# jfdev001/algebraic-multigrid

Hardware: AMD Instinct MI355X
Metric: V-cycles/sec, 2D Poisson N=4096^2 (fine-grid smoother HBM GB/s under roofline) (higher is better)
Workload: dtype f64; 1 GPU; 2D 5-point Poisson 4096x4096 (Grid::laplacian/rhs), true Jacobi smoother omega=0.6 2+2 sweeps, 16-level V-cycle, coarsest 511 dofs, fp64, 1xMI355X; smoother has no counterpart in the reference: pinned to the oracle twin; n=4096, dim=2, levels=16, smoother=jacobi, sweeps=2, graph=True, coarse_solve=band-chain (LDS-resident scalar recurrence, half-bandwidth <= 3, bit-exact), layout=dict

## Files before the change

### algebraic-multigrid_amd/amg_ctypes.py

```python
import contextlib
import ctypes as C
import os

import numpy as np

_HERE = os.path.dirname(os.path.abspath(__file__))
LIB_PATH = os.path.join(_HERE, "libamg_hip.so")

OK, EINVAL, EHIP, ENOMEM, EUNSUPPORTED, ECOMM = 0, 1, 2, 3, 4, 5
SM_SPGS, SM_REF_JACOBI, SM_SOR, SM_JACOBI, SM_MULTICOLOR_GS, SM_CHEBYSHEV, SM_LINE_JACOBI = 0, 1, 2, 3, 4, 5, 6
SM_LINE_ALT = 7
LAYOUT_AUTO, LAYOUT_CSR, LAYOUT_SELL, LAYOUT_DICT = 0, 1, 2, 3

_i32p = C.POINTER(C.c_int32)
_f64p = C.POINTER(C.c_double)
_i64p = C.POINTER(C.c_int64)


class AmgHipError(RuntimeError):
    def __init__(self, status, msg):
        super().__init__(f"amg_hip status {status}: {msg}")
        self.status = status
        self.message = msg

# ... 85 lines not shown
                                             C.POINTER(C.c_void_p)]),
    "amg_hip_create_tensor_semi_dev": (C.c_int, [C.c_int64, C.c_void_p, C.c_void_p, C.c_void_p, C.c_void_p,
                                                 C.c_int32, _i64p, C.c_int32, _i32p, C.c_double, C.c_int64,
                                                 C.POINTER(Options), C.POINTER(C.c_void_p)]),
    "amg_hip_get_level_axes": (C.c_int, [C.c_void_p, C.c_int32, _i32p]),
    "amg_hip_create_tensor_opdep": (C.c_int, [C.c_int64, _i32p, _i32p, _f64p, _f64p, C.c_int32, _i64p,
                                              C.c_int32, _i32p, C.c_int64, C.POINTER(Options),
                                              C.POINTER(C.c_void_p)]),
    "amg_hip_set_axis_stencil": (None, [C.c_int32]),
    "amg_hip_get_axis_weights": (C.c_int, [C.c_void_p, C.c_int32, _f64p]),
    "amg_hip_axis_restrict": (C.c_int, [C.c_int32, _i64p, C.c_int32, _f64p, _f64p, _f64p]),
    "amg_hip_axis_prolong_add": (C.c_int, [C.c_int32, _i64p, C.c_int32, _f64p, _f64p, _f64p]),
    "amg_hip_get_natural_sides": (C.c_int, [C.c_void_p, _i32p]),
    "amg_hip_create_tensor_periodic": (C.c_int, [C.c_int64, _i32p, _i32p, _f64p, _f64p, C.c_int32, _i64p,
                                                 C.c_int32, C.c_int32, _i32p, C.POINTER(Options),
                                                 C.POINTER(C.c_void_p)]),
    "amg_hip_create_tensor_periodic_dev": (C.c_int, [C.c_int64, C.c_void_p, C.c_void_p, C.c_void_p, C.c_void_p,
                                                     C.c_int32, _i64p, C.c_int32, C.c_int32, _i32p,
                                                     C.POINTER(Options), C.POINTER(C.c_void_p)]),
    "amg_hip_get_periodic_axes": (C.c_int, [C.c_void_p, _i32p]),
    "amg_hip_tensor_restrict_per": (C.c_int, [C.c_int32, _i64p, C.c_int32, C.c_int32, C.c_int32, _f64p, _f64p]),
    "amg_hip_tensor_prolong_add_per": (C.c_int, [C.c_int32, _i64p, C.c_int32, C.c_int32, C.c_int32, _f64p, _f64p]),
    "amg_hip_tensor_restrict_bc": (C.c_int, [C.c_int32, _i64p, C.c_int32, C.c_int32, _f64p, _f64p]),
    "amg_hip_tensor_prolong_add_bc": (C.c_int, [C.c_int32, _i64p, C.c_int32, C.c_int32, _f64p, _f64p]),
    "amg_hip_tensor_axis_strength": (C.c_int, [C.c_int64, _i32p, _i32p, _f64p, C.c_int32, _i64p, _f64p]),
    "amg_hip_tensor_restrict_axes": (C.c_int, [C.c_int32, _i64p, C.c_int32, _f64p, _f64p]),
    "amg_hip_tensor_prolong_add_axes": (C.c_int, [C.c_int32, _i64p, C.c_int32, _f64p, _f64p]),
    "amg_hip_level_transfer_kind": (C.c_int, [C.c_void_p, C.c_int32, _i32p]),
    "amg_hip_tensor_restrict": (C.c_int, [C.c_int32, _i64p, _f64p, _f64p]),
    "amg_hip_tensor_prolong_add": (C.c_int, [C.c_int32, _i64p, _f64p, _f64p]),
    "amg_hip_destroy": (None, [C.c_void_p]),
    "amg_hip_vcycle": (C.c_int, [C.c_void_p]),
    "amg_hip_vcycles": (C.c_int, [C.c_void_p, C.c_int32]),
    "amg_hip_sync": (C.c_int, [C.c_void_p]),
    "amg_hip_solve": (C.c_int, [C.c_void_p, C.c_double, C.c_int64, C.c_int64, _i64p, _f64p,
                                _i32p]),
    "amg_hip_rss": (C.c_int, [C.c_void_p, _f64p]),
    "amg_hip_apply": (C.c_int, [C.c_void_p, C.c_void_p, C.c_void_p]),
    "amg_hip_pcg": (C.c_int, [C.c_void_p, C.c_double, C.c_int64, _i64p, _f64p]),
    "amg_hip_set_mean_projection": (C.c_int, [C.c_void_p, C.c_int32]),
    "amg_hip_get_mean_projection": (C.c_int, [C.c_void_p, _i32p]),
    "amg_hip_center_vec": (C.c_int, [C.c_void_p, C.c_int32, C.c_int32]),
    "amg_hip_block_vcycles": (C.c_int, [C.c_void_p, C.c_int32, C.c_void_p, C.c_void_p, C.c_int32]),
    "amg_hip_block_rss": (C.c_int, [C.c_void_p, C.c_int32, C.c_void_p, C.c_void_p, _f64p]),
    "amg_hip_block_pcg": (C.c_int, [C.c_void_p, C.c_int32, C.c_void_p, C.c_void_p, C.c_double, C.c_int64,
                                    _i64p, _f64p]),
    "amg_hip_block_must_move": (C.c_int, [C.c_void_p, C.c_int32, _f64p]),
    "amg_hip_apply_f32": (C.c_int, [C.c_void_p, C.c_void_p, C.c_void_p]),
    "amg_hip_pcg_mixed": (C.c_int, [C.c_void_p, C.c_double, C.c_int64, _i64p, _f64p]),
    "amg_hip_f32_must_move": (C.c_int, [C.c_void_p, _f64p]),
    "amg_hip_f32_get_vec": (C.c_int, [C.c_void_p, C.c_int32, C.c_int32, C.POINTER(C.c_float)]),
    "amg_hip_f32_set_vec": (C.c_int, [C.c_void_p, C.c_int32, C.c_int32, C.POINTER(C.c_float)]),
    "amg_hip_f32_level_op": (C.c_int, [C.c_void_p, C.c_int32, C.c_int32]),
    "amg_hip_f32_line_subsweep": (C.c_int, [C.c_void_p, C.c_int32, C.c_int32, C.c_int32]),
    "amg_hip_f32_line_factors": (C.c_int, [C.c_void_p, C.c_int32] + [C.POINTER(C.c_float)] * 3),
    "amg_hip_set_f32_lines": (None, [C.c_int32]),
    "amg_hip_set_f32_dict": (None, [C.c_int32]),
    "amg_hip_set_block_lines": (None, [C.c_int32]),
    "amg_hip_n_levels": (C.c_int32, [C.c_void_p]),
    "amg_hip_get_n_dofs": (C.c_int64, [C.c_void_p, C.c_int32]),
    "amg_hip_get_level_nnz": (C.c_int64, [C.c_void_p, C.c_int32]),
    "amg_hip_get_level_matrix": (C.c_int, [C.c_void_p, C.c_int32, _i32p, _i32p, _f64p]),
    "amg_hip_get_transfer_nnz": (C.c_int64, [C.c_void_p, C.c_int32, C.c_int32]),
    "amg_hip_get_transfer": (C.c_int, [C.c_void_p, C.c_int32, C.c_int32, _i32p, _i32p, _f64p]),
    "amg_hip_get_vec": (C.c_int, [C.c_void_p, C.c_int32, C.c_int32, _f64p]),
    "amg_hip_set_vec": (C.c_int, [C.c_void_p, C.c_int32, C.c_int32, _f64p]),
    "amg_hip_copy_vec_dev": (C.c_int, [C.c_void_p, C.c_int32, C.c_int32, C.c_void_p, C.c_int32]),
    "amg_hip_zero_vec": (C.c_int, [C.c_void_p, C.c_int32, C.c_int32]),
    "amg_hip_coarse_halfbw": (C.c_int64, [C.c_void_p]),
    "amg_hip_coarse_solve_kind": (C.c_int32, [C.c_void_p]),
    "amg_hip_fine_sweep_info": (C.c_int, [C.c_void_p, C.c_char_p, C.c_int32, _i32p, _f64p]),
    "amg_hip_set_patch_min_rows": (None, [C.c_int64]),
    "amg_hip_set_band_chain": (None, [C.c_int32]),
    "amg_hip_set_tail_fusion": (None, [C.c_int32]),
    "amg_hip_set_pair_duo": (None, [C.c_int32]),
    "amg_hip_pair_duo_partner": (C.c_int32, [C.c_void_p, C.c_int32]),
    "amg_hip_duo_windows": (C.c_int32, [C.c_int32, C.c_int32, C.c_int32, _i32p]),
    "amg_hip_duo_owned": (C.c_int32, [C.c_int32, C.c_int32, _i32p]),
    "amg_hip_duo_tile_rows": (C.c_int32, [C.c_int32]),
    "amg_hip_set_periodic_device_setup": (None, [C.c_int32]),
    "amg_hip_set_patch_tile_flags": (None, [C.c_int32]),
    "amg_hip_set_patch_xf": (None, [C.c_int32]),
    "amg_hip_set_patch_tall": (None, [C.c_int32]),
    "amg_hip_set_patch_seam": (None, [C.c_int32]),
    "amg_hip_patch_leg_lines": (C.c_int32, [C.c_void_p, C.c_int32, C.c_int32]),
    "amg_hip_create_rs": (C.c_int, [C.c_int64, _i32p, _i32p, _f64p, _f64p, C.c_int32, C.c_double, C.c_int64,
                                    C.POINTER(Options), C.POINTER(C.c_void_p)]),
    "amg_hip_slab_plan": (C.c_int, [C.c_int64, C.c_int32, C.c_int32, C.c_int32, C.POINTER(SlabInfo)]),
    "amg_hip_slab_setup": (C.c_int, [C.c_void_p, C.c_int32, C.c_int32, C.c_int32, C.POINTER(SlabInfo)]),
    "amg_hip_slab_run": (C.c_int, [C.c_void_p, C.c_int32]),
    "amg_hip_create_poisson_window": (C.c_int, [C.c_int32, C.c_int64, C.c_int64, C.c_int64, C.c_int32,
                                                C.POINTER(Options), C.POINTER(C.c_void_p)]),
    "amg_hip_window_setup": (C.c_int, [C.c_void_p, _i64p, _i64p, _i64p, _i64p]),
    "amg_hip_window_run": (C.c_int, [C.c_void_p, C.c_int32]),
    "amg_hip_vec_dev_ptr": (C.c_int, [C.c_void_p, C.c_int32, C.c_int32, C.POINTER(C.c_void_p), _i64p]),
    "amg_hip_get_stream": (C.c_int, [C.c_void_p, C.POINTER(C.c_void_p)]),
    "amg_hip_comm_unique_id": (C.c_int, [C.c_char_p]),
    "amg_hip_comm_create": (C.c_int, [C.c_char_p, C.c_int32, C.c_int32, C.c_int32, C.POINTER(C.c_void_p)]),
    "amg_hip_comm_destroy": (None, [C.c_void_p]),
    "amg_hip_comm_rank": (C.c_int32, [C.c_void_p]),
    "amg_hip_comm_world": (C.c_int32, [C.c_void_p]),
    "amg_hip_comm_neighbor_exchange": (C.c_int, [C.c_void_p, C.c_void_p, C.c_int64, C.c_void_p, C.c_int64,
                                                 C.c_void_p, C.c_int64, C.c_void_p, C.c_int64, C.c_void_p]),
    "amg_hip_comm_all_gather": (C.c_int, [C.c_void_p, C.c_void_p, C.c_void_p, C.c_int64, C.c_void_p]),
    "amg_hip_slab_cycle": (C.c_int, [C.c_void_p, C.c_void_p, C.POINTER(SlabInfo)]),
    "amg_hip_window_cycle": (C.c_int, [C.c_void_p, C.c_void_p, C.c_void_p, C.POINTER(WindowPlanC)]),
    "amg_hip_level_layout": (C.c_int32, [C.c_void_p, C.c_int32, C.POINTER(C.c_int32), C.POINTER(C.c_int64)]),
    "amg_hip_get_colors": (C.c_int, [C.c_void_p, C.c_int32, _i32p, _i32p]),
    "amg_hip_level_op": (C.c_int, [C.c_void_p, C.c_int32, C.c_int32]),
    "amg_hip_cheb_bounds": (C.c_int, [C.c_void_p, C.c_int32, _f64p, _f64p]),
    "amg_hip_line_stride": (C.c_int, [C.c_void_p, C.c_int32, C.POINTER(C.c_int64)]),
    "amg_hip_smooth_line": (C.c_int, [C.c_int64, _i32p, _i32p, _f64p, C.c_int64, C.c_double, C.c_int64,
                                      _f64p, _f64p]),
    "amg_hip_line_directions": (C.c_int, [C.c_void_p, C.c_int32, C.POINTER(C.c_int32), C.POINTER(C.c_int64)]),
    "amg_hip_smooth_line_alt": (C.c_int, [C.c_int64, _i32p, _i32p, _f64p, C.c_int32, C.POINTER(C.c_int64),
                                          C.c_double, C.c_int64, C.c_int32, _f64p, _f64p]),
    "amg_hip_line_cyclic": (C.c_int, [C.c_void_p, C.c_int32, _i32p]),
    "amg_hip_smooth_line_alt_per": (C.c_int, [C.c_int64, _i32p, _i32p, _f64p, C.c_int32, C.POINTER(C.c_int64),
                                              C.c_int32, C.c_double, C.c_int64, C.c_int32, _f64p, _f64p]),
    "amg_hip_smooth_chebyshev": (C.c_int, [C.c_int64, _i32p, _i32p, _f64p, _f64p, _f64p, C.c_int32,
                                           C.c_double, C.c_double, C.c_int64]),
    "amg_hip_cycle_bytes": (C.c_int, [C.c_void_p, _f64p, _f64p]),
    "amg_hip_cycle_must_move": (C.c_int, [C.c_void_p, C.c_int32, _f64p]),
    "amg_hip_profile_fine_sweep": (C.c_int, [C.c_void_p, C.c_int32, _f64p, _f64p]),
    "amg_hip_smooth": (C.c_int, [C.c_int32, C.c_int64, _i32p, _i32p, _f64p, _f64p, _f64p,
                                 C.c_double, C.c_double, C.c_int64, C.c_int64, _i64p, _i32p]),
    "amg_hip_spgs_sweep": (C.c_int, [C.c_int32, C.c_int64, _i32p, _i32p, _f64p, _f64p, _f64p]),
    "amg_hip_residual": (C.c_int, [C.c_int64, _i32p, _i32p, _f64p, _f64p, _f64p, _f64p]),
    "amg_hip_spmv": (C.c_int, [C.c_int64, C.c_int64, _i32p, _i32p, _f64p, _f64p, _f64p]),
    "amg_hip_linear_restrict": (C.c_int, [C.c_int64, C.c_int64, _f64p, _f64p]),
    "amg_hip_linear_prolong_add": (C.c_int, [C.c_int64, C.c_int64, _f64p, _f64p]),
    "amg_hip_rss_host": (C.c_int, [C.c_int64, _i32p, _i32p, _f64p, _f64p, _f64p, _f64p]),
    "amg_hip_coarse_solve": (C.c_int, [C.c_int64, _i32p, _i32p, _f64p, _f64p, _f64p, _i64p]),
    "amg_hip_coarse_solve_fast": (C.c_int, [C.c_int64, _i32p, _i32p, _f64p, _f64p, _f64p, _i64p,
                                            _i32p]),
    "amg_hip_laplacian": (C.c_int64, [C.c_int32, C.c_int64, _i32p, _i32p, _f64p]),
    "amg_hip_rhs": (C.c_int, [C.c_int32, C.c_int64, _f64p]),
    "amg_hip_csr_shape": (C.c_int, [C.c_int64, _i32p, _i32p, _i32p]),
    "amg_hip_dev_residual": (C.c_int, [C.c_int64, C.c_int64, C.c_int32, C.c_int32, C.c_void_p,
                                       C.c_void_p, C.c_void_p, C.c_void_p, C.c_void_p,
                                       C.c_void_p, C.c_void_p]),
    "amg_hip_dev_jacobi": (C.c_int, [C.c_int64, C.c_int64, C.c_int32, C.c_int32, C.c_void_p,
                                     C.c_void_p, C.c_void_p, C.c_void_p, C.c_void_p, C.c_void_p,
                                     C.c_double, C.c_int64, C.c_void_p]),
    "amg_hip_dev_spmv": (C.c_int, [C.c_int64, C.c_int64, C.c_int32, C.c_int32, C.c_void_p,
                                   C.c_void_p, C.c_void_p, C.c_void_p, C.c_void_p, C.c_void_p]),
    "amg_hip_devmat_create": (C.c_int, [C.c_int64, C.c_int64, _i32p, _i32p, _f64p, C.c_int32,
                                        C.c_int64, C.c_int32, C.POINTER(C.c_void_p)]),
    "amg_hip_set_index16": (None, [C.c_int32]),
    "amg_hip_set_nontemporal": (None, [C.c_int32]),
    "amg_hip_set_dict_rows": (None, [C.c_int32]),
    "amg_hip_set_dict_stencil": (None, [C.c_int32]),
    "amg_hip_set_xcd_mapping": (None, [C.c_int32]),
    "amg_hip_set_row_types": (None, [C.c_int32]),
    "amg_hip_dict_probe": (C.c_int, [C.c_int64, C.c_int64, _i32p, _i32p, _f64p, C.c_int64,
                                     C.POINTER(C.c_int32), C.POINTER(C.c_int32), C.POINTER(C.c_int32)]),
    "amg_hip_devmat_destroy": (None, [C.c_void_p]),
    "amg_hip_devmat_layout": (C.c_int, [C.c_void_p, C.POINTER(C.c_int32), C.POINTER(C.c_int64)]),
    "amg_hip_devmat_apply": (C.c_int, [C.c_void_p, C.c_int32, C.c_void_p, C.c_void_p, C.c_void_p,
                                       C.c_double, C.c_int64, C.c_void_p]),
    "amg_hip_dev_jacobi_from_zero": (C.c_int, [C.c_int64, C.c_void_p, C.c_void_p, C.c_void_p,
                                               C.c_double, C.c_void_p]),
    "amg_hip_dev_axpy1": (C.c_int, [C.c_int64, C.c_void_p, C.c_void_p, C.c_void_p]),
    "amg_hip_arena_create": (C.c_int, [C.c_int64, C.c_int32, C.POINTER(C.c_void_p)]),
    "amg_hip_arena_destroy": (None, [C.c_void_p]),
    "amg_hip_arena_base": (C.c_void_p, [C.c_void_p]),
# ... 60 lines not shown


def set_default_layout(layout):
    lib().amg_hip_set_default_layout(layout)


def set_index16(on):
    lib().amg_hip_set_index16(int(on))


def set_nontemporal(on):
    lib().amg_hip_set_nontemporal(int(on))


def set_dict_rows(rows_per_lane):
    lib().amg_hip_set_dict_rows(int(rows_per_lane))


def set_dict_stencil(on):
    lib().amg_hip_set_dict_stencil(int(on))


def dict_probe(rowptr, col, val, ncols, diag_shift=0):
    rowptr, col, val = _a32(rowptr), _a32(col), _a64(val)
    a, b, c = C.c_int32(0), C.c_int32(0), C.c_int32(0)
    st = lib().amg_hip_dict_probe(rowptr.size - 1, ncols, _p32(rowptr), _p32(col), _p64(val),
                                  diag_shift, C.byref(a), C.byref(b), C.byref(c))
    if st == EUNSUPPORTED:
        return None
    _chk(st)
    return a.value, b.value, c.value


class Comm:

    def __init__(self, id_bytes, rank, world, device=-1):
        h = C.c_void_p()
        _chk(lib().amg_hip_comm_create(bytes(id_bytes), int(rank), int(world), int(device), C.byref(h)))
        self._h, self.rank, self.world = h, rank, world

    @staticmethod
    def unique_id():
        buf = C.create_string_buffer(128)
        _chk(lib().amg_hip_comm_unique_id(buf))
        return buf.raw

    def slab_cycle(self, mg, info):
        _chk(lib().amg_hip_slab_cycle(mg._h, self._h, C.byref(info)))

    def window_cycle(self, window_mg, tail_mg, plan_c):
        _chk(lib().amg_hip_window_cycle(window_mg._h, tail_mg._h, self._h, C.byref(plan_c)))

    def close(self):
        if getattr(self, "_h", None):
            lib().amg_hip_comm_destroy(self._h)
            self._h = None

    def __del__(self):
        self.close()


def slab_plan(lines, rank, world, levels):
    info = SlabInfo()
    _chk(lib().amg_hip_slab_plan(int(lines), int(rank), int(world), int(levels), C.byref(info)))
    return info


def set_patch_tile_flags(on):
    lib().amg_hip_set_patch_tile_flags(int(bool(on)))


def set_axis_stencil(on):
    lib().amg_hip_set_axis_stencil(int(bool(on)))


def set_patch_xf(on):
    lib().amg_hip_set_patch_xf(int(bool(on)))


def set_patch_tall(on):
    lib().amg_hip_set_patch_tall(int(bool(on)))


def set_patch_seam(on):
    lib().amg_hip_set_patch_seam(int(bool(on)))


def set_tail_fusion(on):
    lib().amg_hip_set_tail_fusion(int(bool(on)))


def set_pair_duo(on):
    lib().amg_hip_set_pair_duo(int(bool(on)))


DUO_WINDOWS_LEN = 31


def duo_windows(hb_l, hb_l1, tile_rows=510):
    out = np.zeros(DUO_WINDOWS_LEN, np.int32)
    rc = lib().amg_hip_duo_windows(int(hb_l), int(hb_l1), int(tile_rows), out.ctypes.data_as(_i32p))
    return rc == 0, out


def duo_owned(tile, tile_rows=510):
    out = np.zeros(6, np.int32)
    if lib().amg_hip_duo_owned(int(tile), int(tile_rows), out.ctypes.data_as(_i32p)) != 0:
        raise ValueError("amg_hip_duo_owned: bad argument")
    return [(int(out[0]), int(out[1])), (int(out[2]), int(out[3])), (int(out[4]), int(out[5]))]


def duo_tile_rows(hb_l):
    return int(lib().amg_hip_duo_tile_rows(int(hb_l)))


def set_periodic_device_setup(on):
    lib().amg_hip_set_periodic_device_setup(int(bool(on)))


def set_f32_lines(on):
    lib().amg_hip_set_f32_lines(int(bool(on)))


@contextlib.contextmanager
def f32_lines():
    set_f32_lines(1)
    try:
        yield
    finally:
        set_f32_lines(0)


def set_f32_dict(on):
    lib().amg_hip_set_f32_dict(int(bool(on)))


@contextlib.contextmanager
def f32_dict():
    set_f32_dict(1)
    try:
        yield
    finally:
        set_f32_dict(0)


def set_block_lines(on):
    lib().amg_hip_set_block_lines(int(bool(on)))


@contextlib.contextmanager
def block_lines():
    set_block_lines(1)
    try:
        yield
    finally:
        set_block_lines(0)


def set_band_chain(on):
    lib().amg_hip_set_band_chain(int(bool(on)))


PATCH_MIN_ROWS_DEFAULT = 1000000


def set_patch_min_rows(rows):
# ... 525 lines not shown
        return int(lib().amg_hip_get_n_dofs(self._h, level))

    def get_coefficient_matrix(self, level):
        n = self.get_n_dofs(level)
        nnz = lib().amg_hip_get_level_nnz(self._h, level)
        colptr = np.empty(n + 1, np.int32)
        rowind = np.empty(nnz, np.int32)
        val = np.empty(nnz, np.float64)
        _chk(lib().amg_hip_get_level_matrix(self._h, level, _p32(colptr), _p32(rowind), _p64(val)))
        return colptr, rowind, val

    def get_transfer(self, level, which):
        w = 1 if which == "R" else 0
        nnz = lib().amg_hip_get_transfer_nnz(self._h, level, w)
        if nnz < 0:
            raise ValueError("level out of range")
        n_h, n_H = self.get_n_dofs(level), self.get_n_dofs(level + 1)
        cols = n_h if w else n_H
        colptr = np.empty(cols + 1, np.int32)
        rowind = np.empty(nnz, np.int32)
        val = np.empty(nnz, np.float64)
        _chk(lib().amg_hip_get_transfer(self._h, level, w, _p32(colptr), _p32(rowind), _p64(val)))
        return colptr, rowind, val

    def _get(self, level, which):
        out = np.empty(self.get_n_dofs(level), np.float64)
        _chk(lib().amg_hip_get_vec(self._h, level, which, _p64(out)))
        return out

    def get_soln(self, level=0):
        return self._get(level, 0)

    def get_rhs(self, level=0):
        return self._get(level, 1)

    def get_residual(self, level=0):
        return self._get(level, 2)

    def set_vec(self, level, which, v):
        v = _a64(v)
        assert v.size == self.get_n_dofs(level)
        _chk(lib().amg_hip_set_vec(self._h, level, {"u": 0, "f": 1, "r": 2}[which], _p64(v)))

    def copy_vec_dev(self, level, which, dev_ptr, to_solver):
        _chk(lib().amg_hip_copy_vec_dev(self._h, level, {"u": 0, "f": 1, "r": 2}[which],
                                        C.c_void_p(dev_ptr), int(to_solver)))

    def zero_vec(self, level, which):
        _chk(lib().amg_hip_zero_vec(self._h, level, {"u": 0, "f": 1, "r": 2}[which]))

    def get_tolerance(self):
        return self.tolerance

    def level_layout(self, level):
        lay, nb = C.c_int32(0), C.c_int64(0)
        _chk(lib().amg_hip_level_layout(self._h, level, C.byref(lay), C.byref(nb)))
        return int(lay.value), int(nb.value)

    def coarse_halfbw(self):
        return int(lib().amg_hip_coarse_halfbw(self._h))

    def get_colors(self, level):
        color = np.empty(self.get_n_dofs(level), np.int32)
        nc = C.c_int32(0)
        _chk(lib().amg_hip_get_colors(self._h, level, _p32(color), C.byref(nc)))
        return color, nc.value

    def cycle_bytes(self):
        a, b = C.c_double(0), C.c_double(0)
        _chk(lib().amg_hip_cycle_bytes(self._h, C.byref(a), C.byref(b)))
        return a.value, b.value

    def cycle_must_move(self, part=0):
        b = C.c_double(0)
        _chk(lib().amg_hip_cycle_must_move(self._h, int(part), C.byref(b)))
        return b.value

    def pair_duo_partner(self, level):
        return int(lib().amg_hip_pair_duo_partner(self._h, int(level)))

    def patch_leg_lines(self, level, leg):
        return int(lib().amg_hip_patch_leg_lines(self._h, int(level), int(leg)))

    def profile_fine_sweep(self, n_launches):
        a, b = C.c_double(0), C.c_double(0)
        _chk(lib().amg_hip_profile_fine_sweep(self._h, n_launches, C.byref(a), C.byref(b)))
        name = C.create_string_buffer(256)
        k, nb = C.c_int32(0), C.c_double(0)
        _chk(lib().amg_hip_fine_sweep_info(self._h, name, 256, C.byref(k), C.byref(nb)))
        return a.value, b.value, k.value, name.value.decode(), nb.value

    def fine_sweep_info(self):
        name = C.create_string_buffer(256)
        k, nb = C.c_int32(0), C.c_double(0)
        _chk(lib().amg_hip_fine_sweep_info(self._h, name, 256, C.byref(k), C.byref(nb)))
        return name.value.decode(), k.value, nb.value

    def cheb_bounds(self, level):
        lo, hi = C.c_double(0), C.c_double(0)
        st = lib().amg_hip_cheb_bounds(self._h, int(level), C.byref(lo), C.byref(hi))
        if st == EINVAL:
            raise ValueError(lib().amg_hip_last_error().decode())
        _chk(st)
        return lo.value, hi.value

    def line_stride(self, level):
        s = C.c_int64(0)
        st = lib().amg_hip_line_stride(self._h, int(level), C.byref(s))
        if st == EINVAL:
            raise ValueError(lib().amg_hip_last_error().decode())
        _chk(st)
        return s.value

    def line_directions(self, level):
        nd = C.c_int32(0)
        st3 = (C.c_int64 * 3)()
        st = lib().amg_hip_line_directions(self._h, int(level), C.byref(nd), st3)
        if st == EINVAL:
            raise ValueError(lib().amg_hip_last_error().decode())
        _chk(st)
        return [int(st3[d]) for d in range(nd.value)]

    def line_cyclic(self, level):
        m = C.c_int32(0)
        st = lib().amg_hip_line_cyclic(self._h, int(level), C.byref(m))
        if st == EINVAL:
            raise ValueError(lib().amg_hip_last_error().decode())
        _chk(st)
        return m.value

    def coarse_solve_kind(self):
        return {0: "band (one wave, sequential, bit-exact)", 1: "spike (partitioned, parallel)",
                2: "band-wide (blocked sequential, any half-bandwidth, bit-exact)",
                3: "band-chain (LDS-resident scalar recurrence, half-bandwidth <= 3, bit-exact)"}[
                    int(lib().amg_hip_coarse_solve_kind(self._h))]

    def level_op(self, level, op):
        _chk(lib().amg_hip_level_op(self._h, level, op))

    def vcycle(self, n=1):
        _chk(lib().amg_hip_vcycles(self._h, n))

    def sync(self):
        _chk(lib().amg_hip_sync(self._h))

    def rss(self):
        out = C.c_double(0)
        _chk(lib().amg_hip_rss(self._h, C.byref(out)))
        return out.value

    def slab_setup(self, rank, world, max_levels=-1):
        info = SlabInfo()
        _chk(lib().amg_hip_slab_setup(self._h, int(rank), int(world), int(max_levels), C.byref(info)))
        return info

    def slab_run(self, part):
        _chk(lib().amg_hip_slab_run(self._h, int(part)))

    def apply_dev(self, v_dev, z_dev):
        _chk(lib().amg_hip_apply(self._h, C.c_void_p(v_dev), C.c_void_p(z_dev)))

    def pcg(self, rtol=1e-10, max_iters=100):
        it, rel = C.c_int64(0), C.c_double(0)
        _chk(lib().amg_hip_pcg(self._h, rtol, max_iters, C.byref(it), C.byref(rel)))
        return self.get_soln(0), it.value, rel.value

# ... 360 lines not shown
```

### algebraic-multigrid_amd/csrc/kernels.hip

```cpp
#include <hip/hip_runtime.h>
#include <cstdlib>
#include <stdint.h>

#include <cstdio>
#include <type_traits>
#include <utility>
#include <vector>
#include <algorithm>
#include <cmath>

#include "kernels.hpp"

namespace amg_hip {

__device__ __forceinline__ void lds_barrier() {
  asm volatile("s_waitcnt lgkmcnt(0)\n\ts_barrier" ::: "memory");
}

constexpr bool mode_cheb(int m) { return (m & ~3) == 16; }
constexpr bool mode_jac(int m) { return m == CSR_JACOBI || mode_cheb(m); }
constexpr bool cheb_first(int m) { return (m & 1) != 0; }
constexpr bool cheb_last(int m) { return (m & 2) != 0; }
template <int MODE>
__device__ __forceinline__ double cheb_update(double t, double xi, double di, double alpha, double beta,
// ... 1506 lines not shown
  constexpr int WC0 = DUO_U_M0 * W0, WC1 = DUO_U_M1 * W1;
  __shared__ DictEntry tab[256];
  __shared__ __attribute__((aligned(16))) uint64_t wc0[WC0];
  __shared__ __attribute__((aligned(16))) uint64_t wc1[WC1];
  __shared__ uint16_t tw0[DUO_U_M0 / 2];
  __shared__ uint16_t tw1[DUO_U_M1 / 2];
  __shared__ __attribute__((aligned(16))) double aw1[DUO_U_A1];
  __shared__ __attribute__((aligned(16))) double fw1[DUO_U_M1];
  __shared__ __attribute__((aligned(16))) double uw1[DUO_U_M1];
  __shared__ __attribute__((aligned(16))) double aw0[DUO_U_A0];
  __shared__ __attribute__((aligned(16))) double fw0[DUO_U_M0];
  __shared__ __attribute__((aligned(16))) double uw0[DUO_U_M0];
  double* vw1 = aw1;
  double* rs = aw0;
  int w[DW_COUNT];
  duo_windows(hbw0, hbw1, T, w);
  const int tile = xcd_tile(blockIdx.x, gridDim.x, xcd_map);
  const int t0 = tile * T, ce = (t0 / 2) & ~1;
  const int m0 = t0 - hbw0, M0 = w[DW_U_M0], A0 = w[DW_U_A0];
  const int m1 = ce - w[DW_U_M1_LO], M1 = w[DW_U_M1], A1 = w[DW_U_A1];
  const bool types0 = rtype0 != nullptr, types1 = rtype1 != nullptr;
  const int t = threadIdx.x;
  DuoLoads<W1, (DUO_U_A1 / 2 + 255) / 256, 1> g1;
  DuoLoads<W0, (DUO_U_A0 / 2 + 255) / 256, (DUO_U_M0 + 511) / 512> g0;
  if (types1) duo_issue<W1, true>(g1, n1, m1 - hbw1, A1, m1, M1, codes1, rtype1, rwords1, doff1, dval1, ntab1, a1, f1);
  else duo_issue<W1, false>(g1, n1, m1 - hbw1, A1, m1, M1, codes1, rtype1, rwords1, doff1, dval1, ntab1, a1, f1);
  if (types0) duo_issue<W0, true>(g0, n0, m0 - hbw0, A0, m0, M0, codes0, rtype0, rwords0, doff0, dval0, ntab0, u0_in, f0);
  else duo_issue<W0, false>(g0, n0, m0 - hbw0, A0, m0, M0, codes0, rtype0, rwords0, doff0, dval0, ntab0, u0_in, f0);
  pair_f64x2 pre[2];
  double pre1;
  if (T == DUO_T) dict_prolong_pre<DUO_T>(tile, n0, n_h, uh_in, pre, pre1);
  else dict_prolong_pre<DUO_T_SMALL>(tile, n0, n_h, uh_in, pre, pre1);
  dict_put_table<CSR_JACOBI>(tab, g1.tv, g1.to, ntab1);
  if (types1) duo_commit<W1, true>(g1, n1, A1, m1, M1, wc1, tw1, aw1, fw1);
  else duo_commit<W1, false>(g1, n1, A1, m1, M1, wc1, tw1, aw1, fw1);
  if (types0) duo_commit<W0, true>(g0, n0, A0, m0, M0, wc0, tw0, aw0, fw0);
  else duo_commit<W0, false>(g0, n0, A0, m0, M0, wc0, tw0, aw0, fw0);
  __syncthreads();
  duo_stage<CSR_JACOBI, W1, U1>(n1, m1, M1, 0, M1, types1, tab, wc1, tw1, fw1, aw1, hbw1, omega, uw1, nullptr, 0, 0);
  __syncthreads();
  int own[6];
  duo_owned(t0, T, own);
  const int c_own = own[2], c_end = own[3];
  duo_stage<CSR_JACOBI, W1, U1>(n1, m1, M1, hbw1, w[DW_U_S1], types1, tab, wc1, tw1, fw1, uw1, 0, omega, vw1,
                                u1_out, c_own, c_end);
  __syncthreads();
  dict_put_table<CSR_JACOBI>(tab, g0.tv, g0.to, ntab0);
  {
    const int s1 = ce - w[DW_U_S1_LO], a_lo = m0 - hbw0;
    for (int k = 2 * t; k < A0; k += 512) {
      const int i = a_lo + k;
      if (i < 0 || i >= n0) continue;
      const int j = i >> 1;
      double p0 = 0.0, p1 = 0.0;
      const double b = (j < n1) ? vw1[j - s1] : 0.0;
      if (j >= 1 && j - 1 < n1) p0 += 0.5 * vw1[j - 1 - s1];
      if (j < n1) {
        p0 += 0.5 * b;
        p1 += 1.0 * b;
      }
      aw0[k] = aw0[k] + p0;
      if (i + 1 < n0) aw0[k + 1] = aw0[k + 1] + p1;
    }
  }
  __syncthreads();
  duo_stage<CSR_JACOBI, W0, U0>(n0, m0, M0, 0, M0, types0, tab, wc0, tw0, fw0, aw0, hbw0, omega, uw0, nullptr, 0, 0);
  __syncthreads();
  duo_stage<CSR_JACOBI, W0, U0>(n0, m0, M0, hbw0, w[DW_U_S0], types0, tab, wc0, tw0, fw0, uw0, 0, omega, rs, u0_out,
                                own[0], own[1]);
  __syncthreads();
  if (T == DUO_T) dict_prolong_tail<DUO_T>(tile, n0, rs, n_h, pre, pre1, uh_out);
  else dict_prolong_tail<DUO_T_SMALL>(tile, n0, rs, n_h, pre, pre1, uh_out);
}

constexpr int PATCH_TW = 64;
constexpr int PATCH_EH = 48;
constexpr int patch_th(int rings) { return PATCH_EH - 2 * rings; }
static bool patch_rings_ok(int rings) { return rings == 2 || rings == 3; }
constexpr int PATCH_EC = PATCH_TW + 8;
constexpr int PATCH_NT = 432;
constexpr int PATCH_K = PATCH_EH * PATCH_EC / PATCH_NT;
constexpr int PATCH_BUF = (PATCH_EH + 2) * PATCH_EC;
constexpr int PATCH_MAXTAB = 192;
static_assert(PATCH_EH * PATCH_EC == PATCH_K * PATCH_NT && PATCH_NT % PATCH_EC == 0, "patch geometry");
template <int EH_, int EC_>
struct PatchFrameT {
  static constexpr int EH = EH_, EC = EC_, CL = (EC_ - PATCH_TW) / 2;
  static constexpr int NT = EH_ / PATCH_K * EC_, BUF = (EH_ + 2) * EC_;
  static constexpr int th(int rings) { return EH_ - 2 * rings; }
  static_assert(EH_ % PATCH_K == 0 && (EC_ - PATCH_TW) % 2 == 0 && NT >= PATCH_MAXTAB && NT <= 1024, "patch frame");
};
using PatchFrame = PatchFrameT<PATCH_EH, PATCH_EC>;
static_assert(PatchFrame::NT == PATCH_NT && PatchFrame::BUF == PATCH_BUF && PatchFrame::CL == 4, "patch geometry");

struct PatchJ { double a, d; };
struct PatchR { double a; int32_t loff, ok; };

struct PatchCells {
  int cell0, row0, lj0, li;
  double f[PATCH_K];
  uint32_t ty[PATCH_K / 4];
  bool live[PATCH_K];
  bool uniform;
  uint32_t tu;
  bool flagged;
  __device__ __forceinline__ uint32_t type(int k) const {
    return flagged ? tu : (ty[k >> 2] >> (8 * (k & 3))) & 255u;
  }
};

struct PatchU {
  double wj[9], wr[9], diag;
#ifdef AMG_PATCH_FASTDIV
  double rdiag;
#endif
  uint32_t rmask, corners;
};
__device__ __forceinline__ void patch_load_u(PatchU& U, uint32_t tu, const double* __restrict__ utabd,
                                             const int32_t* __restrict__ utabi) {
  const double* d = utabd + (size_t)tu * 19;
  const int32_t* i = utabi + (size_t)tu * 2;
#pragma unroll
  for (int e = 0; e < 9; ++e) {
    U.wj[e] = d[e];
    U.wr[e] = d[9 + e];
  }
  U.diag = d[18];
#ifdef AMG_PATCH_FASTDIV
  U.rdiag = 1.0 / (U.diag == 0.0 ? 1.0 : U.diag);
#endif
  U.rmask = (uint32_t)i[0];
  U.corners = (uint32_t)i[1];
}
template <bool RESID, bool CORNERS, bool GS = false, int MASK = -1, class FR = PatchFrame>
__device__ __forceinline__ void patch_eval_u(const double* buf, int cell0, const PatchU& U,
                                             const double (&f)[PATCH_K], double omega,
                                             double (&res)[PATCH_K]) {
  const double* p = buf + cell0 - FR::EC;
  if (!CORNERS && !RESID && U.diag == 0.0) {
#pragma unroll
    for (int k = 0; k < PATCH_K; ++k) res[k] = p[(k + 1) * FR::EC];
    return;
  }
  double w[3][3];
#pragma unroll
  for (int r = 0; r < 2; ++r)
#pragma unroll
    for (int c = 0; c < 3; ++c) w[r][c] = (CORNERS || c == 1 || r == 1) ? p[r * FR::EC + c - 1] : 0.0;
#pragma unroll
  for (int k = 0; k < PATCH_K; ++k) {
#pragma unroll
    for (int c = 0; c < 3; ++c)
      w[2][c] = (CORNERS || c == 1) ? p[(k + 2) * FR::EC + c - 1] : 0.0;
    if (!CORNERS) {
      w[2][0] = p[(k + 2) * FR::EC - 1];
      w[2][2] = p[(k + 2) * FR::EC + 1];
    }
    const double xi = w[1][1];
    if (RESID) {
      double acc = f[k];
#pragma unroll
      for (int s9 = 0; s9 < 9; ++s9) {
        const int r = s9 / 3, c = s9 % 3;
        if (!CORNERS && r != 1 && c != 1) continue;
        if (MASK >= 0) {
          if ((MASK >> s9) & 1) acc -= U.wr[s9] * w[r][c];
        } else {
          double t = U.wr[s9] * w[r][c];
          t = ((U.rmask >> s9) & 1u) ? t : 0.0;
          acc -= t;
        }
      }
      res[k] = acc;
    } else {
      double acc = 0.0;
#pragma unroll
      for (int s9 = 0; s9 < 9; ++s9) {
        const int r = s9 / 3, c = s9 % 3;
        if (s9 == 4 || (!CORNERS && r != 1 && c != 1)) continue;
        if (MASK >= 0 && !((MASK >> s9) & 1)) continue;
        acc += U.wj[s9] * w[r][c];
      }
      if (CORNERS && U.diag == 0.0) {
        res[k] = xi;
      } else {
#ifdef AMG_PATCH_FASTDIV
        const double nm = f[k] - acc;
        const double q0 = nm * U.rdiag;
        const double r0 = __builtin_fma(-U.diag, q0, nm);
        const double q1 = __builtin_fma(r0, U.rdiag, q0);
        const double r1 = __builtin_fma(-U.diag, q1, nm);
        const double q = __builtin_fma(r1, U.rdiag, q1);
#else
        const double q = (f[k] - acc) / U.diag;
#endif
        res[k] = GS ? q : xi + omega * (q - xi);
      }
    }
#pragma unroll
    for (int c = 0; c < 3; ++c) {
      w[0][c] = w[1][c];
      w[1][c] = w[2][c];
    }
  }
}
template <int UN, bool RESID, bool GS = false>
__device__ __forceinline__ double patch_eval(const double* buf, int cell, uint32_t type,
                                             const PatchJ* tabJ, const PatchR* tabR, double fi,
                                             double omega) {
  const int t0 = (int)type * UN;
  double xx[UN];
  if (RESID) {
    double av[UN];
    bool ok[UN];
#pragma unroll
    for (int e = 0; e < UN; ++e) {
      const PatchR r = tabR[t0 + e];
      av[e] = r.a;
      ok[e] = r.ok != 0;
      xx[e] = buf[cell + r.loff];
    }
    double acc = fi;
#pragma unroll
    for (int e = 0; e < UN; ++e) {
      double t = av[e] * xx[e];
      t = ok[e] ? t : 0.0;
      acc -= t;
    }
    return acc;
  }
  double aj[UN], dj[UN];
#pragma unroll
  for (int e = 0; e < UN; ++e) {
    const PatchJ j = tabJ[t0 + e];
    aj[e] = j.a; dj[e] = j.d;
    xx[e] = buf[cell + tabR[t0 + e].loff];
  }
  double acc = 0.0, diag = 0.0;
  const double xi = buf[cell];
#pragma unroll
  for (int e = 0; e < UN; ++e) {
    acc += aj[e] * xx[e];
    diag += dj[e];
  }
  const bool nod = diag == 0.0;
  const double q = (fi - acc) / (nod ? 1.0 : diag);
  return nod ? xi : (GS ? q : xi + omega * (q - xi));
}

template <int UN, int UM, bool RESID, bool NT, bool ZERO, int TH, class FR = PatchFrame>
__device__ __forceinline__ void patch_stage(const PatchCells& pc, int m, int ntypes, double* buf,
                                            const PatchU& U, const PatchJ* tabJ, const PatchR* tabR,
                                            double omega, int l0, int l1, int c0, int c1, double* out) {
  const bool inc = pc.li >= c0 && pc.li < c1;
  double res[PATCH_K];
  bool did[PATCH_K], inr[PATCH_K];
#pragma unroll
  for (int k = 0; k < PATCH_K; ++k) {
    const int lj = pc.lj0 + k;
    inr[k] = inc && lj >= l0 && lj < l1;
    did[k] = inr[k] && pc.live[k];
  }
  if (pc.uniform && U.rmask == (uint32_t)UM) {
    patch_eval_u<RESID, (UM & 0x145) != 0, false, (UM & 0x145) ? -1 : UM, FR>(buf, pc.cell0, U, pc.f, omega, res);
  } else {
#pragma unroll
    for (int k = 0; k < PATCH_K; ++k)
      res[k] = patch_eval<UN, RESID>(buf, pc.cell0 + k * FR::EC,
                                     did[k] ? pc.type(k) : (uint32_t)ntypes, tabJ, tabR, pc.f[k], omega);
  }
  lds_barrier();
  const bool outc = out != nullptr && pc.li >= 0 && pc.li < PATCH_TW;
#pragma unroll
  for (int k = 0; k < PATCH_K; ++k) {
    if (did[k]) buf[pc.cell0 + k * FR::EC] = res[k];
    else if (ZERO && inr[k]) buf[pc.cell0 + k * FR::EC] = 0.0;
    const int lj = pc.lj0 + k;
    if (outc && did[k] && lj >= 0 && lj < TH) {
      double* op = out + (pc.row0 + k * m);
      if (NT) __builtin_nontemporal_store(res[k], op);
      else *op = res[k];
    }
  }
}

template <bool NT, int RINGS, class FR = PatchFrame>
__device__ __forceinline__ void patch_copy_out(const double* buf, double* __restrict__ out, int n, int m,
                                               int j0, int i0) {
  for (int q = threadIdx.x; q < FR::th(RINGS) * PATCH_TW; q += FR::NT) {
    const int lj = q / PATCH_TW, li = q - lj * PATCH_TW;
    const int64_t row = (int64_t)(j0 + lj) * m + i0 + li;
    if (row < (int64_t)n) {
      const double v = buf[(lj + RINGS + 1) * FR::EC + li + FR::CL];
      if (NT) __builtin_nontemporal_store(v, out + row);
      else out[row] = v;
    }
  }
}

struct __attribute__((aligned(8))) PatchPair { double x, y; };

__device__ __forceinline__ uint32_t patch_flag(const uint8_t* __restrict__ flag, int idx) {
  const uint32_t* __restrict__ w = reinterpret_cast<const uint32_t*>(flag);
  return (w[idx >> 2] >> (8 * (idx & 3))) & 255u;
}

static_assert(PATCH_MAXTAB <= PATCH_NT, "one table row per thread");
struct PatchTabRow { double v[4]; };
__device__ __forceinline__ void patch_issue_tables(PatchTabRow& tb, const double* __restrict__ ptab, int nent) {
  const int t = (int)threadIdx.x < nent ? (int)threadIdx.x : 0;
#pragma unroll
  for (int q = 0; q < 4; ++q) tb.v[q] = ptab[4 * t + q];
}
template <class FR = PatchFrame>
__device__ __forceinline__ void patch_stage_tables(PatchJ* tabJ, PatchR* tabR, const PatchTabRow& tb, int nent) {
  const int t = threadIdx.x;
  if (t >= PATCH_MAXTAB) return;
  PatchJ j = {0.0, 0.0};
  PatchR r = {0.0, 0, 0};
  if (t < nent) {
    j.a = tb.v[0];
    j.d = tb.v[1];
    r.a = tb.v[2];
    const double lo = tb.v[3];
    r.ok = lo > -1.0e8 ? 1 : 0;
    r.loff = r.ok ? (int)lo : 0;
    if (FR::EC != PATCH_EC) r.loff += (r.loff > PATCH_EC / 2 ? 1 : (r.loff < -PATCH_EC / 2 ? -1 : 0)) * (FR::EC - PATCH_EC);
  }
  tabJ[t] = j;
  tabR[t] = r;
}
template <class FR = PatchFrame>
__device__ __forceinline__ void patch_clear_guards(double* buf) {
  for (int t = threadIdx.x; t < 2 * FR::EC; t += FR::NT)
    buf[t < FR::EC ? t : FR::BUF - 2 * FR::EC + t] = 0.0;
}
template <int UM, class FR = PatchFrame>
__device__ __forceinline__ void patch_prologue(const PatchCells& pc, const PatchU& U, double* buf, PatchJ* tabJ,
                                               PatchR* tabR, const double* __restrict__ ptab, int nent) {
  if (pc.flagged && U.rmask != (uint32_t)UM) {
    PatchTabRow tb;
    patch_issue_tables(tb, ptab, nent);
    patch_stage_tables<FR>(tabJ, tabR, tb, nent);
  }
  patch_clear_guards<FR>(buf);
}

template <class FR = PatchFrame>
__device__ __forceinline__ void patch_form_x(const PatchCells& pc, const PatchU& U,
                                             const double* __restrict__ utabd, double omega, double* buf) {
  double dv[PATCH_K];
  if (pc.uniform) {
#pragma unroll
    for (int k = 0; k < PATCH_K; ++k) dv[k] = U.diag;
  } else {
#pragma unroll
    for (int k = 0; k < PATCH_K; ++k) dv[k] = utabd[(size_t)pc.type(k) * 19 + 18];
  }
#pragma unroll
  for (int k = 0; k < PATCH_K; ++k) {
    const double sum = pc.f[k], d = dv[k];
    const double xi = 0.0, acc = 0.0;
    const double x0 = (d == 0.0) ? xi : xi + omega * ((sum - acc) / d - xi);
    buf[pc.cell0 + k * FR::EC] = pc.live[k] ? x0 : 0.0;
  }
}

template <int RINGS, bool PROLONG, bool XF = false, class FR = PatchFrame>
__device__ __forceinline__ void patch_load(PatchCells& pc, PatchU& U, const uint8_t* __restrict__ tflag,
                                           int tile, int n, int m,
                                           int j0, int i0, const double* __restrict__ x,
                                           const double* __restrict__ f,
                                           const uint8_t* __restrict__ rtype, int ntypes,
                                           const double* __restrict__ uH, int nH,
                                           const double* __restrict__ ptab, int nent,
                                           const double* __restrict__ utabd,
                                           const int32_t* __restrict__ utabi, double omega, double* buf,
                                           PatchJ* tabJ, PatchR* tabR) {
  const int g = (int)threadIdx.x / FR::EC, col = (int)threadIdx.x - g * FR::EC;
  const int le = g * PATCH_K;
  pc.lj0 = le - RINGS;
  pc.li = col - FR::CL;
  pc.cell0 = (le + 1) * FR::EC + col;
  const int64_t r0 = (int64_t)(j0 + pc.lj0) * m + i0 + pc.li;
  pc.row0 = (int)(r0 < -((int64_t)1 << 30) ? -((int64_t)1 << 30) : r0);
  double xv[PATCH_K];
  PatchPair pr[PATCH_K];
#pragma unroll
  for (int k = 0; k < PATCH_K; ++k) {
    const int64_t r64 = r0 + (int64_t)k * m;
    pc.live[k] = r64 >= 0 && r64 < (int64_t)n;
    if (!XF) xv[k] = x[pc.live[k] ? (int)r64 : 0];
  }
  if (PROLONG) {
#pragma unroll
    for (int k = 0; k < PATCH_K; ++k) {
      const int row = pc.row0 + k * m;
      const int j = pc.live[k] ? (row >> 1) : 0;
      const int jc = j < 1 ? 1 : (j > nH - 1 ? nH - 1 : j);
      pr[k] = *reinterpret_cast<const PatchPair*>(uH + (jc - 1));
    }
  }
  if (!PROLONG) {
#pragma unroll
    for (int k = 0; k < PATCH_K; ++k) {
      const int64_t r64 = r0 + (int64_t)k * m;
      pc.f[k] = f[pc.live[k] ? (int)r64 : 0];
    }
  }
  __builtin_amdgcn_sched_barrier(0);
  const uint32_t tf = tflag ? patch_flag(tflag, tile) : 255u;
  const uint32_t nty = (uint32_t)ntypes;
  pc.flagged = tf != 255u;
  if (pc.flagged) {
    pc.tu = tf;
    pc.uniform = true;
  } else {
    PatchTabRow tb;
    patch_issue_tables(tb, ptab, nent);
    uint32_t mism = 0, ty[PATCH_K];
#pragma unroll
    for (int k = 0; k < PATCH_K; ++k) {
      const int64_t r64 = r0 + (int64_t)k * m;
      ty[k] = (uint32_t)rtype[pc.live[k] ? (int)r64 : 0];
    }
#pragma unroll
    for (int q = 0; q < PATCH_K / 4; ++q) pc.ty[q] = 0;
#pragma unroll
    for (int k = 0; k < PATCH_K; ++k) {
      ty[k] = (pc.live[k] && ty[k] < nty) ? ty[k] : nty;
      pc.ty[k >> 2] |= ty[k] << (8 * (k & 3));
    }
    pc.tu = (uint32_t)__builtin_amdgcn_readfirstlane((int)ty[0]);
#pragma unroll
    for (int q = 0; q < PATCH_K / 4; ++q) mism |= pc.ty[q] ^ (pc.tu * 0x01010101u);
    pc.uniform = __builtin_amdgcn_ballot_w64(mism != 0) == 0 && pc.tu < nty;
    patch_stage_tables<FR>(tabJ, tabR, tb, nent);
  }
  {
    int fl = pc.flagged;
    asm("" : "+v"(fl));
    pc.flagged = __builtin_amdgcn_readfirstlane(fl) != 0;
  }
  patch_load_u(U, pc.uniform ? pc.tu : 0u, utabd, utabi);
  __builtin_amdgcn_sched_barrier(0);
  if (XF) patch_form_x<FR>(pc, U, utabd, omega, buf);
  if (PROLONG) {
    int row0 = pc.row0;
    asm volatile("" : "+v"(row0));
    pc.row0 = row0;
  }
#pragma unroll
  for (int k = 0; k < PATCH_K && !XF; ++k) {
    const int row = pc.row0 + k * m;
    double x0 = pc.live[k] ? xv[k] : 0.0;
    if (PROLONG) {
      const int j = pc.live[k] ? (row >> 1) : 0;
      const int jc = j < 1 ? 1 : (j > nH - 1 ? nH - 1 : j);
      const bool odd = (row & 1) != 0;
      const bool a_ok = pc.live[k] && !odd && j >= 1 && j - 1 < nH;
      const bool b_ok = pc.live[k] && j < nH;
      const double a = (j == jc) ? pr[k].x : pr[k].y;
      const double b = (j == jc) ? pr[k].y : pr[k].x;
      double t = 0.0;
      t = a_ok ? t + 0.5 * a : t;
      t = b_ok ? t + (odd ? 1.0 : 0.5) * b : t;
      x0 = pc.live[k] ? x0 + t : x0;
    }
    buf[pc.cell0 + k * FR::EC] = x0;
  }
  if (PROLONG) {
    __builtin_amdgcn_sched_barrier(0);
#pragma unroll
    for (int k = 0; k < PATCH_K; ++k) pc.f[k] = f[pc.live[k] ? pc.row0 + k * m : 0];
  }
}

__global__ __launch_bounds__(256) void patch_tile_flags_kernel(int n, int m, int px_count, int rings, int eh, int ec,
                                                               const uint8_t* __restrict__ rtype,
                                                               int ntypes, uint8_t* __restrict__ flag) {
  const int tile = blockIdx.x;
  const int py = tile / px_count, px = tile - py * px_count;
  const int64_t base = (int64_t)(py * (eh - 2 * rings) - rings) * m + px * PATCH_TW - (ec - PATCH_TW) / 2;
  const int64_t first = base < 0 ? 0 : (base < n ? base : n - 1);
  const uint32_t t0 = rtype[first];
  int ok = base >= 0 && t0 < (uint32_t)ntypes;
  for (int q = threadIdx.x; q < eh * ec; q += 256) {
    const int le = q / ec, c = q - le * ec;
    const int64_t r = base + (int64_t)le * m + c;
    ok = ok && r >= 0 && r < (int64_t)n && rtype[r < 0 ? 0 : (r < n ? r : n - 1)] == t0;
  }
  ok = __syncthreads_and(ok);
  if (threadIdx.x == 0) flag[tile] = ok ? (uint8_t)t0 : (uint8_t)255;
}
hipError_t launch_patch_tile_flags(int64_t n, int64_t m, int rings, const uint8_t* rtype, int ntypes,
                                   uint8_t* flag, int64_t* n_tiles, hipStream_t st) {
  if (!patch_geometry_ok(n, m) || !patch_rings_ok(rings)) return hipErrorInvalidValue;
  const int64_t lines = (n + m - 1) / m;
  const int pxc = (int)(m / PATCH_TW);
  const int64_t th = patch_th(rings);
  const int64_t tiles = (lines + th - 1) / th * pxc;
  if (n_tiles) *n_tiles = tiles;
  if (!flag) return hipSuccess;
  hipLaunchKernelGGL(patch_tile_flags_kernel, dim3((unsigned)tiles), dim3(256), 0, st, (int)n, (int)m, pxc,
                     rings, PATCH_EH, PATCH_EC, rtype, ntypes, flag);
  return hipGetLastError();
}

__global__ __launch_bounds__(256) void patch_coarse_flags_kernel(int n, int m, int px_count, int th, int nH,
                                                                 const double* __restrict__ diagH, double dref,
                                                                 uint8_t* __restrict__ cflag) {
  const int tile = blockIdx.x;
  const int py = tile / px_count, px = tile - py * px_count;
  const int j0 = py * th, i0 = px * PATCH_TW;
  int ok = 1;
  for (int q = threadIdx.x; q < th * (PATCH_TW / 2); q += 256) {
    const int lj = q / (PATCH_TW / 2), cx = q - lj * (PATCH_TW / 2);
    const int64_t i = (int64_t)(j0 + lj) * m + i0 + 2 * cx;
    const int64_t c = i >> 1;
    if (i >= (int64_t)n || c >= nH) continue;
    ok = ok && __double_as_longlong(diagH[c]) == __double_as_longlong(dref);
  }
  ok = __syncthreads_and(ok);
  if (threadIdx.x == 0) cflag[tile] = ok ? 1 : 0;
}
hipError_t launch_patch_coarse_flags(int64_t n, int64_t m, int rings, int64_t nH, const double* diagH,
                                     double dref, uint8_t* cflag, hipStream_t st) {
  if (!patch_geometry_ok(n, m) || !patch_rings_ok(rings) || !diagH || !cflag) return hipErrorInvalidValue;
  const int64_t lines = (n + m - 1) / m;
  const int pxc = (int)(m / PATCH_TW);
  const int64_t th = patch_th(rings);
  const int64_t tiles = (lines + th - 1) / th * pxc;
  hipLaunchKernelGGL(patch_coarse_flags_kernel, dim3((unsigned)tiles), dim3(256), 0, st, (int)n, (int)m, pxc,
                     (int)th, (int)nH, diagH, dref, cflag);
  return hipGetLastError();
}

#ifdef AMG_PATCH_STAMPS
__device__ unsigned long long* g_patch_stamps = nullptr;
__device__ __forceinline__ void patch_stamp(int k) {
  if (threadIdx.x == 0 && g_patch_stamps) {
    unsigned long long t = __builtin_amdgcn_s_memrealtime();
    asm volatile("s_waitcnt lgkmcnt(0)" ::: "memory");
    g_patch_stamps[(size_t)blockIdx.x * 8 + k] = t;
    if (k == 0) {
      const unsigned hw = __builtin_amdgcn_s_getreg((31 << 11) | 4);
      const unsigned xcc = __builtin_amdgcn_s_getreg((3 << 11) | 20);
      g_patch_stamps[(size_t)blockIdx.x * 8 + 7] = ((unsigned long long)xcc << 32) | hw;
    }
  }
}
hipError_t debug_set_patch_stamps(unsigned long long* p) {
  return hipMemcpyToSymbol(HIP_SYMBOL(g_patch_stamps), &p, sizeof(p));
}
#define PATCH_STAMP(k) patch_stamp(k)
#else
#define PATCH_STAMP(k)
#endif
template <int UN, int UM, bool FIRST, bool NT, bool XF = false, int RINGS = 3>
#ifndef AMG_PATCH_WAVES
#define AMG_PATCH_WAVES 7
#endif
__global__ __launch_bounds__(PATCH_NT, (UN == 5 ? AMG_PATCH_WAVES : AMG_PATCH_WAVES - 1)) void patch_down_kernel(
    int n, int m, int px_count, const uint8_t* __restrict__ rtype, const double* __restrict__ ptab,
    const double* __restrict__ utabd, const int32_t* __restrict__ utabi,
    int nent, int ntypes, const double* x, const double* __restrict__ f, double* u_out, double* r_out, int nH,
    double* __restrict__ fH, const double* __restrict__ diagH, double* __restrict__ uH1,
    double omega, int xcd_map, int py0, const uint8_t* __restrict__ tflag,
    const uint8_t* __restrict__ cflag, double dHu) {
  __shared__ double buf[PATCH_BUF];
  __shared__ PatchJ tabJ[PATCH_MAXTAB];
  __shared__ PatchR tabR[PATCH_MAXTAB];
  PATCH_STAMP(0);
  const int tile = xcd_tile(blockIdx.x, gridDim.x, xcd_map);
  const int py = tile / px_count, px = tile - py * px_count;
  constexpr int TH = patch_th(RINGS);
  const int j0 = (py + py0) * TH, i0 = px * PATCH_TW;
  PatchCells pc;
  PatchU U;
  const int ftile = (py + py0) * px_count + px;
  static_assert(!(FIRST && XF), "level 0 starts from its own u");
  static_assert(RINGS == 3 || (RINGS == 2 && !FIRST), "three dependent stages (FIRST) need three rings");
  patch_load<RINGS, false, XF>(pc, U, tflag, ftile, n, m, j0, i0, x, f, rtype, ntypes, nullptr, 0, ptab, nent,
                               utabd, utabi, omega, buf, tabJ, tabR);
  patch_prologue<UM>(pc, U, buf, tabJ, tabR, ptab, nent);
  const bool cuni = uH1 && cflag && patch_flag(cflag, ftile) != 0;
  lds_barrier();
  PATCH_STAMP(1);
  if (FIRST) {
    patch_stage<UN, UM, false, NT, false, TH>(pc, m, ntypes, buf, U, tabJ, tabR, omega, -2, TH + 2, -2,
                                              PATCH_TW + 3, nullptr);
    lds_barrier();
  }
  PATCH_STAMP(2);
  patch_stage<UN, UM, false, NT, false, TH>(pc, m, ntypes, buf, U, tabJ, tabR, omega, -1, TH + 1, -1,
                                            PATCH_TW + 2, nullptr);
  lds_barrier();
  PATCH_STAMP(3);
  patch_copy_out<NT, RINGS>(buf, u_out, n, m, j0, i0);
  patch_stage<UN, UM, true, NT, true, TH>(pc, m, ntypes, buf, U, tabJ, tabR, omega, 0, TH, 0, PATCH_TW + 1,
                                          r_out);
  lds_barrier();
  PATCH_STAMP(4);
  const double* rsb = buf;
  for (int q = threadIdx.x; q < TH * (PATCH_TW / 2); q += PATCH_NT) {
    const int lj = q / (PATCH_TW / 2), cx = q - lj * (PATCH_TW / 2);
    const int64_t i = (int64_t)(j0 + lj) * m + i0 + 2 * cx;
    const int64_t c = i >> 1;
    if (i >= (int64_t)n || c >= nH) continue;
    const double* rs = rsb + (lj + RINGS + 1) * PATCH_EC + 2 * cx + 4;
    double sum = 0.0;
    if (i < n) sum += 0.5 * rs[0];
    if (i + 1 < n) sum += 1.0 * rs[1];
    if (i + 2 < n) sum += 0.5 * rs[2];
    fH[c] = sum;
    if (uH1 == nullptr) continue;
    const double xi = 0.0, acc = 0.0;
    const double d = cuni ? dHu : diagH[c];
    uH1[c] = (d == 0.0) ? xi : xi + omega * ((sum - acc) / d - xi);
  }
  PATCH_STAMP(5);
}

template <int UN, int UM, bool NT, int RINGS = 3>
__global__ __launch_bounds__(PATCH_NT, AMG_PATCH_WAVES) void patch_up_kernel(
    int n, int m, int px_count, const uint8_t* __restrict__ rtype, const double* __restrict__ ptab,
    const double* __restrict__ utabd, const int32_t* __restrict__ utabi,
    int nent, int ntypes, const double* x, const double* __restrict__ f, const double* __restrict__ uH, int nH,
    double* u_out, double omega, int xcd_map, int py0, const uint8_t* __restrict__ tflag) {
  __shared__ double buf[PATCH_BUF];
  __shared__ PatchJ tabJ[PATCH_MAXTAB];
  __shared__ PatchR tabR[PATCH_MAXTAB];
  const int tile = xcd_tile(blockIdx.x, gridDim.x, xcd_map);
  const int py = tile / px_count, px = tile - py * px_count;
  static_assert(RINGS == 2 || RINGS == 3, "two dependent stages");
  constexpr int TH = patch_th(RINGS);
  const int j0 = (py + py0) * TH, i0 = px * PATCH_TW;
  PatchCells pc;
  PatchU U;
  patch_load<RINGS, true>(pc, U, tflag, (py + py0) * px_count + px, n, m, j0, i0, x, f, rtype, ntypes, uH, nH,
                          ptab, nent, utabd, utabi, omega, buf, tabJ, tabR);
  patch_prologue<UM>(pc, U, buf, tabJ, tabR, ptab, nent);
  lds_barrier();
  patch_stage<UN, UM, false, NT, false, TH>(pc, m, ntypes, buf, U, tabJ, tabR, omega, -1, TH + 1, -1,
                                            PATCH_TW + 1, nullptr);
  lds_barrier();
  patch_stage<UN, UM, false, NT, false, TH>(pc, m, ntypes, buf, U, tabJ, tabR, omega, 0, TH, 0, PATCH_TW,
                                            nullptr);
  lds_barrier();
  patch_copy_out<NT, RINGS>(buf, u_out, n, m, j0, i0);
}

constexpr int PATCH_SEAM_RINGS = 5;
template <int UN, int UM, bool NT, class FR, int WAVES>
__global__ __launch_bounds__(FR::NT, WAVES) void patch_seam_kernel(
    int n, int m, int px_count, const uint8_t* __restrict__ rtype, const double* __restrict__ ptab,
    const double* __restrict__ utabd, const int32_t* __restrict__ utabi,
    int nent, int ntypes, const double* x, const double* __restrict__ f, const double* __restrict__ uH, int nH,
    double* u_out, double* __restrict__ fH, double omega, int xcd_map, const uint8_t* __restrict__ tflag) {
  __shared__ double buf[FR::BUF];
  __shared__ PatchJ tabJ[PATCH_MAXTAB];
  __shared__ PatchR tabR[PATCH_MAXTAB];
  const int tile = xcd_tile(blockIdx.x, gridDim.x, xcd_map);
  const int py = tile / px_count, px = tile - py * px_count;
  constexpr int RINGS = PATCH_SEAM_RINGS, TH = FR::th(RINGS);
  static_assert(TH >= 1 && FR::CL >= RINGS + 1, "five stages and the restriction's column");
  const int j0 = py * TH, i0 = px * PATCH_TW;
  PatchCells pc;
  PatchU U;
  patch_load<RINGS, true, false, FR>(pc, U, tflag, tile, n, m, j0, i0, x, f, rtype, ntypes, uH, nH, ptab, nent,
                                     utabd, utabi, omega, buf, tabJ, tabR);
  patch_prologue<UM, FR>(pc, U, buf, tabJ, tabR, ptab, nent);
  lds_barrier();
#pragma unroll
  for (int q = 4; q >= 1; --q) {
    patch_stage<UN, UM, false, NT, false, TH, FR>(pc, m, ntypes, buf, U, tabJ, tabR, omega, -q, TH + q, -q,
                                                  PATCH_TW + q + 1, nullptr);
    lds_barrier();
  }
  patch_copy_out<NT, RINGS, FR>(buf, u_out, n, m, j0, i0);
  patch_stage<UN, UM, true, NT, true, TH, FR>(pc, m, ntypes, buf, U, tabJ, tabR, omega, 0, TH, 0, PATCH_TW + 1,
                                              nullptr);
  lds_barrier();
  for (int q = threadIdx.x; q < TH * (PATCH_TW / 2); q += FR::NT) {
    const int lj = q / (PATCH_TW / 2), cx = q - lj * (PATCH_TW / 2);
    const int64_t i = (int64_t)(j0 + lj) * m + i0 + 2 * cx;
    const int64_t c = i >> 1;
    if (i >= (int64_t)n || c >= nH) continue;
    const double* rs = buf + (lj + RINGS + 1) * FR::EC + 2 * cx + FR::CL;
    double sum = 0.0;
    if (i < n) sum += 0.5 * rs[0];
    if (i + 1 < n) sum += 1.0 * rs[1];
    if (i + 2 < n) sum += 0.5 * rs[2];
    fH[c] = sum;
  }
}

template <int UN, int UM>
__device__ __forceinline__ void patch_stage_color(const PatchCells& pc, int ntypes, double* buf,
                                                  const PatchU& U, const PatchJ* tabJ, const PatchR* tabR,
                                                  int l0, int l1, int c0, int c1, uint32_t cbits,
                                                  uint32_t c) {
  const bool inc = pc.li >= c0 && pc.li < c1;
  double res[PATCH_K];
  bool did[PATCH_K];
#pragma unroll
  for (int k = 0; k < PATCH_K; ++k) {
    const int lj = pc.lj0 + k;
    did[k] = inc && lj >= l0 && lj < l1 && pc.live[k] && ((cbits >> (2 * k)) & 3u) == c;
  }
  bool any = false;
#pragma unroll
  for (int k = 0; k < PATCH_K; ++k) any |= did[k];
  if (__builtin_amdgcn_ballot_w64(any) == 0) return;
  if (pc.uniform && U.rmask == (uint32_t)UM) {
    constexpr bool CN = (UM & 0x145) != 0;
    constexpr int MK = (UM & 0x145) ? -1 : UM;
    patch_eval_u<false, CN, true, MK>(buf, pc.cell0, U, pc.f, 1.0, res);
  } else {
#pragma unroll
    for (int k = 0; k < PATCH_K; ++k)
      res[k] = patch_eval<UN, false, true>(buf, pc.cell0 + k * PATCH_EC,
                                           did[k] ? pc.type(k) : (uint32_t)ntypes, tabJ, tabR, pc.f[k], 1.0);
  }
#pragma unroll
  for (int k = 0; k < PATCH_K; ++k)
    if (did[k]) buf[pc.cell0 + k * PATCH_EC] = res[k];
}

template <int UN, int UM, bool NT, bool PROLONG, bool TAIL>
#ifndef AMG_RB_WAVES
#define AMG_RB_WAVES 5
#endif
__global__ __launch_bounds__(PATCH_NT, AMG_RB_WAVES) void patch_rb_kernel(
    int n, int m, int px_count, const uint8_t* __restrict__ rtype, const double* __restrict__ ptab,
    const double* __restrict__ utabd, const int32_t* __restrict__ utabi, int nent, int ntypes,
    const double* x, const double* __restrict__ f, const double* __restrict__ uH, int nH, double* u_out,
    double* r_out, double* __restrict__ fH, double* __restrict__ uH_zero, uint32_t stages, uint32_t ctab,
    int xcd_map, int py0, const uint8_t* __restrict__ tflag) {
  __shared__ double buf[PATCH_BUF];
  __shared__ PatchJ tabJ[PATCH_MAXTAB];
  __shared__ PatchR tabR[PATCH_MAXTAB];
  const int tile = xcd_tile(blockIdx.x, gridDim.x, xcd_map);
  const int py = tile / px_count, px = tile - py * px_count;
  constexpr int RINGS = 3, TH = patch_th(RINGS);
  const int j0 = (py + py0) * TH, i0 = px * PATCH_TW;
  PatchCells pc;
  PatchU U;
  patch_load<RINGS, PROLONG>(pc, U, tflag, (py + py0) * px_count + px, n, m, j0, i0, x, f, rtype, ntypes, uH, nH,
                             ptab, nent, utabd, utabi, 1.0, buf, tabJ, tabR);
  patch_prologue<UM>(pc, U, buf, tabJ, tabR, ptab, nent);
  uint32_t cbits = 0;
  {
    const int col = i0 + pc.li;
    const uint32_t line = (uint32_t)(j0 + pc.lj0 + (col < 0 ? -1 : (col >= m ? 1 : 0)) + 64);
    const int tc = col < 0 ? col + m : (col >= m ? col - m : col);
    const uint32_t cls = tc == 0 ? 0u : (tc == 1 ? 1u : (tc == m - 2 ? 2u : (tc == m - 1 ? 3u : 4u + ((uint32_t)tc & 1u))));
#pragma unroll
    for (int k = 0; k < PATCH_K; ++k)
      cbits |= ((ctab >> (2u * (((line + (uint32_t)k) & 1u) * 6u + cls))) & 3u) << (2 * k);
  }
  lds_barrier();
  if (pc.flagged) pc.ty[0] = pc.ty[1] = 0;
  constexpr int E = TAIL ? 1 : 0;
  const int nst = (int)(stages & 7u);
  for (int sg = 0; sg < nst; ++sg) {
    const int ext = nst - 1 - sg + E;
    asm volatile("" : "+v"(pc.ty[0]), "+v"(pc.ty[1]));
    patch_stage_color<UN, UM>(pc, ntypes, buf, U, tabJ, tabR, -ext, TH + ext, -ext, PATCH_TW + ext + E,
                              cbits, (stages >> (4 + 2 * sg)) & 3u);
    lds_barrier();
  }
  patch_copy_out<NT, RINGS>(buf, u_out, n, m, j0, i0);
  if (TAIL) {
    patch_stage<UN, UM, true, NT, true, TH>(pc, m, ntypes, buf, U, tabJ, tabR, 1.0, 0, TH, 0, PATCH_TW + 1,
                                            r_out);
    lds_barrier();
    for (int q = threadIdx.x; q < TH * (PATCH_TW / 2); q += PATCH_NT) {
      const int lj = q / (PATCH_TW / 2), cx = q - lj * (PATCH_TW / 2);
      const int64_t i = (int64_t)(j0 + lj) * m + i0 + 2 * cx;
      const int64_t c = i >> 1;
      if (i >= (int64_t)n || c >= nH) continue;
      const double* rs = buf + (lj + RINGS + 1) * PATCH_EC + 2 * cx + 4;
      double sum = 0.0;
      if (i < n) sum += 0.5 * rs[0];
      if (i + 1 < n) sum += 1.0 * rs[1];
      if (i + 2 < n) sum += 0.5 * rs[2];
      fH[c] = sum;
      if (uH_zero) uH_zero[c] = 0.0;
    }
  }
}
int patch_un(int un) { return un <= 5 ? 5 : un <= 7 ? 7 : 9; }
bool patch_geometry_ok(int64_t n, int64_t m) {
  return m >= 2 * PATCH_TW && (m % PATCH_TW) == 0 && n >= m && n < ((int64_t)1 << 31) - 4 * m - 64;
}
static unsigned patch_grid(int64_t n, int64_t m, int th, int64_t line_lo, int64_t line_hi, int* px_count,
                           int* py0) {
  const int64_t lines = (n + m - 1) / m;
  if (line_hi < 0 || line_hi > lines) line_hi = lines;
  if (line_lo < 0) line_lo = 0;
  if (line_lo > line_hi) line_lo = line_hi;
  *px_count = (int)(m / PATCH_TW);
  *py0 = (int)(line_lo / th);
  return (unsigned)(((line_hi + th - 1) / th - *py0) * *px_count);
}
int patch_tile_lines(int rings) { return patch_rings_ok(rings) ? patch_th(rings) : 0; }
int patch_leg_rings(bool first) { return first ? 3 : 2; }
int patch_default_umask(int un) { return un <= 5 ? 0x0BA : (un <= 7 ? 0x1D7 : 0x1FF); }
int patch_kind_umask(int un, int umask) { return (un > 7 && un <= 9 && umask == 0x1D7) ? 0x1D7 : patch_default_umask(un); }
template <class F>
static hipError_t patch_dispatch(int un, int umask, bool nt, F&& go) {
  using std::integral_constant;
  auto with_nt = [&](auto U, auto M) {
    if (nt) go(U, M, integral_constant<bool, true>{});
    else go(U, M, integral_constant<bool, false>{});
  };
  if (un <= 5) with_nt(integral_constant<int, 5>{}, integral_constant<int, 0x0BA>{});
  else if (un <= 7) with_nt(integral_constant<int, 7>{}, integral_constant<int, 0x1D7>{});
  else if (un <= 9 && umask == 0x1D7) with_nt(integral_constant<int, 9>{}, integral_constant<int, 0x1D7>{});
  else if (un <= 9) with_nt(integral_constant<int, 9>{}, integral_constant<int, 0x1FF>{});
  else return hipErrorInvalidValue;
  return hipGetLastError();
}
hipError_t launch_patch_down(bool first, int64_t n, int64_t m, const PatchRef& P, const double* x,
                             const double* f, double* u_out, double* r_out, int64_t nH, double* fH,
                             const double* diagH, double* uH1, double omega, hipStream_t st,
                             int64_t line_lo, int64_t line_hi, bool xf) {
  if (!patch_geometry_ok(n, m) || !P.rtype || !P.ptab || !P.utabd || !P.utabi || (P.ntypes + 1) * patch_un(P.un) > PATCH_MAXTAB ||
      P.nent != P.ntypes * patch_un(P.un) || !fH || (uH1 && !diagH) || !u_out || u_out == x || (xf ? first : !x) ||
      !patch_rings_ok(P.rings) || P.rings < patch_leg_rings(first))
    return hipErrorInvalidValue;
  int pxc = 0, py0 = 0;
  const unsigned grid = patch_grid(n, m, patch_th(P.rings), line_lo, line_hi, &pxc, &py0);
  if (grid == 0) return hipSuccess;
  const int xm = g_xcd_map ? 1 : 0;
  return patch_dispatch(P.un, P.umask, P.nt != 0, [&](auto U, auto M, auto NTF) {
#define AMG_DOWN(FST, XFF, RG)                                                                                 \
  hipLaunchKernelGGL((patch_down_kernel<decltype(U)::value, decltype(M)::value, FST, decltype(NTF)::value, XFF, RG>), \
                     dim3(grid), dim3(PATCH_NT), 0, st, (int)n, (int)m, pxc, P.rtype, P.ptab, P.utabd, P.utabi, \
                     P.nent, P.ntypes, x, f, u_out, r_out, (int)nH, fH, diagH, uH1, omega, xm, py0, P.tflag,    \
                     P.cflag, P.dHu)
    if (first) AMG_DOWN(true, false, 3);
    else if (xf && P.rings == 2) AMG_DOWN(false, true, 2);
    else if (xf) AMG_DOWN(false, true, 3);
    else if (P.rings == 2) AMG_DOWN(false, false, 2);
    else AMG_DOWN(false, false, 3);
#undef AMG_DOWN
  });
}
hipError_t launch_patch_up(int64_t n, int64_t m, const PatchRef& P, const double* x, const double* f,
                           const double* uH, int64_t nH, double* u_out, double omega,
                           hipStream_t st, int64_t line_lo, int64_t line_hi) {
  if (!patch_geometry_ok(n, m) || !P.rtype || !P.ptab || !P.utabd || !P.utabi || (P.ntypes + 1) * patch_un(P.un) > PATCH_MAXTAB ||
      P.nent != P.ntypes * patch_un(P.un) || !uH || !u_out || u_out == x || !patch_rings_ok(P.rings))
    return hipErrorInvalidValue;
  int pxc = 0, py0 = 0;
  const unsigned grid = patch_grid(n, m, patch_th(P.rings), line_lo, line_hi, &pxc, &py0);
  if (grid == 0) return hipSuccess;
  const int xm = g_xcd_map ? 1 : 0;
  return patch_dispatch(P.un, P.umask, P.nt != 0, [&](auto U, auto M, auto NTF) {
#define AMG_UP(RG)                                                                                            \
  hipLaunchKernelGGL((patch_up_kernel<decltype(U)::value, decltype(M)::value, decltype(NTF)::value, RG>),     \
                     dim3(grid), dim3(PATCH_NT), 0, st, (int)n, (int)m, pxc, P.rtype, P.ptab, P.utabd, P.utabi, \
                     P.nent, P.ntypes, x, f, uH, (int)nH, u_out, omega, xm, py0, P.tflag)
    if (P.rings == 2) AMG_UP(2);
    else AMG_UP(3);
#undef AMG_UP
  });
}
using SeamFrame = PatchFrameT<48, 76>;
constexpr int PATCH_SEAM_WAVES = 6;
int patch_seam_lines() { return SeamFrame::th(PATCH_SEAM_RINGS); }
static bool patch_seam_geometry_ok(int64_t n, int64_t m) {
  return patch_geometry_ok(n, m) && n < ((int64_t)1 << 31) - 64 * m - 128;
}
hipError_t launch_patch_seam_flags(int64_t n, int64_t m, const uint8_t* rtype, int ntypes, uint8_t* flag,
                                   int64_t* n_tiles, hipStream_t st) {
  if (!patch_seam_geometry_ok(n, m)) return hipErrorInvalidValue;
  const int64_t lines = (n + m - 1) / m;
  const int pxc = (int)(m / PATCH_TW);
  const int64_t th = patch_seam_lines();
  const int64_t tiles = (lines + th - 1) / th * pxc;
  if (n_tiles) *n_tiles = tiles;
  if (!flag) return hipSuccess;
  hipLaunchKernelGGL(patch_tile_flags_kernel, dim3((unsigned)tiles), dim3(256), 0, st, (int)n, (int)m, pxc,
                     PATCH_SEAM_RINGS, SeamFrame::EH, SeamFrame::EC, rtype, ntypes, flag);
  return hipGetLastError();
}
hipError_t launch_patch_seam(int64_t n, int64_t m, const PatchRef& P, const double* x, const double* f,
                             const double* uH, int64_t nH, double* u_out, double* fH, double omega,
                             hipStream_t st) {
  if (!patch_seam_geometry_ok(n, m) || !P.rtype || !P.ptab || !P.utabd || !P.utabi ||
      (P.ntypes + 1) * patch_un(P.un) > PATCH_MAXTAB || P.nent != P.ntypes * patch_un(P.un) || !x || !f || !uH ||
      nH < 2 || !u_out || u_out == x || !fH || P.rings != PATCH_SEAM_RINGS || patch_un(P.un) != 5)
    return hipErrorInvalidValue;
  int pxc = 0, py0 = 0;
  const unsigned grid = patch_grid(n, m, patch_seam_lines(), 0, -1, &pxc, &py0);
  if (grid == 0) return hipSuccess;
  const int xm = g_xcd_map ? 1 : 0;
#define AMG_SEAM(NTF)                                                                                          \
  hipLaunchKernelGGL((patch_seam_kernel<5, 0x0BA, NTF, SeamFrame, PATCH_SEAM_WAVES>), dim3(grid), dim3(SeamFrame::NT), \
                     0, st, (int)n, (int)m, pxc, P.rtype, P.ptab, P.utabd, P.utabi, P.nent, P.ntypes, x, f, uH,  \
                     (int)nH, u_out, fH, omega, xm, P.tflag)
  if (P.nt) AMG_SEAM(true);
  else AMG_SEAM(false);
#undef AMG_SEAM
  return hipGetLastError();
}
int patch_rb_max_stages(bool tail) { return tail ? 2 : 3; }
uint32_t patch_rb_stages(const int* colors, int count) {
  uint32_t v = (uint32_t)count & 7u;
  for (int q = 0; q < count && q < 4; ++q) v |= ((uint32_t)colors[q] & 3u) << (4 + 2 * q);
  return v;
}
hipError_t launch_patch_rb(bool prolong, bool tail, int64_t n, int64_t m, const PatchRef& P, const double* x,
                           const double* f, const double* uH, int64_t nH, double* u_out, double* r_out,
                           double* fH, double* uH_zero, uint32_t stages, uint32_t ctab, hipStream_t st,
                           int64_t line_lo, int64_t line_hi) {
  const int nst = (int)(stages & 7u);
  if (!patch_geometry_ok(n, m) || !P.rtype || !P.ptab || !P.utabd || !P.utabi || (P.ntypes + 1) * patch_un(P.un) > PATCH_MAXTAB ||
      P.nent != P.ntypes * patch_un(P.un) || !u_out || u_out == x || (prolong && (!uH || tail)) || (tail && !fH) || nH < 2 ||
      nst < 1 || nst > patch_rb_max_stages(tail) || (m & 1) || P.rings != 3)
    return hipErrorInvalidValue;
  int pxc = 0, py0 = 0;
  const unsigned grid = patch_grid(n, m, patch_th(3), line_lo, line_hi, &pxc, &py0);
  if (grid == 0) return hipSuccess;
  const int xm = g_xcd_map ? 1 : 0;
  return patch_dispatch(P.un, P.umask, P.nt != 0, [&](auto U, auto M, auto NTF) {
#define AMG_RB(PRO, TL)                                                                              \
  hipLaunchKernelGGL((patch_rb_kernel<decltype(U)::value, decltype(M)::value, decltype(NTF)::value, PRO, TL>), dim3(grid), \
                     dim3(PATCH_NT), 0, st, (int)n, (int)m, pxc, P.rtype, P.ptab, P.utabd, P.utabi,    \
                     P.nent, P.ntypes, x, f, uH, (int)nH, u_out, r_out, fH, uH_zero, stages, ctab, xm, py0,  \
                     P.tflag)
    if (tail) AMG_RB(false, true);
    else if (prolong) AMG_RB(true, false);
    else AMG_RB(false, false);
#undef AMG_RB
  });
}
int patch_lds_pitch() { return PATCH_EC; }
int patch_max_entries() { return PATCH_MAXTAB; }

template <int WORDS, int UN>
__global__ __launch_bounds__(256) void dict_gs_color_kernel(
    int p0, int count, const uint64_t* __restrict__ codes, const int32_t* __restrict__ rowid,
    const int32_t* __restrict__ doff, const double* __restrict__ dval, int ntab,
    const double* __restrict__ f, double* u, int xcd_map) {
  typedef uint64_t u64x2 __attribute__((ext_vector_type(2)));
  __shared__ DictEntry tab[256];
  const int k = xcd_tile(blockIdx.x, gridDim.x, xcd_map) * 256 + (int)threadIdx.x;
  const int p = p0 + k;
  const int row = k < count ? rowid[p] : -1;
  DictStream<WORDS, 1> s;
  s.live[0] = row >= 0;
  s.cw[0][0] = s.cw[0][1] = ~(uint64_t)0;
  s.ty = 0xFFFFu;
  s.fi[0] = s.xi[0] = 0.0;
  if (s.live[0]) {
    const uint64_t* cp = codes + (int64_t)p * WORDS;
    if (WORDS == 2) {
      const u64x2 t = *reinterpret_cast<const u64x2*>(cp);
      s.cw[0][0] = t.x; s.cw[0][1] = t.y;
    } else {
      s.cw[0][0] = cp[0];
    }
    s.fi[0] = f[row];
    s.xi[0] = u[row];
  }
  dict_stage_table<CSR_GS>(tab, doff, dval, ntab);
  __syncthreads();
  double res[1];
  dict_rows<CSR_GS, WORDS, UN, 1>(s, s.live[0] ? row : 0, tab, u, 1.0, 0, res);
  if (s.live[0]) u[row] = res[0];
}
template <int WORDS, int UN>
__global__ __launch_bounds__(1024) void dict_gs_sweep_kernel(
    int nc, const int32_t* __restrict__ starts, const uint64_t* __restrict__ codes,
    const int32_t* __restrict__ rowid, const int32_t* __restrict__ doff,
    const double* __restrict__ dval, int ntab, const double* __restrict__ f, double* u) {
  typedef uint64_t u64x2 __attribute__((ext_vector_type(2)));
  __shared__ DictEntry tab[256];
  if (threadIdx.x < 256) dict_stage_table<CSR_GS>(tab, doff, dval, ntab);
  __syncthreads();
  for (int phase = 0; phase < 2 * nc; ++phase) {
    const int c = phase < nc ? phase : 2 * nc - 1 - phase;
    const int p0 = starts[c], count = starts[c + 1] - p0;
// ... 5563 lines not shown
```

### algebraic-multigrid_amd/csrc/kernels.hpp

```cpp
#pragma once
#include <hip/hip_runtime_api.h>
#include <stddef.h>
#include <stdint.h>

namespace amg_hip {

enum CsrMode {
  CSR_RESID = 0,
  CSR_JACOBI = 1,
  CSR_SPMV = 2,
  CSR_RSSQ = 3,
  CSR_GS = 4,
  CSR_JACOBI_P = 5,
  CSR_SPMV_ADD = 6,
  CSR_CHEB = 7
};
constexpr int cheb_kernel_mode(bool first, bool last) { return 16 + (first ? 1 : 0) + (last ? 2 : 0); }
struct ChebStep {
  double* d = nullptr;
  double alpha = 0.0, beta = 0.0;
  bool first = true, last = true;
};

hipError_t launch_dict_gs_sweep(int nc, const int32_t* starts_dev, int64_t n_storage, int words, int wmax,
// ... 77 lines not shown
  int hb = 0;
  const double* utd = nullptr;
  const int32_t* uti = nullptr;
};
void set_xcd_mapping(int on);
void set_dict_rows_per_lane(int r);
void set_dict_stencil(int on);
hipError_t launch_dict(int mode, int64_t n, const DictRef& D, const double* x, const double* f,
                       double* out, double omega, int64_t diag_shift, hipStream_t st);
hipError_t launch_dict_cheb(int64_t n, const DictRef& D, const double* x, const double* f, double* out,
                            const ChebStep& c, hipStream_t st);
void dict_kernel_name(int mode, int64_t n, const DictRef& D, const void* f, const void* out,
                      char* buf, size_t cap);
hipError_t launch_dict_gs_color(int64_t p0, int64_t count, int words, int wmax,
                                const uint64_t* codes, const int32_t* rowid, const int32_t* doff,
                                const double* dval, int ntab, const double* f, double* u,
                                hipStream_t st);
hipError_t launch_dict_resid_restrict(int64_t n, const DictRef& D, const double* x,
                                      const double* f, double* r_out, int64_t nH, double* fH,
                                      const double* diagH, double* uH1, double* uH0,
                                      double omega, hipStream_t st);
hipError_t launch_dict_jacobi_prolong(int64_t n, const DictRef& D, const double* x,
                                      const double* f, double* out, double omega, int64_t n_h,
                                      const double* uh_in, double* uh_out, hipStream_t st);
bool dict_pair_ok(int64_t n, const DictRef& D, int hb, const void* a, const void* b, const void* c);
hipError_t launch_dict_pair_down(int64_t n, const DictRef& D, int hb, const double* a,
                                 const double* f, double* u_out, double* r_out, int64_t nH,
                                 double* fH, const double* diagH, double* uH1, double omega,
                                 hipStream_t st);
hipError_t launch_dict_pair_up(int64_t n, const DictRef& D, int hb, const double* a,
                               const double* f, double* u_out, double omega, int64_t n_h,
                               const double* uh_in, double* uh_out, hipStream_t st);
constexpr int AMG_DUO_WINDOWS_LEN = 31;
int duo_windows_host(int hb0, int hb1, int tile_rows, int32_t* out);
int duo_owned_host(int tile, int tile_rows, int32_t* out);
int duo_tile_rows(int hb0);
bool dict_duo_ok(int64_t n0, const DictRef& D0, int hb0, int64_t n1, const DictRef& D1, int hb1, int64_t n2);
hipError_t launch_dict_duo_down(int64_t n0, const DictRef& D0, int hb0, int64_t n1, const DictRef& D1, int hb1,
                                const double* a0, const double* f0, double* u0_out, double* r0_out,
                                double* f1_out, const double* diag1, double* u1_out, double* r1_out, int64_t n2,
                                double* f2_out, const double* diag2, double* v2_out, double omega,
                                hipStream_t st);
hipError_t launch_dict_duo_up(int64_t n0, const DictRef& D0, int hb0, int64_t n1, const DictRef& D1, int hb1,
                              const double* a1, const double* f1, double* u1_out, const double* u0_in,
                              const double* f0, double* u0_out, double omega, int64_t n_h, const double* uh_in,
                              double* uh_out, hipStream_t st);
constexpr int TAIL_LEVELS_MAX = 6;
struct TailLevelRef {
  int n, hbw, words, ntab;
  const uint8_t* rtype;
  const uint64_t* rwords;
  const int32_t* doff;
  const double* dval;
  const double* f;
  double* u;
  double* tmp;
  const double* diag;
};
struct TailRef {
  int nlev;
  TailLevelRef L[TAIL_LEVELS_MAX];
  int nc, wc;
  const double *cf, *cb, *dg;
  double *fc, *uc, *tmpc;
  const double* diagc;
  int n_fine;
  const double* uf_in;
  double* uf_out;
  double omega;
};
bool tail_level_ok(int64_t n, const DictRef& D, int hb);
int tail_max_coarse();
size_t tail_lds_bytes(const TailRef& A);
size_t tail_lds_capacity();
hipError_t launch_tail(const TailRef& A, hipStream_t st);

struct PatchRef {
  const uint8_t* rtype = nullptr;
  const double* ptab = nullptr;
  const double* utabd = nullptr;
  const int32_t* utabi = nullptr;
  int rings = 3;
  const uint8_t* tflag = nullptr;
  int nent = 0, ntypes = 0, un = 0, nt = 0;
  int umask = 0;
  const uint8_t* cflag = nullptr;
  double dHu = 0.0;
};
hipError_t launch_patch_coarse_flags(int64_t n, int64_t m, int rings, int64_t nH, const double* diagH,
                                     double dref, uint8_t* cflag, hipStream_t st);
hipError_t launch_patch_tile_flags(int64_t n, int64_t m, int rings, const uint8_t* rtype, int ntypes,
                                   uint8_t* flag, int64_t* n_tiles, hipStream_t st);
bool patch_geometry_ok(int64_t n, int64_t m);
int patch_un(int longest_row);
int patch_default_umask(int un);
int patch_kind_umask(int un, int umask);
int patch_lds_pitch();
int patch_max_entries();
hipError_t launch_patch_down(bool first, int64_t n, int64_t m, const PatchRef& P, const double* x,
                             const double* f, double* u_out, double* r_out, int64_t nH, double* fH,
                             const double* diagH, double* uH1, double omega, hipStream_t st,
                             int64_t line_lo = 0, int64_t line_hi = -1, bool xf = false);
int patch_tile_lines(int rings);
int patch_leg_rings(bool first);
hipError_t launch_patch_up(int64_t n, int64_t m, const PatchRef& P, const double* x, const double* f,
                           const double* uH, int64_t nH, double* u_out, double omega,
                           hipStream_t st, int64_t line_lo = 0, int64_t line_hi = -1);
int patch_seam_lines();
hipError_t launch_patch_seam_flags(int64_t n, int64_t m, const uint8_t* rtype, int ntypes, uint8_t* flag,
                                   int64_t* n_tiles, hipStream_t st);
hipError_t launch_patch_seam(int64_t n, int64_t m, const PatchRef& P, const double* x, const double* f,
                             const double* uH, int64_t nH, double* u_out, double* fH, double omega,
                             hipStream_t st);
int patch_rb_max_stages(bool tail);
uint32_t patch_rb_stages(const int* colors, int count);
hipError_t launch_patch_rb(bool prolong, bool tail, int64_t n, int64_t m, const PatchRef& P, const double* x,
                           const double* f, const double* uH, int64_t nH, double* u_out, double* r_out,
                           double* fH, double* uH_zero, uint32_t stages, uint32_t ctab, hipStream_t st,
                           int64_t line_lo = 0, int64_t line_hi = -1);
struct MarchRef {
  int m = 0, lines = 0, planes = 0, ntypes = 0, tint = -1, chunk_planes = 0;
  double omega = 1.0, dint = 0.0;
  double wint[6] = {0, 0, 0, 0, 0, 0};
  const double* wtab = nullptr;
  const uint8_t* rtype = nullptr;
  const double* x = nullptr;
  const double* f = nullptr;
  double* out = nullptr;
};
bool march_ok(const MarchRef& A);
hipError_t launch_march(MarchRef A, hipStream_t st);
struct MarchForbid {
  int ntypes = 0;
  uint8_t bits[64] = {};
};
hipError_t launch_march_box_check(int64_t n, int m, int lines, const MarchForbid& F, const uint8_t* rtype,
                                  int32_t* bad, hipStream_t st);
struct StripRef {
  int n = 0, nH = 0, T = 0, H = 0, hbw = 0, nst = 0, ntab = 0;
  uint64_t stages = 0;
  const uint8_t* rtype = nullptr;
  const uint64_t* rwords = nullptr;
  const int32_t* doff = nullptr;
  const double* dval = nullptr;
  const uint8_t* color = nullptr;
  const double* x = nullptr;
  const double* f = nullptr;
  double* u_out = nullptr;
  double* r_out = nullptr;
  const double* uH = nullptr;
  double* fH = nullptr;
  double* uH_zero = nullptr;
};
int strip_window_max();
hipError_t launch_mc_strip(bool prolong, bool tail, StripRef A, const DictRef& D, hipStream_t st);
hipError_t launch_linear_prolong_to(int64_t n_h, int64_t n_H, const double* uH,
                                    const double* uh_in, double* uh_out, hipStream_t st);
hipError_t launch_sell_jacobi_prolong(int64_t n, int idx16, const int64_t* soff,
                                      const void* scol, const double* sval, const double* u,
                                      const double* uH, int64_t nH, const double* f, double* out,
                                      double omega, hipStream_t st);
hipError_t launch_jacobi_from_zero(int64_t n, const double* diag, const double* f, double* out,
                                   double omega, hipStream_t st);
hipError_t launch_sell_gs_color(int64_t n_storage, int max_width, const int64_t* soff,
                                const int32_t* scol, const double* sval, const int32_t* rowid,
                                int64_t row0, int64_t count, const double* f, double* u,
                                hipStream_t st);

hipError_t launch_linear_restrict(int64_t n_h, int64_t n_H, const double* r, double* fH,
                                  double* uH_zero, hipStream_t st);
hipError_t launch_linear_prolong_add(int64_t n_h, int64_t n_H, const double* uH,
                                     double* uh, hipStream_t st);
hipError_t launch_tensor_restrict(int dim, const int64_t dims[3], uint32_t mask, uint32_t sides, uint32_t periodic,
                                  const double* r, double* fH, double* uH_zero, hipStream_t st);
hipError_t launch_tensor_prolong_add(int dim, const int64_t dims[3], uint32_t mask, uint32_t sides, uint32_t periodic,
                                     const double* uH, double* uh, hipStream_t st);
hipError_t launch_axis_restrict(int dim, const int64_t dims[3], int axis, const double* W, const double* r,
                                double* fH, double* uH_zero, hipStream_t st);
hipError_t launch_axis_prolong_add(int dim, const int64_t dims[3], int axis, const double* W, const double* uH,
                                   double* uh, hipStream_t st);
hipError_t launch_zero_strided(double* x, int64_t stride, int count, hipStream_t st);
hipError_t launch_add_inplace(int64_t n, const double* x, double* y, hipStream_t st);
hipError_t launch_sum(int64_t n, const double* x, double* out, double* scratch, int square,
                      hipStream_t st);

hipError_t launch_dot(int64_t n, const double* x, const double* y, double* out, double* scratch,
                      hipStream_t st);
hipError_t launch_pcg_update_xr(int64_t n, const double* num, const double* den, double* x, double* r,
                                const double* p, const double* q, hipStream_t st);
hipError_t launch_pcg_update_p(int64_t n, const double* num, const double* den, double* p,
                               const double* z, hipStream_t st);
hipError_t launch_center(int64_t n, const double* sum, const double* src, double* dst, hipStream_t st);
hipError_t launch_center_dot(int64_t n, const double* sum, double* z, const double* r, double* out,
// ... 166 lines not shown
```

### algebraic-multigrid_amd/csrc/solver.cpp

```cpp
#include <cstddef>
#include <hip/hip_runtime.h>

#include <algorithm>
#include <cmath>
#include <chrono>
#include <cstdio>
#include <cstdlib>
#include <cstring>
#include <functional>
#include <map>
#include <memory>
#include <string>
#include <thread>
#include <vector>

#include <dlfcn.h>

#include "../../include/amg_hip.h"
#include "capture_once.hpp"
#include "host_setup.hpp"
#include "kernels.hpp"

using namespace amg_hip;
#ifdef AMG_PATCH_STAMPS
namespace amg_hip { hipError_t debug_set_patch_stamps(unsigned long long* p); }
#endif

namespace {

thread_local std::string g_err;

amg_hip_status fail(amg_hip_status st, const std::string& msg) {
  g_err = msg;
  return st;
}

#define HIP_TRY(expr)                                                          \
  do {                                                                         \
    hipError_t _e = (expr);                                                    \
    if (_e != hipSuccess)                                                      \
      return fail(_e == hipErrorOutOfMemory ? AMG_HIP_ENOMEM : AMG_HIP_EHIP,   \
                  std::string(#expr) + ": " + hipGetErrorString(_e));          \
  } while (0)
#define AMG_TRY(expr)                                                          \
  do {                                                                         \
    const amg_hip_status _s = (expr);                                          \
    if (_s != AMG_HIP_OK) return _s;                                           \
  } while (0)

int host_threads() {
  unsigned h = std::thread::hardware_concurrency();
  if (h == 0) h = 1;
  return (int)std::min(h, 16u);
}

struct DevMem {
  void* p = nullptr;
  size_t bytes = 0;
  DevMem() = default;
  DevMem(const DevMem&) = delete;
  DevMem& operator=(const DevMem&) = delete;
  DevMem(DevMem&& o) noexcept : p(o.p), bytes(o.bytes) { o.p = nullptr; o.bytes = 0; }
  DevMem& operator=(DevMem&& o) noexcept {
    if (this != &o) { release(); p = o.p; bytes = o.bytes; o.p = nullptr; o.bytes = 0; }
    return *this;
  }
  ~DevMem() { release(); }
  void release() {
    if (p) (void)hipFree(p);
    p = nullptr;
    bytes = 0;
  }
  hipError_t alloc(size_t n) {
    release();
    bytes = n;
    return hipMalloc(&p, n + 64);
  }
  template <class T> T* as() const { return reinterpret_cast<T*>(p); }
};

template <class T>
hipError_t upload(DevMem& m, const T* src, size_t count) {
  hipError_t e = m.alloc(count * sizeof(T));
  if (e != hipSuccess) return e;
  if (count == 0) return hipSuccess;
  return hipMemcpy(m.p, src, count * sizeof(T), hipMemcpyHostToDevice);
}

struct DevCsr {
  int64_t n_rows = 0, n_cols = 0, nnz = 0;
  int max_block_nnz = 0, max_row_nnz = 0;
  DevMem ptr, idx, val;
  const int32_t* rowptr() const { return ptr.as<int32_t>(); }
  const int32_t* col() const { return idx.as<int32_t>(); }
  const double* v() const { return val.as<double>(); }
};

hipError_t download_csr(int64_t n, const int32_t* ptr, const int32_t* idx, const double* val, hipStream_t st,
                        Sparse* H) {
  H->n_outer = H->n_inner = n;
  H->ptr.resize((size_t)n + 1);
  hipError_t e = hipMemcpyAsync(H->ptr.data(), ptr, sizeof(int32_t) * H->ptr.size(), hipMemcpyDeviceToHost, st);
  if (e == hipSuccess) e = hipStreamSynchronize(st);
  if (e != hipSuccess) return e;
  const size_t nnz = (size_t)H->ptr.back();
  H->idx.resize(nnz);
  H->val.resize(nnz);
  if (nnz == 0) return hipSuccess;
// ... 99 lines not shown
                                  nullptr, nullptr, ovf.as<int32_t>(), nullptr)) != hipSuccess)
    return e;
  int32_t over = 0;
  if ((e = hipMemcpy(&over, ovf.p, sizeof(int32_t), hipMemcpyDeviceToHost)) != hipSuccess) return e;
  if (over) return hipSuccess;
  if ((e = AH->ptr.alloc(sizeof(int32_t) * (n_H + 1))) != hipSuccess) return e;
  if ((e = launch_exclusive_scan(n_H, cnt.as<int32_t>(), AH->ptr.as<int32_t>(), bsum.as<int64_t>(),
                                 total.as<int64_t>(), nullptr)) != hipSuccess)
    return e;
  int64_t nnz = 0;
  if ((e = hipMemcpy(&nnz, total.p, sizeof(int64_t), hipMemcpyDeviceToHost)) != hipSuccess) return e;
  if (nnz >= ((int64_t)1 << 31) - 1) return hipErrorInvalidValue;
  if ((e = AH->idx.alloc(sizeof(int32_t) * std::max<int64_t>(nnz, 1))) != hipSuccess) return e;
  if ((e = AH->val.alloc(sizeof(double) * std::max<int64_t>(nnz, 1))) != hipSuccess) return e;
  if ((e = launch_tensor_galerkin(true, dim, dims, mask, sides, periodic, A.rowptr(), A.col(), A.v(), nullptr, AH->ptr.as<int32_t>(),
                                  AH->idx.as<int32_t>(), AH->val.as<double>(), ovf.as<int32_t>(), nullptr)) != hipSuccess)
    return e;
  AH->n_rows = AH->n_cols = n_H;
  AH->nnz = nnz;
  *ok = true;
  return hipSuccess;
}

hipError_t device_spgemm(const DevCsr& A, const DevCsr& B, DevCsr* C, bool* ok) {
  *ok = false;
  const int64_t n = A.n_rows;
  hipError_t e;
  DevMem cnt, bsum, total, ovf;
  if ((e = cnt.alloc(sizeof(int32_t) * (n + 1))) != hipSuccess) return e;
  if ((e = bsum.alloc(sizeof(int64_t) * ((n + 1023) / 1024 + 1))) != hipSuccess) return e;
  if ((e = total.alloc(sizeof(int64_t))) != hipSuccess) return e;
  if ((e = ovf.alloc(sizeof(int32_t))) != hipSuccess) return e;
  if ((e = hipMemset(ovf.p, 0, sizeof(int32_t))) != hipSuccess) return e;
  if ((e = launch_spgemm(false, n, A.rowptr(), A.col(), A.v(), B.rowptr(), B.col(), B.v(),
                         cnt.as<int32_t>(), nullptr, nullptr, nullptr, ovf.as<int32_t>(), nullptr)) != hipSuccess)
    return e;
  int32_t over = 0;
  if ((e = hipMemcpy(&over, ovf.p, sizeof(int32_t), hipMemcpyDeviceToHost)) != hipSuccess) return e;
  if (over) return hipSuccess;
  if ((e = C->ptr.alloc(sizeof(int32_t) * (n + 1))) != hipSuccess) return e;
  if ((e = launch_exclusive_scan(n, cnt.as<int32_t>(), C->ptr.as<int32_t>(), bsum.as<int64_t>(),
                                 total.as<int64_t>(), nullptr)) != hipSuccess)
    return e;
  int64_t nnz = 0;
  if ((e = hipMemcpy(&nnz, total.p, sizeof(int64_t), hipMemcpyDeviceToHost)) != hipSuccess) return e;
  if (nnz >= ((int64_t)1 << 31) - 1) return hipSuccess;
  if ((e = C->idx.alloc(sizeof(int32_t) * std::max<int64_t>(nnz, 1))) != hipSuccess) return e;
  if ((e = C->val.alloc(sizeof(double) * std::max<int64_t>(nnz, 1))) != hipSuccess) return e;
  if ((e = launch_spgemm(true, n, A.rowptr(), A.col(), A.v(), B.rowptr(), B.col(), B.v(), nullptr,
                         C->ptr.as<int32_t>(), C->idx.as<int32_t>(), C->val.as<double>(),
                         ovf.as<int32_t>(), nullptr)) != hipSuccess)
    return e;
  C->n_rows = n;
  C->n_cols = B.n_cols;
  C->nnz = nnz;
  *ok = true;
  return hipSuccess;
}
hipError_t device_galerkin_generic(const DevCsr& A, const DevCsr& P, const DevCsr& R, DevCsr* AH,
                                   Sparse* host, bool* ok) {
  DevCsr AP;
  hipError_t e = device_spgemm(A, P, &AP, ok);
  if (e != hipSuccess || !*ok) return e;
  e = device_spgemm(R, AP, AH, ok);
  if (e != hipSuccess || !*ok) return e;
  const int64_t n_H = AH->n_rows, nnz = AH->nnz;
  host->n_outer = host->n_inner = n_H;
  host->ptr.resize(n_H + 1);
  host->idx.resize(nnz);
  host->val.resize(nnz);
  if ((e = hipMemcpy(host->ptr.data(), AH->ptr.p, sizeof(int32_t) * (n_H + 1), hipMemcpyDeviceToHost)) != hipSuccess) return e;
  if (nnz > 0) {
    if ((e = hipMemcpy(host->idx.data(), AH->idx.p, sizeof(int32_t) * nnz, hipMemcpyDeviceToHost)) != hipSuccess) return e;
    if ((e = hipMemcpy(host->val.data(), AH->val.p, sizeof(double) * nnz, hipMemcpyDeviceToHost)) != hipSuccess) return e;
  }
  return hipSuccess;
}

int g_patch_tile_flags = 1;
int g_axis_stencil = 1;
int g_patch_xf = 1;
int g_patch_tall = 1;
int g_patch_seam = 1;

struct DevMat {
  bool sell = false;
  int64_t n_rows = 0, nnz = 0;
  DevCsr csr;
  int max_width = 0;
  int64_t slots = 0;
  int idx16 = 0;
  DevMem soff, scol, sval;
  bool dict = false;
  int dict_words = 0, dict_wmax = 0, dict_ntab = 0, dict_nt = 0;
  int64_t dict_shift = 0;
  int dict_hb = 0;
  bool dict_typed = false;
  DevMem dcodes, doff, dval, drtype, drwords;
  DevMem dutd, duti;
  DevMem dmarch;
  int march_m = 0, march_M = 0, march_ntypes = 0, march_tint = -1;
  double march_wint[6] = {0, 0, 0, 0, 0, 0}, march_dint = 0.0;
  int64_t scan_gap = 0, scan_far = 0;
  int scan_new = 99;
  bool patch = false;
  int64_t patch_m = 0;
  int patch_un = 0, patch_ntypes = 0, patch_umask = 0;
  DevMem patch_tab, patch_utabd, patch_utabi, patch_flags, patch_flags2, patch_flags5;
  DevMem patch_cflags;
  int patch_crings = 3;
  double patch_dH = 0.0;
  double patch_cfrac = 0.0;
  PatchRef patch_ref(int rings = 3) const {
    PatchRef P;
    P.rings = rings;
    P.rtype = drtype.as<uint8_t>();
    P.tflag = g_patch_tile_flags ? (rings == 2 ? patch_flags2 : (rings == 5 ? patch_flags5 : patch_flags)).as<uint8_t>()
                                 : nullptr;
    P.cflag = g_patch_tile_flags && rings == patch_crings ? patch_cflags.as<uint8_t>() : nullptr;
    P.dHu = patch_dH;
    P.ptab = patch_tab.as<double>();
    P.utabd = patch_utabd.as<double>();
    P.utabi = patch_utabi.as<int32_t>();
    P.ntypes = patch_ntypes;
    P.un = patch_un;
    P.umask = patch_umask;
    P.nent = patch_ntypes * patch_un;
    P.nt = dict_nt;
    return P;
  }
  DictRef dict_ref() const {
    DictRef D;
    D.words = dict_words; D.wmax = dict_wmax; D.nt = dict_nt; D.ntab = dict_ntab;
    D.codes = dcodes.as<uint64_t>();
    D.rtype = dict_typed ? drtype.as<uint8_t>() : nullptr;
    D.rwords = dict_typed ? drwords.as<uint64_t>() : nullptr;
    D.doff = doff.as<int32_t>();
    D.dval = dval.as<double>();
    D.scan_new = scan_new;
    D.hb = dict_hb;
    D.utd = (dict_typed && dutd.p) ? dutd.as<double>() : nullptr;
    D.uti = (dict_typed && duti.p) ? duti.as<int32_t>() : nullptr;
    return D;
  }
};

int g_row_types = 1;

int g_index16 = 1;
int g_nontemporal = 1;

int g_default_layout = AMG_HIP_LAYOUT_AUTO;

Sparse without_exact_zeros(const Sparse& M) {
  Sparse R;
  R.n_outer = M.n_outer;
  R.n_inner = M.n_inner;
  R.ptr.assign(M.n_outer + 1, 0);
  R.idx.reserve(M.idx.size());
  R.val.reserve(M.val.size());
  for (int64_t o = 0; o < M.n_outer; ++o) {
    for (int32_t p = M.ptr[o]; p < M.ptr[o + 1]; ++p)
      if (M.val[p] != 0.0) {
        R.idx.push_back(M.idx[p]);
        R.val.push_back(M.val[p]);
      }
    R.ptr[o + 1] = (int32_t)R.idx.size();
  }
  return R;
}

hipError_t upload_mat(const Sparse& M, int layout, DevMat* D, int64_t diag_shift, bool allow16);

bool build_patch_table(const DictMat& T, int64_t n, int64_t* m_out, int* un_out, int* ntypes_out,
                       std::vector<double>* tab) {
  if (T.rwords.empty() || T.max_width > 9 || T.doff.empty()) return false;
  int64_t omax = 0;
  for (int32_t o : T.doff) omax = std::max<int64_t>(omax, o < 0 ? -(int64_t)o : o);
  int ntypes = 0;
  for (int t = 0; t < 255; ++t) {
    bool used = false;
    for (int k = 0; k < T.words; ++k) used = used || T.rwords[(size_t)t * T.words + k] != ~(uint64_t)0;
    if (used) ntypes = t + 1;
  }
  const int un = patch_un(T.max_width);
  if (ntypes < 1 || (ntypes + 1) * un > patch_max_entries()) return false;
  const int pitch = patch_lds_pitch();
  for (int64_t m : {omax, omax - 1}) {
    if (!patch_geometry_ok(n, m)) continue;
    bool ok = true;
    std::vector<double> out((size_t)ntypes * un * 4, 0.0);
    for (int t = 0; t < ntypes && ok; ++t)
      for (int e = 0; e < un; ++e) {
        double* q = &out[((size_t)t * un + e) * 4];
        const int code = e < 8 * T.words ? (int)((T.rwords[(size_t)t * T.words + e / 8] >> (8 * (e % 8))) & 0xFF) : 0xFF;
        if (code == 0xFF) { q[3] = -1.0e9; continue; }
        if (code >= (int)T.doff.size()) { ok = false; break; }
        const int64_t o = T.doff[code];
        const double v = T.dval[code];
        int64_t dj = 0;
        if (o > m / 2) dj = 1;
// ... 124 lines not shown
        tint = t;
        pm = r[5].first;
        pM = r[6].first;
      }
    }
    if (tint >= 0 && last < 64 && pM < ((int64_t)1 << 30) && n % pM == 0) {
      const int64_t P[6] = {-pM, -pm, -1, 1, pm, pM};
      std::vector<double> wt((size_t)(last + 1) * 8, 0.0);
      bool ok = true;
      for (int t = 0; t <= last && ok; ++t) {
        double diag = 0.0;
        for (const auto& e : rows[(size_t)t]) {
          if (e.first == 0) {
            diag = diag + e.second;
            continue;
          }
          int at = -1;
          for (int u = 0; u < 6; ++u)
            if (P[u] == e.first) at = u;
          if (at < 0) { ok = false; break; }
          wt[(size_t)t * 8 + at] = e.second;
        }
        wt[(size_t)t * 8 + 6] = diag;
      }
      if (ok) {
        MarchForbid F;
        F.ntypes = last + 1;
        for (int t = 0; t <= last; ++t)
          for (const auto& e : rows[(size_t)t])
            F.bits[t] |= (uint8_t)((e.first == -1 ? 1 : 0) | (e.first == 1 ? 2 : 0) | (e.first == -pm ? 4 : 0) |
                                   (e.first == pm ? 8 : 0));
        DevMem dbad;
        int32_t bad = 0;
        if ((e = dbad.alloc(sizeof(int32_t))) != hipSuccess) return e;
        if ((e = hipMemset(dbad.p, 0, sizeof(int32_t))) != hipSuccess) return e;
        if ((e = launch_march_box_check(n, (int)pm, (int)(pM / pm), F, D->drtype.as<uint8_t>(),
                                        dbad.as<int32_t>(), nullptr)) != hipSuccess)
          return e;
        if ((e = hipMemcpy(&bad, dbad.p, sizeof(int32_t), hipMemcpyDeviceToHost)) != hipSuccess) return e;
        ok = bad == 0;
      }
      if (ok) {
        if ((e = upload(D->dmarch, wt.data(), wt.size())) != hipSuccess) return e;
        D->march_m = (int)pm;
        D->march_M = (int)pM;
        D->march_ntypes = last + 1;
        D->march_tint = tint;
        for (int u = 0; u < 6; ++u) D->march_wint[u] = wt[(size_t)tint * 8 + u];
        D->march_dint = wt[(size_t)tint * 8 + 6];
      }
    }
  }
  D->patch = false;
  if (D->dict_typed && diag_shift == 0) {
    std::vector<double> tab;
    if (build_patch_table(T, n, &D->patch_m, &D->patch_un, &D->patch_ntypes, &tab)) {
      if ((e = upload(D->patch_tab, tab.data(), tab.size())) != hipSuccess) return e;
      const int un = D->patch_un, nty = D->patch_ntypes, pitch = patch_lds_pitch();
      std::vector<double> ud((size_t)(nty + 1) * 19, 0.0);
      std::vector<int32_t> ui((size_t)(nty + 1) * 2, 0);
      for (int t = 0; t < nty; ++t) {
        double diag = 0.0;
        uint32_t rm = 0;
        for (int k = 0; k < un; ++k) {
          const double* q = &tab[((size_t)t * un + k) * 4];
          if (!(q[3] > -1.0e8)) continue;
          const int lo = (int)q[3];
          const int dj = lo > pitch / 2 ? 1 : (lo < -pitch / 2 ? -1 : 0), di = lo - dj * pitch;
          const int slot = (dj + 1) * 3 + (di + 1);
          ud[(size_t)t * 19 + slot] = q[0];
          ud[(size_t)t * 19 + 9 + slot] = q[2];
          diag += q[1];
          rm |= 1u << slot;
        }
        ud[(size_t)t * 19 + 18] = diag;
        ui[(size_t)t * 2] = (int32_t)rm;
        ui[(size_t)t * 2 + 1] = (rm & 0x145u) ? 1 : 0;
      }
      if ((e = upload(D->patch_utabd, ud.data(), ud.size())) != hipSuccess) return e;
      if ((e = upload(D->patch_utabi, ui.data(), ui.size())) != hipSuccess) return e;
      int64_t tiles = 0;
      for (int rings = 2; rings <= 3; ++rings) {
        DevMem& F = rings == 2 ? D->patch_flags2 : D->patch_flags;
        if ((e = launch_patch_tile_flags(n, D->patch_m, rings, nullptr, nty, nullptr, &tiles, nullptr)) != hipSuccess) return e;
        if ((e = F.alloc(((size_t)tiles + 3) & ~(size_t)3)) != hipSuccess) return e;
        if ((e = hipMemset(F.p, 0, F.bytes)) != hipSuccess) return e;
        if ((e = launch_patch_tile_flags(n, D->patch_m, rings, D->drtype.as<uint8_t>(), nty, F.as<uint8_t>(),
                                         nullptr, nullptr)) != hipSuccess) return e;
      }
      if (patch_un(un) == 5) {
        int64_t t5 = 0;
        if ((e = launch_patch_seam_flags(n, D->patch_m, nullptr, nty, nullptr, &t5, nullptr)) == hipSuccess) {
          if ((e = D->patch_flags5.alloc(((size_t)t5 + 3) & ~(size_t)3)) != hipSuccess) return e;
          if ((e = hipMemset(D->patch_flags5.p, 0, D->patch_flags5.bytes)) != hipSuccess) return e;
          if ((e = launch_patch_seam_flags(n, D->patch_m, D->drtype.as<uint8_t>(), nty, D->patch_flags5.as<uint8_t>(),
                                           nullptr, nullptr)) != hipSuccess) return e;
        }
      }
      if ((e = hipDeviceSynchronize()) != hipSuccess) return e;
      {
        std::vector<uint8_t> fl((size_t)tiles);
        if ((e = hipMemcpy(fl.data(), D->patch_flags.p, fl.size(), hipMemcpyDeviceToHost)) != hipSuccess) return e;
        std::vector<int64_t> cnt(256, 0);
        for (uint8_t f : fl) ++cnt[f];
        int best = -1;
        for (int t = 0; t < nty; ++t)
          if (cnt[t] > 0 && (best < 0 || cnt[t] > cnt[best])) best = t;
        D->patch_umask = best >= 0 ? ui[(size_t)best * 2] : patch_default_umask(patch_un(un));
      }
      D->patch = true;
    }
  }
  return hipSuccess;
}

hipError_t upload_mat_pruned(const Sparse& M, int layout, bool prune, DevMat* D,
                             int64_t diag_shift = 0) {
  bool any = false;
  if (prune)
    for (double v : M.val)
      if (v == 0.0) { any = true; break; }
  if (!any) return upload_mat(M, layout, D, diag_shift, true);
  return upload_mat(without_exact_zeros(M), layout, D, diag_shift, true);
}

hipError_t upload_mat(const Sparse& M, int layout, DevMat* D, int64_t diag_shift, bool allow16);
hipError_t upload_mat(const Sparse& M, int layout, DevMat* D) {
  return upload_mat(M, layout, D, 0, true);
}
hipError_t upload_mat(const Sparse& M, int layout, DevMat* D, int64_t diag_shift, bool allow16) {
  D->n_rows = M.n_outer;
  D->nnz = M.nnz();
  D->dict = false;
  if ((layout == AMG_HIP_LAYOUT_AUTO || layout == AMG_HIP_LAYOUT_DICT) && allow16 &&
      M.n_outer < ((int64_t)1 << 31) - 512) {
    DictMat T;
    if (to_dict(M, diag_shift, &T)) {
      hipError_t e;
      D->dict_typed = g_row_types != 0 && !T.rtype.empty();
      if (D->dict_typed) {
        if ((e = upload(D->drtype, T.rtype.data(), T.rtype.size())) != hipSuccess) return e;
      } else {
        if ((e = upload(D->dcodes, T.codes.data(), T.codes.size())) != hipSuccess) return e;
      }
      return finish_dict(T, M.n_outer, diag_shift, D);
    }
    if (layout == AMG_HIP_LAYOUT_DICT) layout = AMG_HIP_LAYOUT_SELL;
  }
  if (layout == AMG_HIP_LAYOUT_DICT) layout = AMG_HIP_LAYOUT_SELL;
  bool sell = layout == AMG_HIP_LAYOUT_SELL;
  Sell64 S;
  if (layout != AMG_HIP_LAYOUT_CSR && M.n_outer < ((int64_t)1 << 31) - 512) {
    to_sell64(M, &S);
    if (layout == AMG_HIP_LAYOUT_AUTO) sell = (double)S.slots() <= 1.25 * (double)M.nnz() + 4096.0;
  } else {
    sell = false;
  }
  D->sell = sell;
  if (!sell) return upload_csr(M, &D->csr);
  D->max_width = S.max_width;
  D->slots = S.slots();
  hipError_t e;
  if ((e = upload(D->soff, S.soff.data(), S.soff.size())) != hipSuccess) return e;
  bool fits = allow16 && g_index16 != 0;
  std::vector<int16_t> c16;
  if (fits) {
    c16.assign(S.col.size(), (int16_t)-32768);
    const int64_t np = (int64_t)S.soff.size() - 1;
    for (int64_t p = 0; p < np && fits; ++p) {
      const int64_t w = (S.soff[p + 1] - S.soff[p]) / 64;
      for (int64_t j = 0; j < w && fits; ++j)
        for (int64_t l = 0; l < 64; ++l) {
          const int64_t at = S.soff[p] + j * 64 + l;
          const int32_t c = S.col[at];
          if (c < 0) continue;
          const int64_t d = (int64_t)c - (p * 64 + l + diag_shift);
          if (d < -32767 || d > 32767) { fits = false; break; }
          c16[at] = (int16_t)d;
        }
// ... 3582 lines not shown
  }
  return AMG_HIP_OK;
}

amg_hip_status enqueue_f32_vcycle(amg_hip_solver* s, bool dry) {
  const int nl = (int)s->lv.size();
  amg_hip_status r;
  F32_DO(launch_zero_f32(s->lv[0].n, s->f32.lv[0].u.as<float>(), s->stream));
  s->facct(4.0 * (double)s->lv[0].n);
  for (int l = 0; l + 1 < nl; ++l) {
    if ((r = enqueue_f32_smooth(s, l, dry)) != AMG_HIP_OK) return r;
    if ((r = enqueue_f32_residual(s, l, dry)) != AMG_HIP_OK) return r;
    if ((r = enqueue_f32_restrict(s, l, dry)) != AMG_HIP_OK) return r;
  }
  if ((r = enqueue_f32_coarse(s, dry)) != AMG_HIP_OK) return r;
  for (int l = nl - 2; l >= 0; --l) {
    if ((r = enqueue_f32_prolong(s, l, dry)) != AMG_HIP_OK) return r;
    if ((r = enqueue_f32_smooth(s, l, dry, true)) != AMG_HIP_OK) return r;
  }
  return AMG_HIP_OK;
}
#undef F32_DO

amg_hip_status f32_apply(amg_hip_solver* s, const double* v, double* z) {
  F32& F = s->f32;
  const int64_t n = s->lv[0].n;
  HIP_TRY(launch_to_f32(n, v, F.lv[0].f.as<float>(), s->stream));
  if (!s->opt.use_graph) {
    amg_hip_status r = enqueue_f32_vcycle(s, false);
    if (r != AMG_HIP_OK) return r;
  } else {
    if (!F.exec) AMG_TRY(capture_once(s->stream, [s] { return enqueue_f32_vcycle(s, false); }, &F.graph, &F.exec));
    HIP_TRY(hipGraphLaunch(F.exec, s->stream));
  }
  HIP_TRY(launch_to_f64(n, F.lv[0].u.as<float>(), z, s->stream));
  return AMG_HIP_OK;
}

}

namespace amg_hip {
amg_hip_status fail_status(amg_hip_status st, const std::string& msg) { return fail(st, msg); }
}

extern "C" {

const char* amg_hip_last_error(void) { return g_err.c_str(); }

static_assert(offsetof(amg_hip_options, cyclic_lines) == 68 && offsetof(amg_hip_options, stream) == 72 &&
                  offsetof(amg_hip_options, singular) == 108 && sizeof(amg_hip_options) == 112,
              "amg_hip_options: the layout of the earlier releases must not move");
void amg_hip_default_options(amg_hip_options* o) {
  if (!o) return;
  std::memset(o, 0, sizeof(*o));
  o->smoother = AMG_HIP_SM_SPGS;
  o->smoother_iters = 1;
  o->omega = 1.0;
  o->device = -1;
  o->use_graph = 1;
  o->stencil_transfers = 1;
  o->layout = g_default_layout;
  o->keep_structural_zeros = 0;
  o->no_fusion = 0;
  o->fuse_prolong = 0;
  o->fast_coarse_solve = 0;
  o->stream = nullptr;
  o->window = 0;
  o->cheb_degree = 2;
  o->cheb_lower = 0.3;
  o->cheb_upper = 1.0;
}

void amg_hip_set_index16(int32_t on) { g_index16 = on ? 1 : 0; }
void amg_hip_set_nontemporal(int32_t on) { g_nontemporal = on ? 1 : 0; }
void amg_hip_set_xcd_mapping(int32_t on) { set_xcd_mapping(on); }
void amg_hip_set_row_types(int32_t on) { g_row_types = on ? 1 : 0; }
void amg_hip_set_dict_rows(int32_t rows_per_lane) { set_dict_rows_per_lane(rows_per_lane); }
void amg_hip_set_dict_stencil(int32_t on) { set_dict_stencil(on); }
void amg_hip_set_patch_tile_flags(int32_t on) { g_patch_tile_flags = on ? 1 : 0; }
void amg_hip_set_axis_stencil(int32_t on) { g_axis_stencil = on ? 1 : 0; }
void amg_hip_set_patch_xf(int32_t on) { g_patch_xf = on ? 1 : 0; }
void amg_hip_set_patch_tall(int32_t on) { g_patch_tall = on ? 1 : 0; }
void amg_hip_set_patch_seam(int32_t on) { g_patch_seam = on ? 1 : 0; }
void amg_hip_set_band_chain(int32_t on) { g_no_band_chain = on ? 0 : 1; }
void amg_hip_set_tail_fusion(int32_t on) { g_tail_fusion = on ? 1 : 0; }
void amg_hip_set_pair_duo(int32_t on) { g_pair_duo = on ? 1 : 0; }
int32_t amg_hip_pair_duo_partner(const amg_hip_solver* s, int32_t level) {
  if (!s || level < 0 || level >= (int32_t)s->lv.size()) return -1;
  const LegForm up = current_plan(s).lv[(size_t)level].up;
  return up == LEG_DUO_FINE ? level + 1 : (up == LEG_DUO_COARSE ? level - 1 : -1);
}
int32_t amg_hip_duo_windows(int32_t hb_l, int32_t hb_l1, int32_t tile_rows, int32_t* out) {
  return duo_windows_host(hb_l, hb_l1, tile_rows, out);
}
int32_t amg_hip_duo_owned(int32_t tile, int32_t tile_rows, int32_t* out) { return duo_owned_host(tile, tile_rows, out); }
int32_t amg_hip_duo_tile_rows(int32_t hb_l) { return hb_l < 0 ? -1 : duo_tile_rows(hb_l); }
void amg_hip_set_periodic_device_setup(int32_t on) { g_periodic_device_setup = on ? 1 : 0; }
void amg_hip_set_f32_lines(int32_t on) { g_f32_lines = on ? 1 : 0; }
void amg_hip_set_f32_dict(int32_t on) { g_f32_dict = on ? 1 : 0; }
void amg_hip_set_block_lines(int32_t on) { g_block_lines = on ? 1 : 0; }
void amg_hip_set_patch_min_rows(int64_t rows) { g_patch_min_rows = rows < 0 ? INT64_MAX : rows; }

void amg_hip_set_default_layout(int32_t layout) {
  if (layout >= AMG_HIP_LAYOUT_AUTO && layout <= AMG_HIP_LAYOUT_DICT) g_default_layout = layout;
}

int amg_hip_device_count(void) {
  int n = 0;
  if (hipGetDeviceCount(&n) != hipSuccess) return 0;
  return n;
}

amg_hip_status amg_hip_create(int64_t n, const int32_t* colptr, const int32_t* rowind,
                              const double* val, const double* b, int32_t n_levels,
                              const amg_hip_options* opts, amg_hip_solver** out) {
  return build_solver(n, colptr, rowind, val, b, n_levels, opts, out);
}

amg_hip_status amg_hip_create_custom(int64_t n, const int32_t* colptr, const int32_t* rowind,
                                     const double* val, const double* b, int32_t n_levels,
                                     const int32_t* const* P_colptr,
                                     const int32_t* const* P_rowind, const double* const* P_val,
                                     const int32_t* const* R_colptr,
                                     const int32_t* const* R_rowind, const double* const* R_val,
                                     const amg_hip_options* opts, amg_hip_solver** out) {
  if (n_levels > 1 && (!P_colptr || !P_rowind || !P_val || !R_colptr || !R_rowind || !R_val))
    return fail(AMG_HIP_EINVAL, "custom transfer operator arrays are null");
  HierarchySpec h;
  h.Pc = P_colptr, h.Pr = P_rowind, h.Pv = P_val;
  h.Rc = R_colptr, h.Rr = R_rowind, h.Rv = R_val;
  return build_solver(n, colptr, rowind, val, b, n_levels, opts, out, h);
}

amg_hip_status amg_hip_create_rs(int64_t n, const int32_t* colptr, const int32_t* rowind,
                                 const double* val, const double* b, int32_t max_levels,
                                 double theta, int64_t min_coarse, const amg_hip_options* opts,
                                 amg_hip_solver** out) {
  if (!(theta >= 0.0 && theta <= 1.0)) return fail(AMG_HIP_EINVAL, "`theta` must be in [0, 1]");
  if (min_coarse < 1) return fail(AMG_HIP_EINVAL, "`min_coarse` must be at least 1");
  HierarchySpec h;
  h.rs_theta = theta;
  h.rs_min_coarse = min_coarse;
  return build_solver(n, colptr, rowind, val, b, max_levels, opts, out, h);
}

static std::string tensor_dims_error(int32_t dim, const int64_t* dims) {
  if (dim != 2 && dim != 3) return "`dim` must be 2 or 3";
  if (!dims) return "`dims` is null";
  if (dims[0] < 1 || dims[1] < 1 || dims[2] < 1) return "every entry of `dims` must be at least 1";
  if (dim == 2 && dims[2] != 1) return "`dims[2]` must be 1 when `dim` is 2";
  if (dims[0] >= ((int64_t)1 << 31) / dims[1] / dims[2]) return "the grid has 2^31 points or more";
  return "";
}

static std::string window_error(const std::string& who, const char* kind) {
  return who + "window solvers (opt.window) coarsen the flat index; a " + kind + "-coarsening hierarchy is not sharded";
}
static std::string grid_size_error(int64_t n, const int64_t* dims, bool figures) {
  if (n == dims[0] * dims[1] * dims[2]) return "";
  const std::string grid = std::to_string(dims[0]) + " x " + std::to_string(dims[1]) + " x " +
                           std::to_string(dims[2]) + " grid";
  return "`n`" + (figures ? " = " + std::to_string(n) : "") + " is not the " + (figures ? grid : "number of points") +
         " of `dims`";
}
static amg_hip_status tensor_grid_args(const std::string& who, int64_t n, int32_t dim, const int64_t* dims,
                                       int32_t window, const char* kind) {
// ... 512 lines not shown
    sb.levels = 0;
    return r;
  }
  s->reset_seam_graphs();
  if (s->graph_ready) {
    (void)hipGraphExecDestroy(s->graph_exec);
    (void)hipGraphDestroy(s->graph);
    s->graph_exec = nullptr;
    s->graph = nullptr;
    s->graph_ready = false;
  }
  *info = pl;
  info->pitch0 = m0;
  info->gather_pitch = mk;
  info->gather_rows = G.n;
  info->u0 = s->lv[0].u.as<double>();
  info->f_gather = G.f.as<double>();
  return AMG_HIP_OK;
}

amg_hip_status amg_hip_slab_run(amg_hip_solver* s, int32_t part) {
  if (!s || part < CYCLE_SLAB_DOWN || part > CYCLE_SLAB_UP)
    return fail(AMG_HIP_EINVAL, "amg_hip_slab_run: part is 1 (down-legs), 2 (replicated rest) or 3 (up-legs)");
  Slab& sb = s->slab;
  if (sb.levels < 1) return fail(AMG_HIP_EINVAL, "amg_hip_slab_run: amg_hip_slab_setup has not succeeded");
  amg_hip_status r = set_device(s);
  if (r != AMG_HIP_OK) return r;
  if (!s->opt.use_graph) return enqueue_vcycle(s, part);
  const int gi = part - 1;
  if (!sb.exec[gi])
    AMG_TRY(capture_once(s->stream, [s, part] { return enqueue_vcycle(s, part); }, &sb.graph[gi], &sb.exec[gi]));
  HIP_TRY(hipGraphLaunch(sb.exec[gi], s->stream));
  return AMG_HIP_OK;
}

amg_hip_status amg_hip_window_setup(amg_hip_solver* s, const int64_t* down_lo, const int64_t* down_hi,
                                    const int64_t* up_lo, const int64_t* up_hi) {
  if (!s) return fail(AMG_HIP_EINVAL, "null solver");
  if (!s->opt.window) return fail(AMG_HIP_EINVAL, "amg_hip_window_setup: not a window solver (opt.window)");
  if ((down_lo || down_hi || up_lo || up_hi) && !(down_lo && down_hi && up_lo && up_hi))
    return fail(AMG_HIP_EINVAL, "amg_hip_window_setup: give all four range arrays or none");
  amg_hip_status r = set_device(s);
  if (r != AMG_HIP_OK) return r;
  HIP_TRY(hipStreamSynchronize(s->stream));
  const int k = (int)s->lv.size() - 1;
  Slab& sb = s->slab;
  sb.reset_graphs();
  s->plan_kept = false;
  sb.levels = k;
  sb.rank = 0;
  sb.world = 1;
  sb.down_lo.assign(k, 0);
  sb.down_hi.assign(k, -1);
  sb.up_lo.assign(k, 0);
  sb.up_hi.assign(k, -1);
  if (down_lo)
    for (int l = 0; l < k; ++l) {
      if (down_lo[l] < 0 || up_lo[l] < 0 || down_hi[l] < down_lo[l] || up_hi[l] < up_lo[l])
        return fail(AMG_HIP_EINVAL, "amg_hip_window_setup: bad line range");
      sb.down_lo[l] = down_lo[l];
      sb.down_hi[l] = down_hi[l];
      sb.up_lo[l] = up_lo[l];
      sb.up_hi[l] = up_hi[l];
    }
  return AMG_HIP_OK;
}

amg_hip_status amg_hip_window_run(amg_hip_solver* s, int32_t part) {
  if (!s || (part != CYCLE_SLAB_DOWN && part != CYCLE_SLAB_UP))
    return fail(AMG_HIP_EINVAL, "amg_hip_window_run: part is 1 (down-legs) or 3 (up-legs)");
  if (!s->opt.window) return fail(AMG_HIP_EINVAL, "amg_hip_window_run: not a window solver (opt.window)");
  if (s->slab.levels < 1) {
    amg_hip_status r = amg_hip_window_setup(s, nullptr, nullptr, nullptr, nullptr);
    if (r != AMG_HIP_OK) return r;
  }
  return amg_hip_slab_run(s, part);
}

#ifdef AMG_PATCH_STAMPS
amg_hip_status amg_hip_debug_patch_stamps(void* dev_ptr) {
  HIP_TRY(debug_set_patch_stamps((unsigned long long*)dev_ptr));
  return AMG_HIP_OK;
}
#endif

amg_hip_status amg_hip_get_stream(amg_hip_solver* s, void** stream) {
  if (!s || !stream) return fail(AMG_HIP_EINVAL, "bad argument");
  if (s->opt.host_only) return fail(AMG_HIP_EINVAL, "solver was created with host_only = 1: no device state");
  *stream = (void*)s->stream;
  return AMG_HIP_OK;
}

static DevMem* level_vec(amg_hip_solver* s, int32_t level, int32_t which) {
  if (!s || level < 0 || level >= (int32_t)s->lv.size()) return nullptr;
  Level& L = s->lv[level];
  if (which == 0) return &resting(s, current_plan(s), level);
  return which == 1 ? &L.f : (which == 2 ? &L.r : nullptr);
}
struct DuoView {
  Level* lv[2] = {nullptr, nullptr};
  DuoView(amg_hip_solver* s, int level) {
    const int nl = (int)s->lv.size();
    const CyclePlan P = current_plan(s);
    for (int q = 0; q < 2; ++q)
      if (level + q < nl && P.lv[(size_t)level + q].rests_tmp) {
        lv[q] = &s->lv[level + q];
        std::swap(lv[q]->u, lv[q]->tmp);
      }
  }
  ~DuoView() {
    for (Level* L : lv)
      if (L) std::swap(L->u, L->tmp);
  }
  DuoView(const DuoView&) = delete;
  DuoView& operator=(const DuoView&) = delete;
};

amg_hip_status amg_hip_vec_dev_ptr(amg_hip_solver* s, int32_t level, int32_t which, void** ptr, int64_t* n) {
  if (!s || !ptr || level < 0 || level >= (int32_t)s->lv.size() || which < 0 || which > 2)
    return fail(AMG_HIP_EINVAL, "bad argument");
  if (s->opt.host_only) return fail(AMG_HIP_EINVAL, "solver was created with host_only = 1: no device state");
  Level& L = s->lv[level];
  *ptr = level_vec(s, level, which)->p;
  if (n) *n = L.n;
  return AMG_HIP_OK;
}

amg_hip_status amg_hip_sync(amg_hip_solver* s) {
  if (!s) return fail(AMG_HIP_EINVAL, "null solver");
  amg_hip_status r = set_device(s);
  if (r != AMG_HIP_OK) return r;
  HIP_TRY(hipStreamSynchronize(s->stream));
  return AMG_HIP_OK;
}

amg_hip_status amg_hip_copy_vec_dev(amg_hip_solver* s, int32_t level, int32_t which,
                                    void* dev_ptr, int32_t to_solver) {
  if (!s || !dev_ptr || level < 0 || level >= (int32_t)s->lv.size() || which < 0 || which > 2)
    return fail(AMG_HIP_EINVAL, "bad argument");
  amg_hip_status r = set_device(s);
  if (r != AMG_HIP_OK) return r;
  Level& L = s->lv[level];
  void* v = level_vec(s, level, which)->p;
  if (to_solver)
    HIP_TRY(hipMemcpyAsync(v, dev_ptr, sizeof(double) * L.n, hipMemcpyDeviceToDevice, s->stream));
  else
    HIP_TRY(hipMemcpyAsync(dev_ptr, v, sizeof(double) * L.n, hipMemcpyDeviceToDevice, s->stream));
  return AMG_HIP_OK;
}

amg_hip_status amg_hip_zero_vec(amg_hip_solver* s, int32_t level, int32_t which) {
  if (!s || level < 0 || level >= (int32_t)s->lv.size() || which < 0 || which > 2)
    return fail(AMG_HIP_EINVAL, "bad argument");
  amg_hip_status r = set_device(s);
  if (r != AMG_HIP_OK) return r;
  Level& L = s->lv[level];
  void* v = level_vec(s, level, which)->p;
  HIP_TRY(hipMemsetAsync(v, 0, sizeof(double) * L.n, s->stream));
  return AMG_HIP_OK;
}

amg_hip_status amg_hip_level_op(amg_hip_solver* s, int32_t level, int32_t op) {
  if (!s) return fail(AMG_HIP_EINVAL, "null solver");
  const int nl = (int)s->lv.size();
  if (level < 0 || level >= nl) return fail(AMG_HIP_EINVAL, "level out of range");
  amg_hip_status r = set_device(s);
// ... 570 lines not shown
  auto restore = [&]() -> amg_hip_status {
    if (mc && !mc_patch)
      HIP_TRY(hipMemcpyAsync(L.u.p, L.r.p, sizeof(double) * L.n, hipMemcpyDeviceToDevice, s->stream));
    return AMG_HIP_OK;
  };
  return time_launches(s->stream, n_launches, avg_ms, min_ms, restore, [&]() -> amg_hip_status {
    if (mc_patch) {
      int nd = 0;
      const std::vector<McLaunch> plan = mc_plan(s, 0, &nd);
      HIP_TRY(launch_patch_rb(false, false, L.n, L.A_rows.patch_m, L.A_rows.patch_ref(), L.u.as<double>(),
                              L.f.as<double>(), nullptr, s->lv[1].n, L.tmp.as<double>(), nullptr, nullptr,
                              nullptr, plan[0].stages, (uint32_t)L.mc_ctab, s->stream));
    } else if (mc) {
      if (L.mc_dict)
        HIP_TRY(launch_dict_gs_color(L.mc_start[0], L.mc_start[1] - L.mc_start[0], L.mc_words, L.mc_wmax,
                                     L.mc_codes.as<uint64_t>(), L.mc_rowid.as<int32_t>(),
                                     L.mc_doff.as<int32_t>(), L.mc_dval.as<double>(), L.mc_ntab,
                                     L.f.as<double>(), L.u.as<double>(), s->stream));
      else
        HIP_TRY(launch_sell_gs_color(L.mc_mat.n_rows, L.mc_mat.max_width, L.mc_mat.soff.as<int64_t>(),
                                     L.mc_mat.scol.as<int32_t>(), L.mc_mat.sval.as<double>(),
                                     L.mc_rowid.as<int32_t>(), L.mc_start[0], L.mc_start[1] - L.mc_start[0],
                                     L.f.as<double>(), L.u.as<double>(), s->stream));
    } else if (march) {
      HIP_TRY(launch_march(MR, s->stream));
    } else if (patch) {
      Level& C = s->lv[1];
      HIP_TRY(launch_patch_down(true, L.n, A.patch_m, A.patch_ref(), L.u.as<double>(),
                                L.f.as<double>(), L.tmp.as<double>(), nullptr, C.n, C.f.as<double>(),
                                C.diag.as<double>(), P.lv[0].xf_out ? nullptr : C.tmp.as<double>(),
                                s->opt.omega, s->stream,
                                slab ? s->slab.down_lo[0] : 0, slab ? s->slab.down_hi[0] : -1));
    } else {
      HIP_TRY(launch_mat(CSR_JACOBI, A, L.u.as<double>(), L.f.as<double>(), L.tmp.as<double>(),
                         s->opt.omega, s->stream));
    }
    return AMG_HIP_OK;
  });
}

amg_hip_status amg_hip_cycle_must_move(amg_hip_solver* s, int32_t part, double* bytes) {
  if (!s || !bytes || part < 0 || part > 4) return fail(AMG_HIP_EINVAL, "bad argument");
  if (s->opt.host_only) return fail(AMG_HIP_EINVAL, "host_only solver has no device cycle");
  if (part == 4) {
    if (!current_plan(s).seam) return amg_hip_cycle_must_move(s, CYCLE_ALL, bytes);
    if (s->must_move[4] == 0.0) {
      amg_hip_status r = set_device(s);
      if (r != AMG_HIP_OK) return r;
      if (!s->opt.use_graph) return fail(AMG_HIP_EINVAL, "amg_hip_cycle_must_move: run two V-cycles in one call first");
      const int gi = 2;
      s->seam_piece = SEAM_CYCLE;
      s->seam_src = 0;
      r = s->seam_exec[gi] ? AMG_HIP_OK
                           : capture_once(s->stream, [s] { return enqueue_vcycle(s); }, &s->seam_graph[gi], &s->seam_exec[gi]);
      s->seam_piece = SEAM_OFF;
      if (r != AMG_HIP_OK) return r;
    }
    *bytes = s->must_move[4];
    return AMG_HIP_OK;
  }
  if (part == CYCLE_ALL && s->must_move[0] == 0.0 && !s->opt.window) {
    amg_hip_status r = set_device(s);
    if (r != AMG_HIP_OK) return r;
    if (s->opt.use_graph) {
      if ((r = ensure_graph(s)) != AMG_HIP_OK) return r;
    } else {
      return fail(AMG_HIP_EINVAL, "amg_hip_cycle_must_move: run a V-cycle first");
    }
  }
  *bytes = s->must_move[part];
  return AMG_HIP_OK;
}

int32_t amg_hip_patch_leg_lines(const amg_hip_solver* s, int32_t level, int32_t leg) {
  if (!s || s->opt.host_only || level < 0 || level >= (int32_t)s->lv.size() || leg < 0 || leg > 2) return 0;
  const CyclePlan P = current_plan(s);
  const LegForm form = P.lv[(size_t)level].up;
  if (leg == 2) return (level == 0 && P.seam) ? patch_seam_lines() : 0;
  if (form == LEG_MC_PATCH) return patch_tile_lines(3);
  if (form != LEG_PATCH) return 0;
  return patch_tile_lines(patch_rings(s, leg == 0 && level == 0));
}

amg_hip_status amg_hip_fine_sweep_info(const amg_hip_solver* s, char* name, int32_t name_cap,
                                       int32_t* sweeps_per_launch, double* bytes_per_launch) {
  if (!s || !name || name_cap < 32) return fail(AMG_HIP_EINVAL, "bad argument");
  if (s->opt.smoother == AMG_HIP_SM_LINE_JACOBI || s->opt.smoother == AMG_HIP_SM_LINE_ALT)
    return fail(AMG_HIP_EUNSUPPORTED, "fine_sweep_info: a line-smoother sweep is not one launch");
  if (s->opt.host_only) return fail(AMG_HIP_EINVAL, "host_only solver has no device matrices");
  const Level& L = s->lv[0];
  const DevMat& A = L.A_cols();
  const CyclePlan P = current_plan(s);
  const LevelPlan& Q = P.lv[0];
  int32_t lay = 0;
  int64_t mat = 0;
  layout_of(A, &lay, &mat);
  int sweeps = 1;
  double bytes = 12.0 * (double)L.nnz_struct + 28.0 * (double)L.n;
  if (s->opt.smoother == AMG_HIP_SM_CHEBYSHEV) {
    ChebStep c;
    cheb_profiled_step(s, &c);
    const int mode = cheb_kernel_mode(c.first, c.last);
    const DevMat& R = L.A_rows;
    layout_of(R, &lay, &mat);
    if (R.dict) {
      dict_kernel_name(mode, R.n_rows, R.dict_ref(), L.f.p, L.tmp.p, name, (size_t)name_cap);
    } else if (R.sell) {
      std::snprintf(name, (size_t)name_cap, "sell_kernel<%d, %s, %s>", mode, (R.idx16 & 1) ? "true" : "false",
                    (R.idx16 & 2) ? "true" : "false");
    } else {
      std::snprintf(name, (size_t)name_cap, "csr_stage_kernel<%d>", mode);
    }
    bytes = (double)mat + 24.0 * (double)L.n + (c.first ? 0.0 : 8.0 * L.n) + (c.last ? 0.0 : 8.0 * L.n);
  } else if (s->opt.smoother == AMG_HIP_SM_MULTICOLOR_GS) {
    if (Q.down == LEG_MC_PATCH) {
      std::snprintf(name, (size_t)name_cap, "patch_rb_kernel<%d, %d, %s, false, false>", patch_un(A.patch_un),
                    patch_kind_umask(A.patch_un, A.patch_umask), A.dict_nt ? "true" : "false");
      bytes = 25.0 * (double)L.n;
    } else {
      std::snprintf(name, (size_t)name_cap, "%s", L.mc_dict ? "dict_gs_color_kernel" : "sell_kernel<5>");
      const double rows = (double)(L.mc_start.size() > 1 ? L.mc_start[1] - L.mc_start[0] : L.n);
      bytes = L.mc_dict ? rows * (8.0 * L.mc_words + 4.0 + 16.0)
                        : rows / (double)L.n * (12.0 * (double)L.nnz_struct + 28.0 * (double)L.n);
    }
  } else if (Q.down == LEG_PATCH) {
    std::snprintf(name, (size_t)name_cap, "patch_down_kernel<%d, %d, true, %s, false, 3>", patch_un(A.patch_un),
                  patch_kind_umask(A.patch_un, A.patch_umask), A.dict_nt ? "true" : "false");
    sweeps = 2;
    bytes = 25.0 * (double)L.n + (Q.xf_out ? 8.0 : 24.0 - 8.0 * A.patch_cfrac) * (double)s->lv[1].n;
    if (s->slab.levels > 0 && s->slab.world > 1) {
      const int64_t th = patch_tile_lines(patch_rings(s, true));
      const int64_t l0 = s->slab.down_lo[0] / th * th;
      const int64_t l1 = std::min<int64_t>(s->slab.lines, (s->slab.down_hi[0] + th - 1) / th * th);
      bytes *= (double)(l1 - l0) / (double)s->slab.lines;
    }
  } else if (Q.march) {
    std::snprintf(name, (size_t)name_cap, "march_kernel");
    sweeps = 2;
    bytes = (double)mat + 24.0 * (double)L.n;
  } else if (A.dict) {
    dict_kernel_name(CSR_JACOBI, A.n_rows, A.dict_ref(), L.f.p, L.tmp.p, name, (size_t)name_cap);
    bytes = (double)mat + 24.0 * (double)L.n;
  } else if (A.sell) {
    std::snprintf(name, (size_t)name_cap, "sell_kernel<1, %s, %s>", (A.idx16 & 1) ? "true" : "false",
                  (A.idx16 & 2) ? "true" : "false");
  } else {
    std::snprintf(name, (size_t)name_cap, "csr_stage_kernel<1>");
  }
  if (sweeps_per_launch) *sweeps_per_launch = sweeps;
  if (bytes_per_launch) *bytes_per_launch = bytes;
  return AMG_HIP_OK;
}

amg_hip_status amg_hip_residual(int64_t n, const int32_t* colptr, const int32_t* rowind,
                                const double* val, const double* u, const double* f,
                                double* r) {
  amg_hip_status st = need_device();
  if (st != AMG_HIP_OK) return st;
  if (n <= 0 || !colptr || !rowind || !val || !u || !f || !r)
    return fail(AMG_HIP_EINVAL, "bad argument");
  Sparse A = from_raw(n, n, colptr, rowind, val);
  std::string v = validate(A, "A");
  if (!v.empty()) return fail(AMG_HIP_EINVAL, v);
  Sparse Ar = transpose(A);
  DevMat D;
  DevMem du, df, dr;
// ... 1029 lines not shown
```

### include/amg_hip.h

```cpp
#ifndef AMG_HIP_H
#define AMG_HIP_H

#include <stddef.h>
#include <stdint.h>

#ifdef __cplusplus
extern "C" {
#endif

typedef enum {
  AMG_HIP_OK = 0,
  AMG_HIP_EINVAL = 1,
  AMG_HIP_EHIP = 2,
  AMG_HIP_ENOMEM = 3,
  AMG_HIP_EUNSUPPORTED = 4,
  AMG_HIP_ECOMM = 5
} amg_hip_status;

typedef enum {
  AMG_HIP_SM_SPGS = 0,
  AMG_HIP_SM_REF_JACOBI = 1,
  AMG_HIP_SM_SOR = 2,
  AMG_HIP_SM_JACOBI = 3,
  AMG_HIP_SM_MULTICOLOR_GS = 4,
  AMG_HIP_SM_CHEBYSHEV = 5,
  AMG_HIP_SM_LINE_JACOBI = 6,
  AMG_HIP_SM_LINE_ALT = 7
} amg_hip_smoother;

typedef enum {
  AMG_HIP_LAYOUT_AUTO = 0,
  AMG_HIP_LAYOUT_CSR = 1,
  AMG_HIP_LAYOUT_SELL = 2,
  AMG_HIP_LAYOUT_DICT = 3
} amg_hip_layout;

typedef struct {
  int32_t smoother;
  int32_t smoother_iters;
  double omega;
  int32_t device;
  int32_t use_graph;
  int32_t stencil_transfers;
  int32_t layout;
  int32_t host_only;
  int32_t keep_structural_zeros;
  int32_t no_fusion;
  int32_t fuse_prolong;
  int32_t fast_coarse_solve;
  int32_t host_galerkin;
  int32_t keep_residual;
  int32_t exact_coarse_solve;
  int32_t exact_gs;
  int32_t cyclic_lines;
  void* stream;
  int32_t window;
  int32_t cheb_degree;
  double cheb_lower;
  double cheb_upper;
  int32_t natural_sides;
  int32_t singular;
} amg_hip_options;

typedef struct amg_hip_solver amg_hip_solver;

const char* amg_hip_last_error(void);
void amg_hip_default_options(amg_hip_options* o);

void amg_hip_set_default_layout(int32_t layout);

void amg_hip_set_index16(int32_t on);
void amg_hip_set_nontemporal(int32_t on);
void amg_hip_set_xcd_mapping(int32_t on);
void amg_hip_set_row_types(int32_t on);
void amg_hip_set_dict_rows(int32_t rows_per_lane);
void amg_hip_set_dict_stencil(int32_t on);
void amg_hip_set_patch_min_rows(int64_t rows);

void amg_hip_set_patch_tile_flags(int32_t on);
void amg_hip_set_patch_xf(int32_t on);
void amg_hip_set_patch_tall(int32_t on);
void amg_hip_set_patch_seam(int32_t on);
void amg_hip_set_band_chain(int32_t on);

void amg_hip_set_tail_fusion(int32_t on);

void amg_hip_set_pair_duo(int32_t on);
int32_t amg_hip_pair_duo_partner(const amg_hip_solver* s, int32_t level);
int32_t amg_hip_duo_windows(int32_t hb_l, int32_t hb_l1, int32_t tile_rows, int32_t* out);
int32_t amg_hip_duo_owned(int32_t tile, int32_t tile_rows, int32_t* out);
int32_t amg_hip_duo_tile_rows(int32_t hb_l);

void amg_hip_set_periodic_device_setup(int32_t on);

void amg_hip_set_f32_lines(int32_t on);

void amg_hip_set_f32_dict(int32_t on);

void amg_hip_set_block_lines(int32_t on);

int amg_hip_device_count(void);

amg_hip_status amg_hip_create(int64_t n, const int32_t* colptr,
                              const int32_t* rowind, const double* val,
                              const double* b, int32_t n_levels,
                              const amg_hip_options* opts,
                              amg_hip_solver** out);

amg_hip_status amg_hip_create_custom(int64_t n, const int32_t* colptr,
                                     const int32_t* rowind, const double* val,
                                     const double* b, int32_t n_levels,
                                     const int32_t* const* P_colptr,
                                     const int32_t* const* P_rowind,
                                     const double* const* P_val,
                                     const int32_t* const* R_colptr,
                                     const int32_t* const* R_rowind,
                                     const double* const* R_val,
                                     const amg_hip_options* opts,
                                     amg_hip_solver** out);

amg_hip_status amg_hip_create_rs(int64_t n, const int32_t* colptr, const int32_t* rowind,
                                 const double* val, const double* b, int32_t max_levels,
                                 double theta, int64_t min_coarse, const amg_hip_options* opts,
                                 amg_hip_solver** out);

amg_hip_status amg_hip_create_tensor(int64_t n, const int32_t* colptr, const int32_t* rowind,
                                     const double* val, const double* b, int32_t dim,
                                     const int64_t* dims , int32_t n_levels,
                                     const amg_hip_options* opts, amg_hip_solver** out);
amg_hip_status amg_hip_create_tensor_semi(int64_t n, const int32_t* colptr, const int32_t* rowind,
                                          const double* val, const double* b, int32_t dim,
                                          const int64_t* dims , int32_t n_levels,
                                          const int32_t* axis_masks ,
                                          double theta, int64_t min_coarse,
                                          const amg_hip_options* opts, amg_hip_solver** out);
amg_hip_status amg_hip_create_tensor_opdep(int64_t n, const int32_t* colptr, const int32_t* rowind,
                                           const double* val, const double* b, int32_t dim,
                                           const int64_t* dims , int32_t n_levels,
                                           const int32_t* axis_masks ,
                                           int64_t min_coarse, const amg_hip_options* opts, amg_hip_solver** out);
void amg_hip_set_axis_stencil(int32_t on);
amg_hip_status amg_hip_get_axis_weights(const amg_hip_solver* s, int32_t level, double* W);
amg_hip_status amg_hip_get_natural_sides(const amg_hip_solver* s, int32_t* mask);
amg_hip_status amg_hip_create_tensor_periodic(int64_t n, const int32_t* colptr, const int32_t* rowind,
                                              const double* val, const double* b, int32_t dim,
                                              const int64_t* dims , int32_t periodic_axes,
                                              int32_t n_levels,
                                              const int32_t* axis_masks ,
                                              const amg_hip_options* opts, amg_hip_solver** out);
amg_hip_status amg_hip_get_periodic_axes(const amg_hip_solver* s, int32_t* mask);
amg_hip_status amg_hip_get_level_axes(const amg_hip_solver* s, int32_t level, int32_t* axis_mask);
amg_hip_status amg_hip_tensor_axis_strength(int64_t n, const int32_t* colptr, const int32_t* rowind,
                                            const double* val, int32_t dim, const int64_t* dims ,
                                            double* w );
amg_hip_status amg_hip_get_level_dims(const amg_hip_solver* s, int32_t level, int64_t* dims );
amg_hip_status amg_hip_level_transfer_kind(const amg_hip_solver* s, int32_t level, int32_t* kind);

amg_hip_status amg_hip_create_poisson(int32_t dim, int64_t n, int32_t n_levels,
                                      const amg_hip_options* opts, amg_hip_solver** out);

amg_hip_status amg_hip_create_poisson_tensor(int32_t dim, int64_t n, int32_t n_levels,
                                             const amg_hip_options* opts, amg_hip_solver** out);
amg_hip_status amg_hip_create_tensor_dev(int64_t n, const int32_t* rowptr_dev, const int32_t* col_dev,
                                         const double* val_dev, const double* b_dev, int32_t dim,
// ... 72 lines not shown
  int64_t send_prev_cnt, recv_prev_cnt, send_next_cnt, recv_next_cnt;
  int64_t own_k_off, own_k_cnt, block_k, uk_off;
} amg_hip_window_plan;
amg_hip_status amg_hip_window_cycle(amg_hip_solver* w, amg_hip_solver* t, amg_hip_comm* c,
                                    const amg_hip_window_plan* p);

amg_hip_status amg_hip_solve(amg_hip_solver* s, double tol, int64_t every,
                             int64_t n_iters, int64_t* iters, double* last_rss,
                             int32_t* converged);

amg_hip_status amg_hip_apply(amg_hip_solver* s, const double* v_dev, double* z_dev);
amg_hip_status amg_hip_pcg(amg_hip_solver* s, double rtol, int64_t max_iters, int64_t* iters,
                           double* relres);
amg_hip_status amg_hip_set_mean_projection(amg_hip_solver* s, int32_t on);
amg_hip_status amg_hip_get_mean_projection(const amg_hip_solver* s, int32_t* on);
amg_hip_status amg_hip_center_vec(amg_hip_solver* s, int32_t level, int32_t which );

amg_hip_status amg_hip_rss(amg_hip_solver* s, double* out);

amg_hip_status amg_hip_block_vcycles(amg_hip_solver* s, int32_t k, const double* F, double* U,
                                     int32_t n_cycles);
amg_hip_status amg_hip_block_rss(amg_hip_solver* s, int32_t k, const double* F, const double* U,
                                 double* out );
amg_hip_status amg_hip_block_pcg(amg_hip_solver* s, int32_t k, const double* B, double* X,
                                 double rtol, int64_t max_iters,
                                 int64_t* iters , double* relres );
amg_hip_status amg_hip_block_must_move(amg_hip_solver* s, int32_t k, double* bytes);

amg_hip_status amg_hip_apply_f32(amg_hip_solver* s, const double* v_dev, double* z_dev);
amg_hip_status amg_hip_pcg_mixed(amg_hip_solver* s, double rtol, int64_t max_iters, int64_t* iters,
                                 double* relres);
amg_hip_status amg_hip_f32_must_move(amg_hip_solver* s, double* bytes);
amg_hip_status amg_hip_f32_get_vec(amg_hip_solver* s, int32_t level, int32_t which, float* out_host);
amg_hip_status amg_hip_f32_set_vec(amg_hip_solver* s, int32_t level, int32_t which, const float* in_host);
amg_hip_status amg_hip_f32_level_op(amg_hip_solver* s, int32_t level, int32_t op);
amg_hip_status amg_hip_f32_line_subsweep(amg_hip_solver* s, int32_t level, int32_t d, int32_t reverse);
amg_hip_status amg_hip_f32_line_factors(amg_hip_solver* s, int32_t level, float* dl, float* ip, float* cp);

int32_t amg_hip_n_levels(const amg_hip_solver* s);
int64_t amg_hip_get_n_dofs(const amg_hip_solver* s, int32_t level);
int64_t amg_hip_get_level_nnz(const amg_hip_solver* s, int32_t level);
amg_hip_status amg_hip_get_level_matrix(const amg_hip_solver* s, int32_t level,
                                        int32_t* colptr, int32_t* rowind,
                                        double* val);
int64_t amg_hip_get_transfer_nnz(const amg_hip_solver* s, int32_t level, int32_t which);
amg_hip_status amg_hip_get_transfer(const amg_hip_solver* s, int32_t level,
                                    int32_t which, int32_t* colptr,
                                    int32_t* rowind, double* val);
amg_hip_status amg_hip_get_vec(amg_hip_solver* s, int32_t level, int32_t which,
                               double* out);
amg_hip_status amg_hip_set_vec(amg_hip_solver* s, int32_t level, int32_t which,
                               const double* in);
amg_hip_status amg_hip_copy_vec_dev(amg_hip_solver* s, int32_t level, int32_t which,
                                    void* dev_ptr, int32_t to_solver);
amg_hip_status amg_hip_zero_vec(amg_hip_solver* s, int32_t level, int32_t which);

amg_hip_status amg_hip_level_layout(const amg_hip_solver* s, int32_t level, int32_t* layout,
                                    int64_t* matrix_stream_bytes);

int64_t amg_hip_coarse_halfbw(const amg_hip_solver* s);
int32_t amg_hip_coarse_solve_kind(const amg_hip_solver* s);
amg_hip_status amg_hip_get_colors(const amg_hip_solver* s, int32_t level,
                                  int32_t* color, int32_t* n_colors);

amg_hip_status amg_hip_level_op(amg_hip_solver* s, int32_t level, int32_t op);

amg_hip_status amg_hip_cheb_bounds(const amg_hip_solver* s, int32_t level, double* lo, double* hi);

amg_hip_status amg_hip_line_stride(const amg_hip_solver* s, int32_t level, int64_t* stride);

amg_hip_status amg_hip_line_directions(const amg_hip_solver* s, int32_t level, int32_t* n_dir,
                                       int64_t strides[3]);

amg_hip_status amg_hip_line_cyclic(const amg_hip_solver* s, int32_t level, int32_t* axis_mask);

amg_hip_status amg_hip_cycle_bytes(const amg_hip_solver* s, double* cycle_bytes,
                                   double* fine_sweep_bytes);

amg_hip_status amg_hip_cycle_must_move(amg_hip_solver* s, int32_t part, double* bytes);

amg_hip_status amg_hip_profile_fine_sweep(amg_hip_solver* s, int32_t n_launches,
                                          double* avg_ms, double* min_ms);
int32_t amg_hip_patch_leg_lines(const amg_hip_solver* s, int32_t level, int32_t leg);
amg_hip_status amg_hip_fine_sweep_info(const amg_hip_solver* s, char* name, int32_t name_cap,
                                       int32_t* sweeps_per_launch, double* bytes_per_launch);

amg_hip_status amg_hip_smooth(int32_t kind, int64_t n, const int32_t* colptr,
                              const int32_t* rowind, const double* val,
                              double* u, const double* b, double omega,
                              double tol, int64_t every, int64_t n_iters,
                              int64_t* iters, int32_t* converged);
amg_hip_status amg_hip_smooth_chebyshev(int64_t n, const int32_t* colptr, const int32_t* rowind,
                                        const double* val, double* u, const double* b,
                                        int32_t degree, double lower, double upper,
                                        int64_t n_iters);
amg_hip_status amg_hip_smooth_line(int64_t n, const int32_t* colptr, const int32_t* rowind,
                                   const double* val, int64_t stride, double omega, int64_t iters,
                                   double* u, const double* f);
amg_hip_status amg_hip_smooth_line_alt(int64_t n, const int32_t* colptr, const int32_t* rowind,
                                       const double* val, int32_t dim, const int64_t* dims, double omega,
                                       int64_t iters, int32_t reverse, double* u, const double* f);
amg_hip_status amg_hip_smooth_line_alt_per(int64_t n, const int32_t* colptr, const int32_t* rowind,
                                           const double* val, int32_t dim, const int64_t* dims,
                                           int32_t periodic_axes, double omega, int64_t iters,
                                           int32_t reverse, double* u, const double* f);
amg_hip_status amg_hip_spgs_sweep(int32_t dir, int64_t n, const int32_t* colptr,
                                  const int32_t* rowind, const double* val,
                                  double* u, const double* b);
amg_hip_status amg_hip_residual(int64_t n, const int32_t* colptr,
                                const int32_t* rowind, const double* val,
                                const double* u, const double* f, double* r);
amg_hip_status amg_hip_spmv(int64_t rows, int64_t cols, const int32_t* colptr,
                            const int32_t* rowind, const double* val,
                            const double* v, double* out);
amg_hip_status amg_hip_linear_restrict(int64_t n_h, int64_t n_H, const double* r,
                                       double* f_H);
amg_hip_status amg_hip_linear_prolong_add(int64_t n_h, int64_t n_H,
                                          const double* u_H, double* u_h);
amg_hip_status amg_hip_tensor_restrict(int32_t dim, const int64_t* dims_h , const double* r,
                                       double* f_H);
amg_hip_status amg_hip_tensor_prolong_add(int32_t dim, const int64_t* dims_h ,
                                          const double* u_H, double* u_h);
amg_hip_status amg_hip_tensor_restrict_axes(int32_t dim, const int64_t* dims_h , int32_t axis_mask,
                                            const double* r, double* f_H);
amg_hip_status amg_hip_tensor_prolong_add_axes(int32_t dim, const int64_t* dims_h , int32_t axis_mask,
                                               const double* u_H, double* u_h);
amg_hip_status amg_hip_axis_restrict(int32_t dim, const int64_t* dims_h , int32_t axis, const double* W,
                                     const double* r, double* f_H);
amg_hip_status amg_hip_axis_prolong_add(int32_t dim, const int64_t* dims_h , int32_t axis, const double* W,
                                        const double* u_H, double* u_h);
amg_hip_status amg_hip_tensor_restrict_bc(int32_t dim, const int64_t* dims_h , int32_t axis_mask,
                                          int32_t natural_sides, const double* r, double* f_H);
amg_hip_status amg_hip_tensor_prolong_add_bc(int32_t dim, const int64_t* dims_h , int32_t axis_mask,
                                             int32_t natural_sides, const double* u_H, double* u_h);
amg_hip_status amg_hip_tensor_restrict_per(int32_t dim, const int64_t* dims_h , int32_t axis_mask,
                                           int32_t natural_sides, int32_t periodic_axes, const double* r,
                                           double* f_H);
amg_hip_status amg_hip_tensor_prolong_add_per(int32_t dim, const int64_t* dims_h , int32_t axis_mask,
                                              int32_t natural_sides, int32_t periodic_axes, const double* u_H,
                                              double* u_h);
amg_hip_status amg_hip_rss_host(int64_t n, const int32_t* colptr,
                                const int32_t* rowind, const double* val,
                                const double* u, const double* b, double* out);
amg_hip_status amg_hip_coarse_solve(int64_t n, const int32_t* colptr,
                                    const int32_t* rowind, const double* val,
                                    const double* f, double* x, int64_t* halfbw);

amg_hip_status amg_hip_coarse_solve_fast(int64_t n, const int32_t* colptr,
                                         const int32_t* rowind, const double* val,
                                         const double* f, double* x, int64_t* halfbw,
                                         int32_t* partition_rows);

int64_t amg_hip_laplacian(int32_t dim, int64_t n, int32_t* colptr,
                          int32_t* rowind, double* val);
amg_hip_status amg_hip_rhs(int32_t dim, int64_t n, double* b);

amg_hip_status amg_hip_dict_probe(int64_t nrows, int64_t ncols, const int32_t* rowptr,
                                  const int32_t* col, const double* val, int64_t diag_shift,
                                  int32_t* n_pairs, int32_t* n_row_types, int32_t* words);
amg_hip_status amg_hip_csr_shape(int64_t nrows, const int32_t* rowptr_host,
                                 int32_t* max_block_nnz, int32_t* max_row_nnz);
amg_hip_status amg_hip_dev_residual(int64_t nrows, int64_t nnz, int32_t max_block_nnz,
                                    int32_t max_row_nnz, const int32_t* rowptr,
                                    const int32_t* col, const double* val,
                                    const double* u, const double* f, double* r,
                                    void* stream);
// ... 89 lines not shown
```

Baseline: 1594 V-cycles/s.

## Add column-typed patch tiles with per-lane row type and compact slot tables

New measurement: 1705 V-cycles/s, median of 6. +7.0%, better.

```diff
diff --git a/algebraic-multigrid_amd/amg_ctypes.py b/algebraic-multigrid_amd/amg_ctypes.py
--- a/algebraic-multigrid_amd/amg_ctypes.py
+++ b/algebraic-multigrid_amd/amg_ctypes.py
@@ -191,6 +191,8 @@
     "amg_hip_set_patch_tile_flags": (None, [C.c_int32]),
     "amg_hip_set_patch_xf": (None, [C.c_int32]),
     "amg_hip_set_patch_tall": (None, [C.c_int32]),
+    "amg_hip_set_patch_coltype": (None, [C.c_int32]),
+    "amg_hip_patch_tile_classes": (C.c_int, [C.c_void_p, C.c_int32, C.c_int32, _i64p]),
     "amg_hip_set_patch_seam": (None, [C.c_int32]),
     "amg_hip_patch_leg_lines": (C.c_int32, [C.c_void_p, C.c_int32, C.c_int32]),
     "amg_hip_create_rs": (C.c_int, [C.c_int64, _i32p, _i32p, _f64p, _f64p, C.c_int32, C.c_double, C.c_int64,
@@ -417,6 +419,10 @@
     lib().amg_hip_set_patch_tall(int(bool(on)))
 
 
+def set_patch_coltype(on):
+    lib().amg_hip_set_patch_coltype(int(bool(on)))
+
+
 def set_patch_seam(on):
     lib().amg_hip_set_patch_seam(int(bool(on)))
 
@@ -1108,6 +1114,14 @@
     def patch_leg_lines(self, level, leg):
         return int(lib().amg_hip_patch_leg_lines(self._h, int(level), int(leg)))
 
+    def patch_tile_classes(self, level, rings):
+        out = np.zeros(3, np.int64)
+        st = lib().amg_hip_patch_tile_classes(self._h, int(level), int(rings), out.ctypes.data_as(_i64p))
+        if st == EINVAL:
+            raise ValueError(lib().amg_hip_last_error().decode())
+        _chk(st)
+        return tuple(int(v) for v in out)
+
     def profile_fine_sweep(self, n_launches):
         a, b = C.c_double(0), C.c_double(0)
         _chk(lib().amg_hip_profile_fine_sweep(self._h, n_launches, C.byref(a), C.byref(b)))
diff --git a/algebraic-multigrid_amd/csrc/kernels.hip b/algebraic-multigrid_amd/csrc/kernels.hip
--- a/algebraic-multigrid_amd/csrc/kernels.hip
+++ b/algebraic-multigrid_amd/csrc/kernels.hip
@@ -1612,6 +1612,8 @@
 constexpr int PATCH_K = PATCH_EH * PATCH_EC / PATCH_NT;
 constexpr int PATCH_BUF = (PATCH_EH + 2) * PATCH_EC;
 constexpr int PATCH_MAXTAB = 192;
+constexpr uint32_t PATCH_FLAG_COLTYPED = 254u, PATCH_FLAG_GENERAL = 255u;
+constexpr int PATCH_SEAM_RINGS_HOST = 5;
 static_assert(PATCH_EH * PATCH_EC == PATCH_K * PATCH_NT && PATCH_NT % PATCH_EC == 0, "patch geometry");
 template <int EH_, int EC_>
 struct PatchFrameT {
@@ -1634,9 +1636,11 @@
   bool uniform;
   uint32_t tu;
   bool flagged;
+  bool coltyped;
   __device__ __forceinline__ uint32_t type(int k) const {
-    return flagged ? tu : (ty[k >> 2] >> (8 * (k & 3))) & 255u;
-  }
+    return flagged ? tu : (coltyped ? ty[0] : (ty[k >> 2] >> (8 * (k & 3))) & 255u);
+  }
+  __device__ __forceinline__ uint32_t lane_type() const { return ty[0]; }
 };
 
 struct PatchU {
@@ -1734,6 +1738,53 @@
     }
   }
 }
+constexpr int PATCH_CT = 10;
+static_assert((PATCH_MAXTAB / 5) * PATCH_CT * sizeof(double) <= PATCH_MAXTAB * 16,
+              "the slot tables of (ntypes + 1) <= PATCH_MAXTAB / 5 types fit tabJ and tabR");
+template <bool RESID, bool BAR, class FR = PatchFrame>
+__device__ __forceinline__ void patch_eval_c(const double* buf, int cell0, uint32_t tl, const double* ctab,
+                                             const double (&f)[PATCH_K], double omega, double (&res)[PATCH_K]) {
+  const double* p = buf + cell0 - FR::EC;
+  int to = (int)tl * PATCH_CT;
+  uint32_t rmask = 0;
+  if (RESID) rmask = reinterpret_cast<const uint32_t*>(ctab + to + 9)[0];
+  double w[3][3];
+#pragma unroll
+  for (int r = 0; r < 2; ++r)
+#pragma unroll
+    for (int c = 0; c < 3; ++c) w[r][c] = p[r * FR::EC + c - 1];
+#pragma unroll
+  for (int k = 0; k < PATCH_K; ++k) {
+    if (!BAR) asm("" : "+v"(to));
+    const double* wt = ctab + to;
+#pragma unroll
+    for (int c = 0; c < 3; ++c) w[2][c] = p[(k + 2) * FR::EC + c - 1];
+    const double xi = w[1][1];
+    double acc = RESID ? f[k] : 0.0;
+#pragma unroll
+    for (int s9 = 0; s9 < 9; ++s9) {
+      if (BAR && s9 == 5) __builtin_amdgcn_sched_barrier(0);
+      if (!RESID && s9 == 4) continue;
+      const double t = wt[s9] * w[s9 / 3][s9 % 3];
+      if (RESID) acc -= ((rmask >> s9) & 1u) ? t : 0.0;
+      else acc += t;
+    }
+    if (RESID) {
+      res[k] = acc;
+    } else {
+      const double diag = wt[9];
+      const bool nod = diag == 0.0;
+      const double q = (f[k] - acc) / (nod ? 1.0 : diag);
+      res[k] = nod ? xi : xi + omega * (q - xi);
+    }
+#pragma unroll
+    for (int c = 0; c < 3; ++c) {
+      w[0][c] = w[1][c];
+      w[1][c] = w[2][c];
+    }
+    if (BAR) __builtin_amdgcn_sched_barrier(0);
+  }
+}
 template <int UN, bool RESID, bool GS = false>
 __device__ __forceinline__ double patch_eval(const double* buf, int cell, uint32_t type,
                                              const PatchJ* tabJ, const PatchR* tabR, double fi,
@@ -1778,7 +1829,7 @@
   return nod ? xi : (GS ? q : xi + omega * (q - xi));
 }
 
-template <int UN, int UM, bool RESID, bool NT, bool ZERO, int TH, class FR = PatchFrame>
+template <int UN, int UM, bool RESID, bool NT, bool ZERO, int TH, class FR = PatchFrame, bool CBAR = false>
 __device__ __forceinline__ void patch_stage(const PatchCells& pc, int m, int ntypes, double* buf,
                                             const PatchU& U, const PatchJ* tabJ, const PatchR* tabR,
                                             double omega, int l0, int l1, int c0, int c1, double* out) {
@@ -1793,6 +1844,9 @@
   }
   if (pc.uniform && U.rmask == (uint32_t)UM) {
     patch_eval_u<RESID, (UM & 0x145) != 0, false, (UM & 0x145) ? -1 : UM, FR>(buf, pc.cell0, U, pc.f, omega, res);
+  } else if (pc.coltyped) {
+    patch_eval_c<RESID, CBAR, FR>(buf, pc.cell0, pc.lane_type(),
+                            reinterpret_cast<const double*>(RESID ? (const void*)tabR : (const void*)tabJ), pc.f, omega, res);
   } else {
 #pragma unroll
     for (int k = 0; k < PATCH_K; ++k)
@@ -1883,6 +1937,10 @@
   if (pc.uniform) {
 #pragma unroll
     for (int k = 0; k < PATCH_K; ++k) dv[k] = U.diag;
+  } else if (pc.coltyped) {
+    const double d = utabd[(size_t)pc.lane_type() * 19 + 18];
+#pragma unroll
+    for (int k = 0; k < PATCH_K; ++k) dv[k] = d;
   } else {
 #pragma unroll
     for (int k = 0; k < PATCH_K; ++k) dv[k] = utabd[(size_t)pc.type(k) * 19 + 18];
@@ -1896,9 +1954,9 @@
   }
 }
 
-template <int RINGS, bool PROLONG, bool XF = false, class FR = PatchFrame>
+template <int RINGS, bool PROLONG, bool XF = false, class FR = PatchFrame, bool COLT = true>
 __device__ __forceinline__ void patch_load(PatchCells& pc, PatchU& U, const uint8_t* __restrict__ tflag,
-                                           int tile, int n, int m,
+                                           const uint8_t* __restrict__ ctype, int tile, int n, int m,
                                            int j0, int i0, const double* __restrict__ x,
                                            const double* __restrict__ f,
                                            const uint8_t* __restrict__ rtype, int ntypes,
@@ -1939,12 +1997,30 @@
     }
   }
   __builtin_amdgcn_sched_barrier(0);
-  const uint32_t tf = tflag ? patch_flag(tflag, tile) : 255u;
+  const uint32_t tf = tflag ? patch_flag(tflag, tile) : PATCH_FLAG_GENERAL;
   const uint32_t nty = (uint32_t)ntypes;
-  pc.flagged = tf != 255u;
+  pc.flagged = tf < PATCH_FLAG_COLTYPED;
+  pc.coltyped = COLT && ctype != nullptr && tf == PATCH_FLAG_COLTYPED;
   if (pc.flagged) {
     pc.tu = tf;
     pc.uniform = true;
+  } else if (pc.coltyped) {
+    const uint32_t tl = (uint32_t)ctype[(int64_t)tile * FR::EC + col];
+    const int t = (int)threadIdx.x, tt = t / PATCH_CT, tj = t - tt * PATCH_CT;
+    const bool stage = t < (ntypes + 1) * PATCH_CT;
+    double vj = 0.0, vr = 0.0;
+    if (stage) {
+      vj = utabd[tt * 19 + (tj < 9 ? tj : 18)];
+      vr = tj < 9 ? utabd[tt * 19 + 9 + tj] : __longlong_as_double((long long)(uint32_t)utabi[tt * 2]);
+    }
+    pc.ty[0] = tl;
+    pc.ty[1] = 0;
+    pc.tu = (uint32_t)__builtin_amdgcn_readfirstlane((int)tl);
+    pc.uniform = __builtin_amdgcn_ballot_w64(tl != pc.tu) == 0;
+    if (stage) {
+      reinterpret_cast<double*>(tabJ)[t] = vj;
+      reinterpret_cast<double*>(tabR)[t] = vr;
+    }
   } else {
     PatchTabRow tb;
     patch_issue_tables(tb, ptab, nent);
@@ -1968,9 +2044,11 @@
     patch_stage_tables<FR>(tabJ, tabR, tb, nent);
   }
   {
-    int fl = pc.flagged;
+    int fl = (pc.flagged ? 1 : 0) | (pc.coltyped ? 2 : 0);
     asm("" : "+v"(fl));
-    pc.flagged = __builtin_amdgcn_readfirstlane(fl) != 0;
+    fl = __builtin_amdgcn_readfirstlane(fl);
+    pc.flagged = (fl & 1) != 0;
+    pc.coltyped = COLT && (fl & 2) != 0;
   }
   patch_load_u(U, pc.uniform ? pc.tu : 0u, utabd, utabi);
   __builtin_amdgcn_sched_barrier(0);
@@ -2008,23 +2086,34 @@
 
 __global__ __launch_bounds__(256) void patch_tile_flags_kernel(int n, int m, int px_count, int rings, int eh, int ec,
                                                                const uint8_t* __restrict__ rtype,
-                                                               int ntypes, uint8_t* __restrict__ flag) {
+                                                               int ntypes, uint8_t* __restrict__ flag,
+                                                               uint8_t* __restrict__ ctype) {
   const int tile = blockIdx.x;
   const int py = tile / px_count, px = tile - py * px_count;
   const int64_t base = (int64_t)(py * (eh - 2 * rings) - rings) * m + px * PATCH_TW - (ec - PATCH_TW) / 2;
   const int64_t first = base < 0 ? 0 : (base < n ? base : n - 1);
   const uint32_t t0 = rtype[first];
   int ok = base >= 0 && t0 < (uint32_t)ntypes;
+  int okc = base >= 0 && base + (int64_t)(eh - 1) * m + ec <= (int64_t)n;
   for (int q = threadIdx.x; q < eh * ec; q += 256) {
     const int le = q / ec, c = q - le * ec;
     const int64_t r = base + (int64_t)le * m + c;
-    ok = ok && r >= 0 && r < (int64_t)n && rtype[r < 0 ? 0 : (r < n ? r : n - 1)] == t0;
+    const uint32_t t = rtype[r < 0 ? 0 : (r < n ? r : n - 1)];
+    ok = ok && r >= 0 && r < (int64_t)n && t == t0;
+    if (okc) {
+      const uint32_t tc = rtype[base + c];
+      okc = tc < (uint32_t)ntypes && t == tc;
+    }
   }
   ok = __syncthreads_and(ok);
-  if (threadIdx.x == 0) flag[tile] = ok ? (uint8_t)t0 : (uint8_t)255;
-}
+  okc = __syncthreads_and(okc) && ctype != nullptr;
+  if (threadIdx.x == 0)
+    flag[tile] = ok ? (uint8_t)t0 : (okc ? (uint8_t)PATCH_FLAG_COLTYPED : (uint8_t)PATCH_FLAG_GENERAL);
+  if (!ok && okc && (int)threadIdx.x < ec) ctype[(int64_t)tile * ec + threadIdx.x] = rtype[base + threadIdx.x];
+}
+int patch_frame_columns(int rings) { return rings == PATCH_SEAM_RINGS_HOST ? 76 : PATCH_EC; }
 hipError_t launch_patch_tile_flags(int64_t n, int64_t m, int rings, const uint8_t* rtype, int ntypes,
-                                   uint8_t* flag, int64_t* n_tiles, hipStream_t st) {
+                                   uint8_t* flag, int64_t* n_tiles, hipStream_t st, uint8_t* ctype) {
   if (!patch_geometry_ok(n, m) || !patch_rings_ok(rings)) return hipErrorInvalidValue;
   const int64_t lines = (n + m - 1) / m;
   const int pxc = (int)(m / PATCH_TW);
@@ -2033,7 +2122,8 @@
   if (n_tiles) *n_tiles = tiles;
   if (!flag) return hipSuccess;
   hipLaunchKernelGGL(patch_tile_flags_kernel, dim3((unsigned)tiles), dim3(256), 0, st, (int)n, (int)m, pxc,
-                     rings, PATCH_EH, PATCH_EC, rtype, ntypes, flag);
+                     rings, PATCH_EH, PATCH_EC, rtype, ntypes, flag,
+                     ntypes < (int)PATCH_FLAG_COLTYPED ? ctype : nullptr);
   return hipGetLastError();
 }
 
@@ -2068,8 +2158,13 @@
 
 #ifdef AMG_PATCH_STAMPS
 __device__ unsigned long long* g_patch_stamps = nullptr;
-__device__ __forceinline__ void patch_stamp(int k) {
-  if (threadIdx.x == 0 && g_patch_stamps) {
+__device__ int g_patch_stamps_rows = 0;
+__device__ __forceinline__ void patch_stamp_flag(int n, int ftile, uint32_t tf) {
+  if (threadIdx.x == 0 && g_patch_stamps && (g_patch_stamps_rows == 0 || g_patch_stamps_rows == n))
+    g_patch_stamps[(size_t)blockIdx.x * 8 + 6] = ((unsigned long long)(unsigned)ftile << 8) | (tf & 255u);
+}
+__device__ __forceinline__ void patch_stamp(int k, int n) {
+  if (threadIdx.x == 0 && g_patch_stamps && (g_patch_stamps_rows == 0 || g_patch_stamps_rows == n)) {
     unsigned long long t = __builtin_amdgcn_s_memrealtime();
     asm volatile("s_waitcnt lgkmcnt(0)" ::: "memory");
     g_patch_stamps[(size_t)blockIdx.x * 8 + k] = t;
@@ -2083,9 +2178,14 @@
 hipError_t debug_set_patch_stamps(unsigned long long* p) {
   return hipMemcpyToSymbol(HIP_SYMBOL(g_patch_stamps), &p, sizeof(p));
 }
-#define PATCH_STAMP(k) patch_stamp(k)
+hipError_t debug_set_patch_stamps_rows(int rows) {
+  return hipMemcpyToSymbol(HIP_SYMBOL(g_patch_stamps_rows), &rows, sizeof(rows));
+}
+#define PATCH_STAMP(k) patch_stamp(k, n)
+#define PATCH_STAMP_FLAG(ftile, tf) patch_stamp_flag(n, ftile, tf)
 #else
 #define PATCH_STAMP(k)
+#define PATCH_STAMP_FLAG(ftile, tf)
 #endif
 template <int UN, int UM, bool FIRST, bool NT, bool XF = false, int RINGS = 3>
 #ifndef AMG_PATCH_WAVES
@@ -2097,7 +2197,7 @@
     int nent, int ntypes, const double* x, const double* __restrict__ f, double* u_out, double* r_out, int nH,
     double* __restrict__ fH, const double* __restrict__ diagH, double* __restrict__ uH1,
     double omega, int xcd_map, int py0, const uint8_t* __restrict__ tflag,
-    const uint8_t* __restrict__ cflag, double dHu) {
+    const uint8_t* __restrict__ cflag, double dHu, const uint8_t* __restrict__ ctype) {
   __shared__ double buf[PATCH_BUF];
   __shared__ PatchJ tabJ[PATCH_MAXTAB];
   __shared__ PatchR tabR[PATCH_MAXTAB];
@@ -2111,12 +2211,13 @@
   const int ftile = (py + py0) * px_count + px;
   static_assert(!(FIRST && XF), "level 0 starts from its own u");
   static_assert(RINGS == 3 || (RINGS == 2 && !FIRST), "three dependent stages (FIRST) need three rings");
-  patch_load<RINGS, false, XF>(pc, U, tflag, ftile, n, m, j0, i0, x, f, rtype, ntypes, nullptr, 0, ptab, nent,
+  patch_load<RINGS, false, XF, PatchFrame, UN != 5>(pc, U, tflag, ctype, ftile, n, m, j0, i0, x, f, rtype, ntypes, nullptr, 0, ptab, nent,
                                utabd, utabi, omega, buf, tabJ, tabR);
   patch_prologue<UM>(pc, U, buf, tabJ, tabR, ptab, nent);
   const bool cuni = uH1 && cflag && patch_flag(cflag, ftile) != 0;
   lds_barrier();
   PATCH_STAMP(1);
+  PATCH_STAMP_FLAG(ftile, pc.flagged ? pc.tu : (pc.coltyped ? PATCH_FLAG_COLTYPED : PATCH_FLAG_GENERAL));
   if (FIRST) {
     patch_stage<UN, UM, false, NT, false, TH>(pc, m, ntypes, buf, U, tabJ, tabR, omega, -2, TH + 2, -2,
                                               PATCH_TW + 3, nullptr);
@@ -2157,7 +2258,8 @@
     int n, int m, int px_count, const uint8_t* __restrict__ rtype, const double* __restrict__ ptab,
     const double* __restrict__ utabd, const int32_t* __restrict__ utabi,
     int nent, int ntypes, const double* x, const double* __restrict__ f, const double* __restrict__ uH, int nH,
-    double* u_out, double omega, int xcd_map, int py0, const uint8_t* __restrict__ tflag) {
+    double* u_out, double omega, int xcd_map, int py0, const uint8_t* __restrict__ tflag,
+    const uint8_t* __restrict__ ctype) {
   __shared__ double buf[PATCH_BUF];
   __shared__ PatchJ tabJ[PATCH_MAXTAB];
   __shared__ PatchR tabR[PATCH_MAXTAB];
@@ -2168,26 +2270,28 @@
   const int j0 = (py + py0) * TH, i0 = px * PATCH_TW;
   PatchCells pc;
   PatchU U;
-  patch_load<RINGS, true>(pc, U, tflag, (py + py0) * px_count + px, n, m, j0, i0, x, f, rtype, ntypes, uH, nH,
+  patch_load<RINGS, true>(pc, U, tflag, ctype, (py + py0) * px_count + px, n, m, j0, i0, x, f, rtype, ntypes, uH, nH,
                           ptab, nent, utabd, utabi, omega, buf, tabJ, tabR);
   patch_prologue<UM>(pc, U, buf, tabJ, tabR, ptab, nent);
   lds_barrier();
-  patch_stage<UN, UM, false, NT, false, TH>(pc, m, ntypes, buf, U, tabJ, tabR, omega, -1, TH + 1, -1,
-                                            PATCH_TW + 1, nullptr);
+  patch_stage<UN, UM, false, NT, false, TH, PatchFrame, true>(pc, m, ntypes, buf, U, tabJ, tabR, omega, -1, TH + 1, -1,
+                                                              PATCH_TW + 1, nullptr);
   lds_barrier();
-  patch_stage<UN, UM, false, NT, false, TH>(pc, m, ntypes, buf, U, tabJ, tabR, omega, 0, TH, 0, PATCH_TW,
-                                            nullptr);
+  patch_stage<UN, UM, false, NT, false, TH, PatchFrame, true>(pc, m, ntypes, buf, U, tabJ, tabR, omega, 0, TH, 0,
+                                                              PATCH_TW, nullptr);
   lds_barrier();
   patch_copy_out<NT, RINGS>(buf, u_out, n, m, j0, i0);
 }
 
 constexpr int PATCH_SEAM_RINGS = 5;
+static_assert(PATCH_SEAM_RINGS == PATCH_SEAM_RINGS_HOST, "patch_frame_columns");
 template <int UN, int UM, bool NT, class FR, int WAVES>
 __global__ __launch_bounds__(FR::NT, WAVES) void patch_seam_kernel(
     int n, int m, int px_count, const uint8_t* __restrict__ rtype, const double* __restrict__ ptab,
     const double* __restrict__ utabd, const int32_t* __restrict__ utabi,
     int nent, int ntypes, const double* x, const double* __restrict__ f, const double* __restrict__ uH, int nH,
-    double* u_out, double* __restrict__ fH, double omega, int xcd_map, const uint8_t* __restrict__ tflag) {
+    double* u_out, double* __restrict__ fH, double omega, int xcd_map, const uint8_t* __restrict__ tflag,
+    const uint8_t* __restrict__ ctype) {
   __shared__ double buf[FR::BUF];
   __shared__ PatchJ tabJ[PATCH_MAXTAB];
   __shared__ PatchR tabR[PATCH_MAXTAB];
@@ -2198,7 +2302,7 @@
   const int j0 = py * TH, i0 = px * PATCH_TW;
   PatchCells pc;
   PatchU U;
-  patch_load<RINGS, true, false, FR>(pc, U, tflag, tile, n, m, j0, i0, x, f, rtype, ntypes, uH, nH, ptab, nent,
+  patch_load<RINGS, true, false, FR>(pc, U, tflag, ctype, tile, n, m, j0, i0, x, f, rtype, ntypes, uH, nH, ptab, nent,
                                      utabd, utabi, omega, buf, tabJ, tabR);
   patch_prologue<UM, FR>(pc, U, buf, tabJ, tabR, ptab, nent);
   lds_barrier();
@@ -2277,7 +2381,7 @@
   const int j0 = (py + py0) * TH, i0 = px * PATCH_TW;
   PatchCells pc;
   PatchU U;
-  patch_load<RINGS, PROLONG>(pc, U, tflag, (py + py0) * px_count + px, n, m, j0, i0, x, f, rtype, ntypes, uH, nH,
+  patch_load<RINGS, PROLONG, false, PatchFrame, false>(pc, U, tflag, nullptr, (py + py0) * px_count + px, n, m, j0, i0, x, f, rtype, ntypes, uH, nH,
                              ptab, nent, utabd, utabi, 1.0, buf, tabJ, tabR);
   patch_prologue<UM>(pc, U, buf, tabJ, tabR, ptab, nent);
   uint32_t cbits = 0;
@@ -2370,7 +2474,7 @@
   hipLaunchKernelGGL((patch_down_kernel<decltype(U)::value, decltype(M)::value, FST, decltype(NTF)::value, XFF, RG>), \
                      dim3(grid), dim3(PATCH_NT), 0, st, (int)n, (int)m, pxc, P.rtype, P.ptab, P.utabd, P.utabi, \
                      P.nent, P.ntypes, x, f, u_out, r_out, (int)nH, fH, diagH, uH1, omega, xm, py0, P.tflag,    \
-                     P.cflag, P.dHu)
+                     P.cflag, P.dHu, P.ctype)
     if (first) AMG_DOWN(true, false, 3);
     else if (xf && P.rings == 2) AMG_DOWN(false, true, 2);
     else if (xf) AMG_DOWN(false, true, 3);
@@ -2393,7 +2497,7 @@
 #define AMG_UP(RG)                                                                                            \
   hipLaunchKernelGGL((patch_up_kernel<decltype(U)::value, decltype(M)::value, decltype(NTF)::value, RG>),     \
                      dim3(grid), dim3(PATCH_NT), 0, st, (int)n, (int)m, pxc, P.rtype, P.ptab, P.utabd, P.utabi, \
-                     P.nent, P.ntypes, x, f, uH, (int)nH, u_out, omega, xm, py0, P.tflag)
+                     P.nent, P.ntypes, x, f, uH, (int)nH, u_out, omega, xm, py0, P.tflag, P.ctype)
     if (P.rings == 2) AMG_UP(2);
     else AMG_UP(3);
 #undef AMG_UP
@@ -2405,8 +2509,9 @@
 static bool patch_seam_geometry_ok(int64_t n, int64_t m) {
   return patch_geometry_ok(n, m) && n < ((int64_t)1 << 31) - 64 * m - 128;
 }
+static_assert(SeamFrame::EC == 76, "patch_frame_columns");
 hipError_t launch_patch_seam_flags(int64_t n, int64_t m, const uint8_t* rtype, int ntypes, uint8_t* flag,
-                                   int64_t* n_tiles, hipStream_t st) {
+                                   int64_t* n_tiles, hipStream_t st, uint8_t* ctype) {
   if (!patch_seam_geometry_ok(n, m)) return hipErrorInvalidValue;
   const int64_t lines = (n + m - 1) / m;
   const int pxc = (int)(m / PATCH_TW);
@@ -2415,7 +2520,8 @@
   if (n_tiles) *n_tiles = tiles;
   if (!flag) return hipSuccess;
   hipLaunchKernelGGL(patch_tile_flags_kernel, dim3((unsigned)tiles), dim3(256), 0, st, (int)n, (int)m, pxc,
-                     PATCH_SEAM_RINGS, SeamFrame::EH, SeamFrame::EC, rtype, ntypes, flag);
+                     PATCH_SEAM_RINGS, SeamFrame::EH, SeamFrame::EC, rtype, ntypes, flag,
+                     ntypes < (int)PATCH_FLAG_COLTYPED ? ctype : nullptr);
   return hipGetLastError();
 }
 hipError_t launch_patch_seam(int64_t n, int64_t m, const PatchRef& P, const double* x, const double* f,
@@ -2432,7 +2538,7 @@
 #define AMG_SEAM(NTF)                                                                                          \
   hipLaunchKernelGGL((patch_seam_kernel<5, 0x0BA, NTF, SeamFrame, PATCH_SEAM_WAVES>), dim3(grid), dim3(SeamFrame::NT), \
                      0, st, (int)n, (int)m, pxc, P.rtype, P.ptab, P.utabd, P.utabi, P.nent, P.ntypes, x, f, uH,  \
-                     (int)nH, u_out, fH, omega, xm, P.tflag)
+                     (int)nH, u_out, fH, omega, xm, P.tflag, P.ctype)
   if (P.nt) AMG_SEAM(true);
   else AMG_SEAM(false);
 #undef AMG_SEAM
diff --git a/algebraic-multigrid_amd/csrc/kernels.hpp b/algebraic-multigrid_amd/csrc/kernels.hpp
--- a/algebraic-multigrid_amd/csrc/kernels.hpp
+++ b/algebraic-multigrid_amd/csrc/kernels.hpp
@@ -183,6 +183,7 @@
   const int32_t* utabi = nullptr;
   int rings = 3;
   const uint8_t* tflag = nullptr;
+  const uint8_t* ctype = nullptr;
   int nent = 0, ntypes = 0, un = 0, nt = 0;
   int umask = 0;
   const uint8_t* cflag = nullptr;
@@ -191,7 +192,8 @@
 hipError_t launch_patch_coarse_flags(int64_t n, int64_t m, int rings, int64_t nH, const double* diagH,
                                      double dref, uint8_t* cflag, hipStream_t st);
 hipError_t launch_patch_tile_flags(int64_t n, int64_t m, int rings, const uint8_t* rtype, int ntypes,
-                                   uint8_t* flag, int64_t* n_tiles, hipStream_t st);
+                                   uint8_t* flag, int64_t* n_tiles, hipStream_t st, uint8_t* ctype = nullptr);
+int patch_frame_columns(int rings);
 bool patch_geometry_ok(int64_t n, int64_t m);
 int patch_un(int longest_row);
 int patch_default_umask(int un);
@@ -209,7 +211,7 @@
                            hipStream_t st, int64_t line_lo = 0, int64_t line_hi = -1);
 int patch_seam_lines();
 hipError_t launch_patch_seam_flags(int64_t n, int64_t m, const uint8_t* rtype, int ntypes, uint8_t* flag,
-                                   int64_t* n_tiles, hipStream_t st);
+                                   int64_t* n_tiles, hipStream_t st, uint8_t* ctype = nullptr);
 hipError_t launch_patch_seam(int64_t n, int64_t m, const PatchRef& P, const double* x, const double* f,
                              const double* uH, int64_t nH, double* u_out, double* fH, double omega,
                              hipStream_t st);
diff --git a/algebraic-multigrid_amd/csrc/solver.cpp b/algebraic-multigrid_amd/csrc/solver.cpp
--- a/algebraic-multigrid_amd/csrc/solver.cpp
+++ b/algebraic-multigrid_amd/csrc/solver.cpp
@@ -23,7 +23,10 @@
 
 using namespace amg_hip;
 #ifdef AMG_PATCH_STAMPS
-namespace amg_hip { hipError_t debug_set_patch_stamps(unsigned long long* p); }
+namespace amg_hip {
+hipError_t debug_set_patch_stamps(unsigned long long* p);
+hipError_t debug_set_patch_stamps_rows(int rows);
+}
 #endif
 
 namespace {
@@ -289,6 +292,13 @@
 int g_patch_xf = 1;
 int g_patch_tall = 1;
 int g_patch_seam = 1;
+int g_patch_coltype = 1;
+static hipError_t alloc_patch_ctype(DevMem& ct, int64_t tiles, int rings) {
+  ct.release();
+  if (!g_patch_coltype) return hipSuccess;
+  const hipError_t e = ct.alloc(((size_t)tiles * (size_t)patch_frame_columns(rings) + 3) & ~(size_t)3);
+  return e != hipSuccess ? e : hipMemset(ct.p, 0, ct.bytes);
+}
 
 struct DevMat {
   bool sell = false;
@@ -314,6 +324,7 @@
   int64_t patch_m = 0;
   int patch_un = 0, patch_ntypes = 0, patch_umask = 0;
   DevMem patch_tab, patch_utabd, patch_utabi, patch_flags, patch_flags2, patch_flags5;
+  DevMem patch_ctype, patch_ctype2, patch_ctype5;
   DevMem patch_cflags;
   int patch_crings = 3;
   double patch_dH = 0.0;
@@ -324,6 +335,7 @@
     P.rtype = drtype.as<uint8_t>();
     P.tflag = g_patch_tile_flags ? (rings == 2 ? patch_flags2 : (rings == 5 ? patch_flags5 : patch_flags)).as<uint8_t>()
                                  : nullptr;
+    P.ctype = P.tflag ? (rings == 2 ? patch_ctype2 : (rings == 5 ? patch_ctype5 : patch_ctype)).as<uint8_t>() : nullptr;
     P.cflag = g_patch_tile_flags && rings == patch_crings ? patch_cflags.as<uint8_t>() : nullptr;
     P.dHu = patch_dH;
     P.ptab = patch_tab.as<double>();
@@ -614,19 +626,22 @@
       int64_t tiles = 0;
       for (int rings = 2; rings <= 3; ++rings) {
         DevMem& F = rings == 2 ? D->patch_flags2 : D->patch_flags;
+        DevMem& CT = rings == 2 ? D->patch_ctype2 : D->patch_ctype;
         if ((e = launch_patch_tile_flags(n, D->patch_m, rings, nullptr, nty, nullptr, &tiles, nullptr)) != hipSuccess) return e;
         if ((e = F.alloc(((size_t)tiles + 3) & ~(size_t)3)) != hipSuccess) return e;
         if ((e = hipMemset(F.p, 0, F.bytes)) != hipSuccess) return e;
+        if ((e = alloc_patch_ctype(CT, tiles, rings)) != hipSuccess) return e;
         if ((e = launch_patch_tile_flags(n, D->patch_m, rings, D->drtype.as<uint8_t>(), nty, F.as<uint8_t>(),
-                                         nullptr, nullptr)) != hipSuccess) return e;
+                                         nullptr, nullptr, CT.as<uint8_t>())) != hipSuccess) return e;
       }
       if (patch_un(un) == 5) {
         int64_t t5 = 0;
         if ((e = launch_patch_seam_flags(n, D->patch_m, nullptr, nty, nullptr, &t5, nullptr)) == hipSuccess) {
           if ((e = D->patch_flags5.alloc(((size_t)t5 + 3) & ~(size_t)3)) != hipSuccess) return e;
           if ((e = hipMemset(D->patch_flags5.p, 0, D->patch_flags5.bytes)) != hipSuccess) return e;
+          if ((e = alloc_patch_ctype(D->patch_ctype5, t5, 5)) != hipSuccess) return e;
           if ((e = launch_patch_seam_flags(n, D->patch_m, D->drtype.as<uint8_t>(), nty, D->patch_flags5.as<uint8_t>(),
-                                           nullptr, nullptr)) != hipSuccess) return e;
+                                           nullptr, nullptr, D->patch_ctype5.as<uint8_t>())) != hipSuccess) return e;
         }
       }
       if ((e = hipDeviceSynchronize()) != hipSuccess) return e;
@@ -4375,6 +4390,7 @@
 void amg_hip_set_patch_xf(int32_t on) { g_patch_xf = on ? 1 : 0; }
 void amg_hip_set_patch_tall(int32_t on) { g_patch_tall = on ? 1 : 0; }
 void amg_hip_set_patch_seam(int32_t on) { g_patch_seam = on ? 1 : 0; }
+void amg_hip_set_patch_coltype(int32_t on) { g_patch_coltype = on ? 1 : 0; }
 void amg_hip_set_band_chain(int32_t on) { g_no_band_chain = on ? 0 : 1; }
 void amg_hip_set_tail_fusion(int32_t on) { g_tail_fusion = on ? 1 : 0; }
 void amg_hip_set_pair_duo(int32_t on) { g_pair_duo = on ? 1 : 0; }
@@ -5053,6 +5069,10 @@
   HIP_TRY(debug_set_patch_stamps((unsigned long long*)dev_ptr));
   return AMG_HIP_OK;
 }
+amg_hip_status amg_hip_debug_patch_stamps_rows(int32_t rows) {
+  HIP_TRY(debug_set_patch_stamps_rows((int)rows));
+  return AMG_HIP_OK;
+}
 #endif
 
 amg_hip_status amg_hip_get_stream(amg_hip_solver* s, void** stream) {
@@ -5789,6 +5809,29 @@
   return patch_tile_lines(patch_rings(s, leg == 0 && level == 0));
 }
 
+amg_hip_status amg_hip_patch_tile_classes(amg_hip_solver* s, int32_t level, int32_t rings, int64_t* out) {
+  if (!s || !out || s->opt.host_only || level < 0 || level >= (int32_t)s->lv.size())
+    return fail(AMG_HIP_EINVAL, "amg_hip_patch_tile_classes: bad argument");
+  if (rings != 2 && rings != 3 && rings != 5)
+    return fail(AMG_HIP_EINVAL, "amg_hip_patch_tile_classes: rings is 2 (44-line tiles), 3 (42) or 5 (the seam's, 38)");
+  const LegForm form = current_plan(s).lv[(size_t)level].up;
+  const DevMat& A = s->lv[(size_t)level].A_rows;
+  const DevMem& F = rings == 2 ? A.patch_flags2 : (rings == 5 ? A.patch_flags5 : A.patch_flags);
+  if ((form != LEG_PATCH && form != LEG_MC_PATCH) || !A.patch || !F.p)
+    return fail(AMG_HIP_EINVAL, "amg_hip_patch_tile_classes: the level is no K-Patch level (or has no tiles of this geometry)");
+  int64_t tiles = 0;
+  const int64_t n = s->lv[(size_t)level].n;
+  const amg_hip_status r = set_device(s);
+  if (r != AMG_HIP_OK) return r;
+  HIP_TRY(rings == 5 ? launch_patch_seam_flags(n, A.patch_m, nullptr, A.patch_ntypes, nullptr, &tiles, nullptr)
+                     : launch_patch_tile_flags(n, A.patch_m, rings, nullptr, A.patch_ntypes, nullptr, &tiles, nullptr));
+  std::vector<uint8_t> fl((size_t)tiles);
+  HIP_TRY(hipMemcpy(fl.data(), F.p, fl.size(), hipMemcpyDeviceToHost));
+  out[0] = out[1] = out[2] = 0;
+  for (uint8_t f : fl) ++out[f == 255 ? 2 : (f == 254 ? 1 : 0)];
+  return AMG_HIP_OK;
+}
+
 amg_hip_status amg_hip_fine_sweep_info(const amg_hip_solver* s, char* name, int32_t name_cap,
                                        int32_t* sweeps_per_launch, double* bytes_per_launch) {
   if (!s || !name || name_cap < 32) return fail(AMG_HIP_EINVAL, "bad argument");
diff --git a/include/amg_hip.h b/include/amg_hip.h
--- a/include/amg_hip.h
+++ b/include/amg_hip.h
@@ -80,6 +80,7 @@
 void amg_hip_set_patch_tile_flags(int32_t on);
 void amg_hip_set_patch_xf(int32_t on);
 void amg_hip_set_patch_tall(int32_t on);
+void amg_hip_set_patch_coltype(int32_t on);
 void amg_hip_set_patch_seam(int32_t on);
 void amg_hip_set_band_chain(int32_t on);
 
@@ -318,6 +319,7 @@
 amg_hip_status amg_hip_profile_fine_sweep(amg_hip_solver* s, int32_t n_launches,
                                           double* avg_ms, double* min_ms);
 int32_t amg_hip_patch_leg_lines(const amg_hip_solver* s, int32_t level, int32_t leg);
+amg_hip_status amg_hip_patch_tile_classes(amg_hip_solver* s, int32_t level, int32_t rings, int64_t* out);
 amg_hip_status amg_hip_fine_sweep_info(const amg_hip_solver* s, char* name, int32_t name_cap,
                                        int32_t* sweeps_per_launch, double* bytes_per_launch);
 
```
